# mauruszach/multimodal_diffusion

Measured on AMD Instinct MI355X. Metric: denoising steps/sec @256x256 multimodal-cond batch=32, higher is better.
Workload: dtype f32 via 3xbf16 split operands (6-term products, f32 accumulate; fp32-level error); 1 GPU; C3: 256x256 audio->video CFG denoising step (cond+null MMDiT d512 L8 H8 + noise head + DDIM), 384+37 tokens, batch 32 per GPU, DDIM 50 steps, guidance 3.5; global_batch=32, sampler_steps=50, parallelism=dp1, launch=eager, matmul=bf16x3, attn=default, cfg_halves=one stacked 2B batch, one stream

## Files before the change

include/avdiff_hip.h:

```cpp
#ifndef AVDIFF_HIP_H
#define AVDIFF_HIP_H

#include <stdint.h>

#ifdef __cplusplus
extern "C" {
#endif

#define AVD_ABI_VERSION 7

#define AVD_OK            0
#define AVD_EINVAL       -1
#define AVD_EUNSUPPORTED -2
#define AVD_ELAUNCH      -3
#define AVD_EWORKSPACE   -4

#define AVD_ACT_NONE 0
#define AVD_ACT_GELU 1
#define AVD_ACT_SILU 2
#define AVD_ACT_TANH 3
#define AVD_ACT_RELU 4
#define AVD_ACT_LEAKY_RELU 5

typedef void* avd_stream_t;

int         avd_abi_version(void);
const char* avd_last_error(void);
int         avd_device_arch(char* buf, int buflen);
int         avd_tune_set(const char* key, int64_t value);

int avd_rmsnorm_f32(const float* x, const float* scale, float* y, int64_t rows, int d, float eps,
                    avd_stream_t stream);

int avd_gemm_bias_act_f32(const float* A, int64_t lda, const float* W, const float* bias,
                          const float* residual, int64_t ldr, float* C, int64_t ldc,
                          int64_t M, int N, int K, int act, avd_stream_t stream);

int avd_gemm_rmsfold_f32(const float* A, const float* W, const float* bias, const float* residual, float* C, int64_t M,
                         int N, int K, int act, const float* ss_in, int ss_in_cols, float eps, float* ss_out,
                         avd_stream_t stream);

int avd_attn_fwd_f32(const float* qkv, float* out, int B, int N, int H, int Dh, float scale,
                     int n_query, const uint8_t* key_padding_mask, avd_stream_t stream);

int avd_layernorm_act_f32(const float* x, const float* gamma, const float* beta, float* y,
                          int64_t rows, int d, float eps, int act, avd_stream_t stream);

int avd_timestep_embedding_f32(const int64_t* t, const float* freqs, float* out, int B, int dim, float max_period,
                               avd_stream_t stream);

int avd_tube_patch_f32(const float* z, float* tok, int B, int C, int T, int H, int W, int t, int h, int w,
                       avd_stream_t stream);
int avd_tube_unpatch_f32(const float* tok, float* z, int B, int C, int T, int H, int W, int t, int h, int w,
                         avd_stream_t stream);

int avd_audio_tokens_f32(const float* z, float* tok, int B, int Ca, int F, int len, int stride,
                         avd_stream_t stream);
int avd_audio_untokens_f32(const float* tok, const float* window, float* z, int B, int Ca, int F, int len, int stride,
                           avd_stream_t stream);

int avd_ddim_step_f32(const float* x_t, const float* eps_hat, const int64_t* t_now, const int64_t* t_prev,
                      const float* alpha_bar, int T_train, float eta, const float* noise,
                      float* x_prev, int B, int64_t per_sample, avd_stream_t stream);

int avd_dpmpp_2m_step_f32(const float* x_t, const float* eps_hat, float* x0_hist, const int64_t* t_last, const int64_t* t_now,
                          const int64_t* t_prev, const float* alpha_bar, int T_train, float* x_out, int B, int64_t per_sample,
                          avd_stream_t stream);

int avd_dpmpp_2m_sde_step_f32(const float* x_t, const float* eps_hat, float* x0_hist, const int64_t* t_last, const int64_t* t_now,
                              const int64_t* t_prev, const float* alpha_bar, int T_train, float eta, const float* noise, float* x_out,
                              int B, int64_t per_sample, avd_stream_t stream);

typedef struct {
    uint64_t seed;
    int64_t sample_offset;
} avd_noise_key;
int avd_gaussian_noise_f32(const avd_noise_key* key, const int64_t* t_now, float* out, int B, int64_t per_sample,
                           avd_stream_t stream);

int avd_canvas_noise_f32(const avd_noise_key* key, const int64_t* t_now, float* out, int N, int64_t outer, int L, int hop,
                         int64_t inner, avd_stream_t stream);

// ... 277 lines not shown
```

multimodal_diffusion_amd/_lib.py:

```python
from __future__ import annotations

import ctypes as C
import os
from pathlib import Path
from typing import Optional

import torch

_HERE = Path(__file__).resolve().parent
LIB_PATH = Path(os.environ.get("AVDIFF_HIP_LIB", _HERE / "csrc" / "libavdiff_hip.so"))

ACT_NONE, ACT_GELU, ACT_SILU, ACT_TANH, ACT_RELU, ACT_LEAKY_RELU = 0, 1, 2, 3, 4, 5
EINVAL, EUNSUPPORTED, ELAUNCH, EWORKSPACE = -1, -2, -3, -4


class AvdError(RuntimeError):
    """A HIP-side failure (launch error, unsupported shape, workspace)."""


class EmbedDesc(C.Structure):
    _fields_ = [("target_kind", C.c_int), ("target_first", C.c_int), ("B", C.c_int), ("d", C.c_int),
                ("tdim", C.c_int), ("C", C.c_int), ("T", C.c_int), ("H", C.c_int), ("W", C.c_int),
                ("p0", C.c_int), ("p1", C.c_int), ("p2", C.c_int), ("Nt", C.c_int), ("Np", C.c_int),
                ("temb_freqs", C.c_void_p), ("temb_add", C.c_int)]
# ... 31 lines not shown
                ("guidance", C.c_float), ("eta", C.c_float), ("split_streams", C.c_int)]


class NoiseKey(C.Structure):
    _fields_ = [("seed", C.c_uint64), ("sample_offset", C.c_int64)]


class LatentGuide(C.Structure):
    _fields_ = [("known", C.c_void_p), ("mask", C.c_void_p), ("mask_batch_stride", C.c_int64), ("key", NoiseKey)]


class CfgControl(C.Structure):
    _fields_ = [("guidance", C.c_void_p), ("rescale", C.c_void_p), ("stats", C.c_void_p), ("stats_bytes", C.c_int64)]


class VaeDecodeDesc(C.Structure):
    _fields_ = [("B", C.c_int), ("Cv", C.c_int), ("Tp", C.c_int), ("Hp", C.c_int), ("Wp", C.c_int),
                ("T", C.c_int), ("H", C.c_int), ("W", C.c_int),
                ("base", C.c_int), ("n_blocks", C.c_int), ("out_ch", C.c_int), ("out_tanh", C.c_int),
                ("gn_eps", C.c_float),
                ("from_lat_w", C.c_void_p), ("from_lat_b", C.c_void_p),
                ("conv_w", C.POINTER(C.c_void_p)), ("conv_b", C.POINTER(C.c_void_p)),
                ("gn_w", C.POINTER(C.c_void_p)), ("gn_b", C.POINTER(C.c_void_p)),
                ("to_img_w", C.c_void_p), ("to_img_b", C.c_void_p),
                ("conv_w3", C.POINTER(C.c_void_p)), ("conv_terms", C.c_int),
                ("conv_w_scale", C.POINTER(C.c_float)), ("conv_a_scale", C.POINTER(C.c_float)),
                ("conv0_lat_w3", C.c_void_p), ("conv0_lat_btab", C.c_void_p), ("conv0_lat_w_scale", C.c_float),
                ("conv0_lat_packed", C.c_int)]


class VaeEncodeDesc(C.Structure):
    _fields_ = [("B", C.c_int), ("in_ch", C.c_int), ("T", C.c_int), ("H", C.c_int), ("W", C.c_int),
                ("t_down", C.c_int), ("s_down", C.c_int),
                ("base", C.c_int), ("n_blocks", C.c_int), ("lat_ch", C.c_int), ("gn_eps", C.c_float),
                ("conv_w", C.POINTER(C.c_void_p)), ("conv_b", C.POINTER(C.c_void_p)),
                ("gn_w", C.POINTER(C.c_void_p)), ("gn_b", C.POINTER(C.c_void_p)),
                ("to_lat_w", C.c_void_p), ("to_lat_b", C.c_void_p),
                ("conv_w3", C.POINTER(C.c_void_p)), ("conv_terms", C.c_int),
                ("conv_w_scale", C.POINTER(C.c_float)), ("conv_a_scale", C.POINTER(C.c_float)),
                ("conv0_pk_w3", C.c_void_p)]


ABI_VERSION = 7
_P, _I, _L, _F = C.c_void_p, C.c_int, C.c_int64, C.c_float

SIGNATURES = {
    "avd_abi_version": (_I, []),
    "avd_last_error": (C.c_char_p, []),
    "avd_device_arch": (_I, [C.c_char_p, _I]),
    "avd_rmsnorm_f32": (_I, [_P, _P, _P, _L, _I, _F, _P]),
    "avd_gemm_bias_act_f32": (_I, [_P, _L, _P, _P, _P, _L, _P, _L, _L, _I, _I, _I, _P]),
    "avd_gemm_rmsfold_f32": (_I, [_P, _P, _P, _P, _P, _L, _I, _I, _I, _P, _I, _F, _P, _P]),
    "avd_tune_set": (_I, [C.c_char_p, _L]),
    "avd_attn_fwd_f32": (_I, [_P, _P, _I, _I, _I, _I, _F, _I, _P, _P]),
    "avd_layernorm_act_f32": (_I, [_P, _P, _P, _P, _L, _I, _F, _I, _P]),
    "avd_timestep_embedding_f32": (_I, [_P, _P, _P, _I, _I, _F, _P]),
    "avd_tube_patch_f32": (_I, [_P, _P] + [_I] * 8 + [_P]),
    "avd_tube_unpatch_f32": (_I, [_P, _P] + [_I] * 8 + [_P]),
    "avd_audio_tokens_f32": (_I, [_P, _P] + [_I] * 5 + [_P]),
    "avd_audio_untokens_f32": (_I, [_P, _P, _P] + [_I] * 5 + [_P]),
    "avd_ddim_step_f32": (_I, [_P, _P, _P, _P, _P, _I, _F, _P, _P, _I, _L, _P]),
    "avd_cfg_unpatch_ddim_f32": (_I, [_P, _P, _P, _P, _P, _I, _F, _F, _P, _P] + [_I] * 8 + [_P]),
    "avd_cfg_untoken_ddim_audio_f32": (_I, [_P, _P, _P, _P, _P, _I, _F, _F, _P, _P] + [_I] * 5 + [_P]),
    "avd_embed_workspace_floats": (_L, [C.POINTER(EmbedDesc)]),
    "avd_embed_cfg_pair_f32": (_I, [C.POINTER(EmbedDesc), _P, _P, _P, _P, _P, _P, _P, _P]),
    "avd_core_workspace_bytes": (_L, [C.POINTER(CoreWeights), _I, _I]),
    "avd_core_forward_f32": (_I, [C.POINTER(CoreWeights), _P, _P, _I, _I, _I, _I, _P, _P, _L, _P]),
    "avd_head_workspace_bytes": (_L, [C.POINTER(HeadWeights), _L]),
    "avd_head_forward_f32": (_I, [C.POINTER(HeadWeights), _P, _L, _L, _L, _L, _P, _P, _L, _P]),
    "avd_step_workspace_bytes": (_L, [C.POINTER(StepDesc)]),
    "avd_denoise_step_f32": (_I, [C.POINTER(StepDesc), _P, _P, _P, _P, _P, _P, _P, _L, _P]),
    "avd_denoise_step_seeded_f32": (_I, [C.POINTER(StepDesc), C.POINTER(NoiseKey), _P, _P, _P, _P, _P, _P, _L, _P]),
    "avd_gaussian_noise_f32": (_I, [C.POINTER(NoiseKey), _P, _P, _I, _L, _P]),
    "avd_canvas_noise_f32": (_I, [C.POINTER(NoiseKey), _P, _P, _I, _L, _I, _I, _L, _P]),
    "avd_denoise_step_canvas_f32": (_I, [C.POINTER(StepDesc), C.POINTER(NoiseKey), _I, C.POINTER(CfgControl), C.POINTER(LatentGuide), _I,
                                         _P, _P, _P, _P, _P, _P, _L, _P]),
    "avd_sched_advance": (_I, [_P, _I, _P, _P, _P, _I, _P]),
    "avd_sched_advance_ms": (_I, [_P, _I, _P, _P, _P, _P, _I, _P]),
    "avd_dpmpp_2m_step_f32": (_I, [_P, _P, _P, _P, _P, _P, _P, _I, _P, _I, _L, _P]),
    "avd_denoise_step_dpmpp_2m_f32": (_I, [C.POINTER(StepDesc), _P, _P, _P, _P, _P, _P, _P, _P, _L, _P]),
    "avd_dpmpp_2m_sde_step_f32": (_I, [_P, _P, _P, _P, _P, _P, _P, _I, _F, _P, _P, _I, _L, _P]),
    "avd_denoise_step_dpmpp_2m_sde_f32": (_I, [C.POINTER(StepDesc), C.POINTER(NoiseKey), _I, C.POINTER(CfgControl), C.POINTER(LatentGuide),
                                               _I, _P, _P, _P, _P, _P, _P, _P, _P, _L, _P]),
    "avd_latent_guide_f32": (_I, [C.POINTER(LatentGuide), _P, _P, _I, _P, _P, _I, _L, _P]),
    "avd_latent_guide_canvas_f32": (_I, [C.POINTER(LatentGuide), _P, _P, _I, _P, _P, _I, _L, _I, _I, _L, _P]),
    "avd_denoise_step_canvas_guided_f32": (_I, [C.POINTER(StepDesc), C.POINTER(LatentGuide), _I, C.POINTER(NoiseKey), C.POINTER(CfgControl),
                                                _I, _P, _P, _P, _P, _P, _P, _P, _P, _L, _P]),
    "avd_denoise_step_guided_f32": (_I, [C.POINTER(StepDesc), C.POINTER(LatentGuide), C.POINTER(NoiseKey), _P, _P, _P, _P, _P, _P, _P,
                                         _P, _L, _P]),
    "avd_cfg_stats_bytes": (_L, [_I, _L]),
    "avd_cfg_rescale_f32": (_I, [_P, _P, _P, _P, _L, _P, _I, _L, _P]),
    "avd_denoise_step_cfg_f32": (_I, [C.POINTER(StepDesc), C.POINTER(CfgControl), C.POINTER(LatentGuide), C.POINTER(NoiseKey), _P, _P, _P,
                                      _P, _P, _P, _P, _P, _L, _P]),
    "avd_eps_unpatch_ddim_f32": (_I, [_P, _P, _P, _P, _P, _I, _F, _P, _P] + [_I] * 8 + [C.POINTER(NoiseKey), _P, _P, C.POINTER(LatentGuide), _P]),
    "avd_eps_untoken_ddim_audio_f32": (_I, [_P, _P, _P, _P, _P, _I, _F, _P, _P] + [_I] * 5 + [C.POINTER(NoiseKey), _P, _P,
                                                                                               C.POINTER(LatentGuide), _P]),
    "avd_embed_cond_f32": (_I, [C.POINTER(EmbedDesc), _P, _P, _P, _P, _P, _P, _P, _P, _P]),
    "avd_denoise_step_cond_f32": (_I, [C.POINTER(StepDesc), C.POINTER(LatentGuide), C.POINTER(NoiseKey), _P, _P, _P, _P, _P, _P, _P, _P,
                                       _P, _L, _P]),
    "avd_split3_bytes": (_L, [_L, _I]),
    "avd_split3_f32": (_I, [_P, _P, _L, _I, _P]),
    "avd_rmsnorm_split3_f32": (_I, [_P, _P, _P, _L, _I, _F, _P]),
    "avd_attn_fwd_split3_f32": (_I, [_P, _P, _I, _I, _I, _I, _F, _I, _P]),
    "avd_qkv3_bytes": (_L, [_I, _I, _I]),
    "avd_gemm_bf16x3_qkv3_f32": (_I, [_P, _P, _P, _P, _L, _I, _I, _I, _F, _I, _P]),
    "avd_attn_fwd_qkv3_f32": (_I, [_P, _P, _P, _I, _I, _I, _I, _I, _P]),
# ... 98 lines not shown
```

multimodal_diffusion_amd/csrc/attn_bf16x3.hip:

```cpp
#include "avd_common.h"

#include <stdlib.h>
#include <type_traits>

namespace avd {

constexpr int A3_DH = 64, A3_KT = 64, A3_NW = 4;
constexpr float A3_NEG = -1.0e30f;

typedef short s16x4 __attribute__((ext_vector_type(4)));
typedef unsigned int u32x2 __attribute__((ext_vector_type(2)));
typedef float f32x4t __attribute__((ext_vector_type(4)));

#define AVD_LDS_PTR(p) ((__attribute__((address_space(3))) void*)(p))
#define AVD_GLB_PTR(p) ((const __attribute__((address_space(1))) void*)(p))

template <int TERMS> struct A3Terms;
template <> struct A3Terms<6> { static constexpr int N = 6; static constexpr int PA[6] = {2, 0, 1, 1, 0, 0}; static constexpr int PB[6] = {0, 2, 1, 0, 1, 0}; };
template <> struct A3Terms<9> { static constexpr int N = 9; static constexpr int PA[9] = {2, 2, 1, 2, 0, 1, 1, 0, 0}; static constexpr int PB[9] = {2, 1, 2, 0, 2, 1, 0, 1, 0}; };
template <> struct A3Terms<1> { static constexpr int N = 1; static constexpr int PA[1] = {0}; static constexpr int PB[1] = {0}; };
template <> struct A3Terms<3> { static constexpr int N = 3; static constexpr int PA[3] = {0, 1, 0}; static constexpr int PB[3] = {1, 0, 0}; };

template <bool SPLIT_OUT, int TERMS>
__global__ __launch_bounds__(A3_NW * 64, 2) void attn_bf16x3_kernel(const unsigned char* __restrict__ img, float* __restrict__ out,
                                                                    int Bt, int N, int Npad, int H, int n_query, int nqb,
                                                                    float s_inv2, float v_inv, float o_scale, int out_tok) {
    constexpr int NW = A3_NW, ROWB = QKV3_ROWB;
    constexpr bool F16 = TERMS == 3;
    constexpr int NPL = s3_planes(TERMS);
    constexpr int PPW = 24 / NW;
    __shared__ __attribute__((aligned(16))) unsigned char Ks[A3_KT * ROWB];
    __shared__ __attribute__((aligned(16))) unsigned char Vs[A3_KT * ROWB];

    int qb, h, b;
    {
        const int nwg = gridDim.x, id = blockIdx.x, q = nwg >> 3, r = nwg & 7, x = id & 7;
        const int w = (x < r ? x * (q + 1) : r * (q + 1) + (x - r) * q) + (id >> 3);
        qb = w % nqb;
        h = (w / nqb) % H;
        b = w / (nqb * H);
    }
    const int tid = threadIdx.x, lane = tid & 63, wave = tid >> 6;
    const int l31 = lane & 31, hi = lane >> 5;
    const int64_t hstride = (int64_t)Npad * ROWB;
    const unsigned char* Qb = img + (((int64_t)0 * Bt + b) * H + h) * hstride;
    const unsigned char* Kb = img + (((int64_t)1 * Bt + b) * H + h) * hstride;
    const unsigned char* Vb = img + (((int64_t)2 * Bt + b) * H + h) * hstride;

    const int q_row = qb * (NW * 32) + wave * 32 + l31;
    bf16x8 qf[4][3];
    {
        const unsigned char* src = Qb + (int64_t)(q_row < N ? q_row : N - 1) * ROWB + hi * 16;
#pragma unroll
        for (int s = 0; s < 4; ++s)
#pragma unroll
            for (int p = 0; p < NPL; ++p) qf[s][p] = *reinterpret_cast<const bf16x8*>(src + p * 128 + s * 32);
    }

    auto dma = [&](const unsigned char* gsrc, unsigned char* ldst, int kt) {
        const int last_row = N - 1 - kt * A3_KT;
#pragma unroll
        for (int i = 0; i < PPW; ++i) {
            const int p = wave + NW * i;
            const int off = p * 1024 + lane * 16;
            int row = off / ROWB;
            const int within = off - row * ROWB;
            row = row < last_row ? row : last_row;
            __builtin_amdgcn_global_load_lds(AVD_GLB_PTR(gsrc + ((int64_t)kt * A3_KT + row) * ROWB + within), AVD_LDS_PTR(ldst + p * 1024), 16,
                                             0, 0);
        }
    };

    f32x16 o0, o1;
#pragma unroll
    for (int r = 0; r < 16; ++r) { o0[r] = 0.f; o1[r] = 0.f; }
    float m_run = A3_NEG, l_run = 0.f;

    const int nkt = (N + A3_KT - 1) / A3_KT;
    dma(Kb, Ks, 0);
    dma(Vb, Vs, 0);
    __builtin_amdgcn_s_waitcnt(0x0f70);
    __syncthreads();

    const int ksw = (l31 >> 1) & 7;
    const int k_rd = l31 * ROWB;
    const int i16 = lane & 15, cb = (lane >> 4) & 1;
    const int v_q = i16 >> 2, v_p = i16 & 3;

    const bool active = qb * (NW * 32) + wave * 32 < n_query;
    for (int kt = 0; kt < nkt; ++kt) {
        const bool more = (kt + 1) < nkt;
        if (!active) {
            __builtin_amdgcn_s_waitcnt(0x0f70);
            __syncthreads();
// ... 80 lines not shown
                const int key0 = 32 * kb + 16 * t + 4 * hi + v_q;
                const int sw = qkv3_swizzle(2, key0);
#pragma unroll
                for (int db = 0; db < 2; ++db) {
                    const int chunk = 4 * db + 2 * cb + (v_p >> 1);
                    bf16x8 vf[3];
#pragma unroll
                    for (int p = 0; p < NPL; ++p) {
                        const s16x4 lo = __builtin_amdgcn_ds_read_tr16_b64_v4i16((__attribute__((address_space(3))) s16x4*)AVD_LDS_PTR(
                            Vs + key0 * ROWB + p * 128 + ((chunk ^ sw) << 4) + 8 * (v_p & 1)));
                        const s16x4 up = __builtin_amdgcn_ds_read_tr16_b64_v4i16((__attribute__((address_space(3))) s16x4*)AVD_LDS_PTR(
                            Vs + (key0 + 8) * ROWB + p * 128 + ((chunk ^ sw) << 4) + 8 * (v_p & 1)));
                        const u32x2 a = __builtin_bit_cast(u32x2, lo), c2 = __builtin_bit_cast(u32x2, up);
                        const u32x4 w = {a[0], a[1], c2[0], c2[1]};
                        vf[p] = __builtin_bit_cast(bf16x8, w);
                    }
#pragma unroll
                    for (int tt = 0; tt < TT::N; ++tt) {
                        if (db == 0) o0 = mma16<F16>(vf[TT::PA[tt]], pf[TT::PB[tt]], o0);
                        else o1 = mma16<F16>(vf[TT::PA[tt]], pf[TT::PB[tt]], o1);
                    }
                }
            }
        __builtin_amdgcn_s_waitcnt(0x0f70);
        __syncthreads();
        if (more) dma(Vb, Vs, kt + 1);
    }
    if (!active) return;

    const float l_tot = l_run + __shfl_xor(l_run, 32, 64);
    const float inv = F16 ? v_inv / l_tot : 1.0f / l_tot;
    const int d = H * A3_DH;
    if constexpr (SPLIT_OUT) {
        float ch[8][4];
#pragma unroll
        for (int g4 = 0; g4 < 4; ++g4)
#pragma unroll
            for (int e = 0; e < 4; ++e) {
                ch[g4][e] = o0[4 * g4 + e] * inv;
                ch[4 + g4][e] = o1[4 * g4 + e] * inv;
            }
        unsigned char* o3 = reinterpret_cast<unsigned char*>(out);
#pragma unroll
        for (int c = 0; c < 8; c += 2) {
            float v[8];
#pragma unroll
            for (int e = 0; e < 4; ++e) {
                const float send = hi ? ch[c][e] : ch[c + 1][e];
                const float recv = __shfl_xor(send, 32, 64);
                v[e] = hi ? recv : ch[c][e];
                v[4 + e] = hi ? ch[c + 1][e] : recv;
            }
            if (q_row < n_query) {
                if constexpr (F16) store_split8_h2(o3, (int64_t)b * out_tok + q_row, h * A3_DH + 8 * (c + hi), d, v, o_scale);
                else store_split8(o3, (int64_t)b * out_tok + q_row, h * A3_DH + 8 * (c + hi), d, v);
            }
        }
    } else if (q_row < n_query) {
        float* dst = out + ((int64_t)b * out_tok + q_row) * d + h * A3_DH + 4 * hi;
#pragma unroll
        for (int g4 = 0; g4 < 4; ++g4) {
            f32x4 a = {o0[4 * g4] * inv, o0[4 * g4 + 1] * inv, o0[4 * g4 + 2] * inv, o0[4 * g4 + 3] * inv};
            f32x4 c = {o1[4 * g4] * inv, o1[4 * g4 + 1] * inv, o1[4 * g4 + 2] * inv, o1[4 * g4 + 3] * inv};
            *reinterpret_cast<f32x4*>(dst + 8 * g4) = a;
            *reinterpret_cast<f32x4*>(dst + 32 + 8 * g4) = c;
        }
    }
}

int g_attn_pipe = 1;

template <bool MORE_, bool KCL_, bool VCL_, bool COPY_> struct A3Flags {
    static constexpr bool MORE = MORE_, KCL = KCL_, VCL = VCL_, COPY = COPY_;
};

template <bool SPLIT_OUT, int TERMS>
__global__ __launch_bounds__(A3_NW * 64, 2) void attn_bf16x3_pipe_kernel(const unsigned char* __restrict__ img, float* __restrict__ out,
                                                                         int Bt, int N, int Npad, int H, int n_query, int nqb,
                                                                         float s_inv2, float v_inv, float o_scale, int out_tok) {
    constexpr int NW = A3_NW, ROWB = QKV3_ROWB;
    constexpr bool F16 = TERMS == 3;
    constexpr int NPL = s3_planes(TERMS);
    constexpr int PPW = 24 / NW;
    using TT = A3Terms<TERMS>;
    __shared__ __attribute__((aligned(16))) unsigned char Ks[A3_KT * ROWB];
    __shared__ __attribute__((aligned(16))) unsigned char Vs[A3_KT * ROWB];

    int qb, h, b;
    {
        const int nwg = gridDim.x, id = blockIdx.x, q = nwg >> 3, r = nwg & 7, x = id & 7;
        const int w = (x < r ? x * (q + 1) : r * (q + 1) + (x - r) * q) + (id >> 3);
        qb = w % nqb;
        h = (w / nqb) % H;
        b = w / (nqb * H);
    }
    const int tid = threadIdx.x, lane = tid & 63;
    const int wave = __builtin_amdgcn_readfirstlane(tid >> 6);
    const int l31 = lane & 31, hi = lane >> 5;
    const int64_t hstride = (int64_t)Npad * ROWB;
    const unsigned char* Qb = img + (((int64_t)0 * Bt + b) * H + h) * hstride;
    const unsigned char* Kb = img + (((int64_t)1 * Bt + b) * H + h) * hstride;
    const unsigned char* Vb = img + (((int64_t)2 * Bt + b) * H + h) * hstride;

    const int q_row = qb * (NW * 32) + wave * 32 + l31;
    bf16x8 qf[4][3];
    {
        const unsigned char* src = Qb + (int64_t)(q_row < N ? q_row : N - 1) * ROWB + hi * 16;
#pragma unroll
        for (int s = 0; s < 4; ++s)
#pragma unroll
            for (int p = 0; p < NPL; ++p) qf[s][p] = *reinterpret_cast<const bf16x8*>(src + p * 128 + s * 32);
    }
    auto dma_clamp = [&](const unsigned char* gsrc, unsigned char* ldst, int kt) {
        const int last_row = N - 1 - kt * A3_KT;
#pragma unroll
        for (int i = 0; i < PPW; ++i) {
            const int p = wave + NW * i;
            const int off = p * 1024 + lane * 16;
            int row = off / ROWB;
            const int within = off - row * ROWB;
            row = row < last_row ? row : last_row;
            __builtin_amdgcn_global_load_lds(AVD_GLB_PTR(gsrc + ((int64_t)kt * A3_KT + row) * ROWB + within), AVD_LDS_PTR(ldst + p * 1024), 16,
                                             0, 0);
        }
    };
    const unsigned lane16 = (unsigned)lane * 16u;
    auto dma_full = [&](const unsigned char* gsrc, unsigned char* ldst, int kt) {
        const unsigned char* base = gsrc + ((int64_t)kt * (A3_KT * ROWB) + wave * 1024);
#pragma unroll
        for (int i = 0; i < PPW; ++i)
            __builtin_amdgcn_global_load_lds(AVD_GLB_PTR(base + i * (NW * 1024) + lane16), AVD_LDS_PTR(ldst + (wave + NW * i) * 1024), 16, 0, 0);
    };
    auto sync = [&]() {
        __builtin_amdgcn_s_waitcnt(0x0f70);
        __syncthreads();
    };

    const int nkt = (N + A3_KT - 1) / A3_KT;
    const bool ragged = (N & (A3_KT - 1)) != 0;
    dma_clamp(Kb, Ks, 0);
    dma_clamp(Vb, Vs, 0);
    sync();

    const bool active = qb * (NW * 32) + wave * 32 < n_query;
    if (!active) {
        sync();
        if (nkt > 1) dma_clamp(Kb, Ks, 1);
        sync();
// ... 179 lines not shown
            mt = fmaxf(mt, __shfl_xor(mt, 32, 64));
            m_new = fmaxf(m_run, mt);
            if constexpr (FL::COPY) {
                c0 = n0;
                c1 = n1;
            }
            sync();
            if constexpr (FL::VCL) dma_clamp(Vb, Vs, kt + 1);
            else dma_full(Vb, Vs, kt + 1);
        }
    };
    {
        using Main = A3Flags<true, false, false, false>;
        using MainC = A3Flags<true, false, false, true>;
        using KClamp = A3Flags<true, true, false, true>;
        using VClamp = A3Flags<true, false, true, true>;
        using Last = A3Flags<false, false, false, false>;
        int kt = 0;
        for (; kt + 4 < nkt; kt += 2) {
            tile(Main{}, kt, sa0, sa1, sb0, sb1);
            tile(Main{}, kt + 1, sb0, sb1, sa0, sa1);
        }
        if (nkt - kt == 4) { tile(MainC{}, kt, sa0, sa1, sb0, sb1); ++kt; }
        if (nkt - kt == 3) { tile(KClamp{}, kt, sa0, sa1, sb0, sb1); ++kt; }
        if (nkt - kt == 2) { tile(VClamp{}, kt, sa0, sa1, sb0, sb1); ++kt; }
        tile(Last{}, kt, sa0, sa1, sb0, sb1);
    }
#undef A3_SB

    const float l_tot = l_run + __shfl_xor(l_run, 32, 64);
    const float inv = F16 ? v_inv / l_tot : 1.0f / l_tot;
    const int d = H * A3_DH;
    if constexpr (SPLIT_OUT) {
        float ch[8][4];
#pragma unroll
        for (int g4 = 0; g4 < 4; ++g4)
#pragma unroll
            for (int e = 0; e < 4; ++e) {
                ch[g4][e] = o0[4 * g4 + e] * inv;
                ch[4 + g4][e] = o1[4 * g4 + e] * inv;
            }
        unsigned char* o3 = reinterpret_cast<unsigned char*>(out);
#pragma unroll
        for (int c = 0; c < 8; c += 2) {
            float v[8];
#pragma unroll
            for (int e = 0; e < 4; ++e) {
                const float send = hi ? ch[c][e] : ch[c + 1][e];
                const float recv = __shfl_xor(send, 32, 64);
                v[e] = hi ? recv : ch[c][e];
                v[4 + e] = hi ? ch[c + 1][e] : recv;
            }
            if (q_row < n_query) {
                if constexpr (F16) store_split8_h2(o3, (int64_t)b * out_tok + q_row, h * A3_DH + 8 * (c + hi), d, v, o_scale);
                else store_split8(o3, (int64_t)b * out_tok + q_row, h * A3_DH + 8 * (c + hi), d, v);
            }
        }
    } else if (q_row < n_query) {
        float* dst = out + ((int64_t)b * out_tok + q_row) * d + h * A3_DH + 4 * hi;
#pragma unroll
        for (int g4 = 0; g4 < 4; ++g4) {
            f32x4 a = {o0[4 * g4] * inv, o0[4 * g4 + 1] * inv, o0[4 * g4 + 2] * inv, o0[4 * g4 + 3] * inv};
            f32x4 c = {o1[4 * g4] * inv, o1[4 * g4 + 1] * inv, o1[4 * g4 + 2] * inv, o1[4 * g4 + 3] * inv};
            *reinterpret_cast<f32x4*>(dst + 8 * g4) = a;
            *reinterpret_cast<f32x4*>(dst + 32 + 8 * g4) = c;
        }
    }
}

template <bool F16>
__device__ __forceinline__ f32x4t mma16s(bf16x8 a, bf16x8 b, f32x4t c) {
    if constexpr (F16) return __builtin_amdgcn_mfma_f32_16x16x32_f16(__builtin_bit_cast(f16x8, a), __builtin_bit_cast(f16x8, b), c, 0, 0, 0);
    else return __builtin_amdgcn_mfma_f32_16x16x32_bf16(a, b, c, 0, 0, 0);
}
int g_attn_m16 = 1;

struct S16 { f32x4t t[4][2]; };

template <bool SPLIT_OUT, int TERMS>
__global__ __launch_bounds__(A3_NW * 64, 2) void attn_bf16x3_p16_kernel(const unsigned char* __restrict__ img, float* __restrict__ out,
                                                                        int Bt, int N, int Npad, int H, int n_query, int nqb,
                                                                        float s_inv2, float v_inv, float o_scale, int out_tok) {
    constexpr int NW = A3_NW, ROWB = QKV3_ROWB;
    constexpr bool F16 = TERMS == 3;
    constexpr int NPL = s3_planes(TERMS);
    constexpr int PPW = 24 / NW;
    using TT = A3Terms<TERMS>;
    __shared__ __attribute__((aligned(16))) unsigned char Ks[A3_KT * ROWB];
    __shared__ __attribute__((aligned(16))) unsigned char Vs[A3_KT * ROWB];

    int qb, h, b;
    {
        const int nwg = gridDim.x, id = blockIdx.x, q = nwg >> 3, r = nwg & 7, x = id & 7;
        const int w = (x < r ? x * (q + 1) : r * (q + 1) + (x - r) * q) + (id >> 3);
        qb = w % nqb;
        h = (w / nqb) % H;
        b = w / (nqb * H);
    }
    const int tid = threadIdx.x, lane = tid & 63;
    const int wave = __builtin_amdgcn_readfirstlane(tid >> 6);
    const int l15 = lane & 15, kq = lane >> 4;
    const int64_t hstride = (int64_t)Npad * ROWB;
    const unsigned char* Qb = img + (((int64_t)0 * Bt + b) * H + h) * hstride;
    const unsigned char* Kb = img + (((int64_t)1 * Bt + b) * H + h) * hstride;
    const unsigned char* Vb = img + (((int64_t)2 * Bt + b) * H + h) * hstride;

    const int q_row0 = qb * (NW * 32) + wave * 32 + l15;
    bf16x8 qf[2][2][3];
#pragma unroll
    for (int qt = 0; qt < 2; ++qt) {
        const int qr = q_row0 + 16 * qt;
        const unsigned char* src = Qb + (int64_t)(qr < N ? qr : N - 1) * ROWB + kq * 16;
#pragma unroll
        for (int sd = 0; sd < 2; ++sd)
#pragma unroll
            for (int p = 0; p < NPL; ++p) qf[qt][sd][p] = *reinterpret_cast<const bf16x8*>(src + p * 128 + sd * 64);
    }
    auto dma_clamp = [&](const unsigned char* gsrc, unsigned char* ldst, int kt) {
        const int last_row = N - 1 - kt * A3_KT;
#pragma unroll
        for (int i = 0; i < PPW; ++i) {
            const int p = wave + NW * i;
            const int off = p * 1024 + lane * 16;
            int row = off / ROWB;
            const int within = off - row * ROWB;
            row = row < last_row ? row : last_row;
            __builtin_amdgcn_global_load_lds(AVD_GLB_PTR(gsrc + ((int64_t)kt * A3_KT + row) * ROWB + within), AVD_LDS_PTR(ldst + p * 1024), 16,
                                             0, 0);
        }
    };
    const unsigned lane16 = (unsigned)lane * 16u;
    auto dma_full = [&](const unsigned char* gsrc, unsigned char* ldst, int kt) {
        const unsigned char* base = gsrc + ((int64_t)kt * (A3_KT * ROWB) + wave * 1024);
#pragma unroll
        for (int i = 0; i < PPW; ++i)
            __builtin_amdgcn_global_load_lds(AVD_GLB_PTR(base + i * (NW * 1024) + lane16), AVD_LDS_PTR(ldst + (wave + NW * i) * 1024), 16, 0, 0);
    };
    auto sync = [&]() {
        __builtin_amdgcn_s_waitcnt(0x0f70);
        __syncthreads();
    };

    const int nkt = (N + A3_KT - 1) / A3_KT;
    const bool ragged = (N & (A3_KT - 1)) != 0;
    dma_clamp(Kb, Ks, 0);
    dma_clamp(Vb, Vs, 0);
    sync();

    const bool active = qb * (NW * 32) + wave * 32 < n_query;
    if (!active) {
        sync();
// ... 202 lines not shown
        }
        A3_SB();
        if constexpr (MORE) {
#pragma unroll
            for (int qt = 0; qt < 2; ++qt) {
                if constexpr (F16) mt[qt] *= s_inv2;
                m_new[qt] = fmaxf(m_run[qt], xmax(mt[qt]));
            }
            if constexpr (FL::COPY) c = n;
            sync();
            if constexpr (FL::VCL) dma_clamp(Vb, Vs, kt + 1);
            else dma_full(Vb, Vs, kt + 1);
        }
    };
    {
        using Main = A3Flags<true, false, false, false>;
        using MainC = A3Flags<true, false, false, true>;
        using KClamp = A3Flags<true, true, false, true>;
        using VClamp = A3Flags<true, false, true, true>;
        using Last = A3Flags<false, false, false, false>;
        int kt = 0;
        for (; kt + 4 < nkt; kt += 2) {
            tile(Main{}, kt, sa, sb);
            tile(Main{}, kt + 1, sb, sa);
        }
        if (nkt - kt == 4) { tile(MainC{}, kt, sa, sb); ++kt; }
        if (nkt - kt == 3) { tile(KClamp{}, kt, sa, sb); ++kt; }
        if (nkt - kt == 2) { tile(VClamp{}, kt, sa, sb); ++kt; }
        tile(Last{}, kt, sa, sb);
    }
#undef A3_SB

    float inv[2];
#pragma unroll
    for (int qt = 0; qt < 2; ++qt) {
        const float l_tot = xsum(l_run[qt]);
        inv[qt] = F16 ? v_inv / l_tot : 1.0f / l_tot;
    }
    const int d = H * A3_DH;
    const int q_row = q_row0 + 16 * (kq & 1);
    unsigned char* o3 = reinterpret_cast<unsigned char*>(out);
#pragma unroll
    for (int dt = 0; dt < 4; ++dt) {
        float v[8];
#pragma unroll
        for (int r = 0; r < 4; ++r) {
            const auto sw = __builtin_amdgcn_permlane16_swap(__float_as_uint(o[dt][0][r] * inv[0]), __float_as_uint(o[dt][1][r] * inv[1]), false, false);
            v[r] = __uint_as_float(sw[0]);
            v[4 + r] = __uint_as_float(sw[1]);
        }
        const int col = h * A3_DH + 16 * dt + 8 * (kq >> 1);
        if (q_row < n_query) {
            if constexpr (SPLIT_OUT) {
                if constexpr (F16) store_split8_h2(o3, (int64_t)b * out_tok + q_row, col, d, v, o_scale);
                else store_split8(o3, (int64_t)b * out_tok + q_row, col, d, v);
            } else {
                float* dst = out + ((int64_t)b * out_tok + q_row) * d + col;
                *reinterpret_cast<f32x4*>(dst) = f32x4{v[0], v[1], v[2], v[3]};
                *reinterpret_cast<f32x4*>(dst + 4) = f32x4{v[4], v[5], v[6], v[7]};
            }
        }
    }
}

int64_t qkv3_bytes(int B, int N, int H) { return (int64_t)3 * B * H * qkv3_npad(N) * QKV3_ROWB; }

template <int TERMS>
static void attn3_launch(const unsigned char* img, float* out, void* out3, int B, int N, int Npad, int H, int n_query, int nqb, hipStream_t st,
                         float img_scale, float out_scale, int out_tok) {
    const float s_inv2 = 1.0f / (img_scale * img_scale), v_inv = 1.0f / img_scale;
    if (g_attn_m16 && (TERMS == 6 || TERMS == 9 || g_attn_m16 == 2)) {
        if (out3)
            hipLaunchKernelGGL((attn_bf16x3_p16_kernel<true, TERMS>), dim3(nqb * H * B), dim3(A3_NW * 64), 0, st, img, static_cast<float*>(out3),
                               B, N, Npad, H, n_query, nqb, s_inv2, v_inv, out_scale, out_tok);
        else
            hipLaunchKernelGGL((attn_bf16x3_p16_kernel<false, TERMS>), dim3(nqb * H * B), dim3(A3_NW * 64), 0, st, img, out, B, N, Npad, H,
                               n_query, nqb, s_inv2, v_inv, out_scale, out_tok);
        return;
    }
    if (g_attn_pipe == 2 || (g_attn_pipe == 1 && (TERMS == 6 || TERMS == 9))) {
        if (out3)
            hipLaunchKernelGGL((attn_bf16x3_pipe_kernel<true, TERMS>), dim3(nqb * H * B), dim3(A3_NW * 64), 0, st, img, static_cast<float*>(out3),
                               B, N, Npad, H, n_query, nqb, s_inv2, v_inv, out_scale, out_tok);
        else
            hipLaunchKernelGGL((attn_bf16x3_pipe_kernel<false, TERMS>), dim3(nqb * H * B), dim3(A3_NW * 64), 0, st, img, out, B, N, Npad, H,
                               n_query, nqb, s_inv2, v_inv, out_scale, out_tok);
        return;
    }
    if (out3)
        hipLaunchKernelGGL((attn_bf16x3_kernel<true, TERMS>), dim3(nqb * H * B), dim3(A3_NW * 64), 0, st, img, static_cast<float*>(out3), B, N,
                           Npad, H, n_query, nqb, s_inv2, v_inv, out_scale, out_tok);
    else
        hipLaunchKernelGGL((attn_bf16x3_kernel<false, TERMS>), dim3(nqb * H * B), dim3(A3_NW * 64), 0, st, img, out, B, N, Npad, H, n_query, nqb,
                           s_inv2, v_inv, out_scale, out_tok);
}

int attn_bf16x3(const void* qkv3, float* out, void* out3, int B, int N, int H, int n_query, int terms, hipStream_t st, float img_scale,
                float out_scale, int out_tokens) {
    const int out_tok = out_tokens > 0 ? out_tokens : N;
    AVD_REQUIRE(out_tok >= n_query, AVD_EINVAL, "attn_bf16x3: out_tokens=%d < n_query=%d", out_tok, n_query);
    AVD_REQUIRE(terms == 0 || terms == 6 || terms == 9 || terms == 1 || terms == 3, AVD_EINVAL, "attn_bf16x3: terms must be 6, 9, 1 or 3, got %d", terms);
    AVD_REQUIRE(img_scale > 0.f && img_scale < __builtin_inff() && out_scale > 0.f && out_scale < __builtin_inff() &&
                    img_scale * img_scale < __builtin_inff(), AVD_EINVAL, "attn_bf16x3: image scales must be positive and finite");
    AVD_REQUIRE(qkv3 && (out || out3), AVD_EINVAL, "attn_bf16x3: null pointer");
    AVD_REQUIRE(B > 0 && N > 0 && H > 0, AVD_EINVAL, "attn_bf16x3: bad dims B=%d N=%d H=%d", B, N, H);
    AVD_REQUIRE(n_query >= 0 && n_query <= N, AVD_EINVAL, "attn_bf16x3: n_query=%d outside [0,%d]", n_query, N);
    AVD_REQUIRE(aligned16(qkv3) && aligned16(out) && aligned16(out3), AVD_EUNSUPPORTED, "attn_bf16x3: pointers must be 16-byte aligned");
    AVD_REQUIRE(!out3 || (H * A3_DH) % 16 == 0, AVD_EUNSUPPORTED, "attn_bf16x3: split3 output needs d %% 16 == 0");
    if (n_query == 0) return AVD_OK;
    const int nqb = (n_query + 32 * A3_NW - 1) / (32 * A3_NW);
    AVD_REQUIRE((int64_t)B * H * nqb < (1ll << 31), AVD_EUNSUPPORTED, "attn_bf16x3: grid too large");
    const int tag = prof_tag_id("attn_bf16x3_kernel<%d>", terms ? terms : 6);
    ProfScope prof(tag, 4.0 * (double)B * H * (double)n_query * N * A3_DH, st);
    const int Npad = qkv3_npad(N);
    const auto* img = static_cast<const unsigned char*>(qkv3);
    if (terms == 9) attn3_launch<9>(img, out, out3, B, N, Npad, H, n_query, nqb, st, 1.f, 1.f, out_tok);
    else if (terms == 1) attn3_launch<1>(img, out, out3, B, N, Npad, H, n_query, nqb, st, 1.f, 1.f, out_tok);
    else if (terms == 3) attn3_launch<3>(img, out, out3, B, N, Npad, H, n_query, nqb, st, img_scale, out_scale, out_tok);
    else attn3_launch<6>(img, out, out3, B, N, Npad, H, n_query, nqb, st, 1.f, 1.f, out_tok);
    AVD_CHECK_LAUNCH("attn_bf16x3");
    return AVD_OK;
}

}

extern "C" int64_t avd_qkv3_bytes(int B, int N, int H) {
    if (B <= 0 || N <= 0 || H <= 0) return -1;
    return avd::qkv3_bytes(B, N, H);
}
extern "C" int avd_attn_fwd_qkv_f16x2_f32(const void* qkv, float* out, void* out2, int B, int N, int H, int n_query, float qkv_scale,
                                          float out_scale, avd_stream_t stream) {
    return avd::attn_bf16x3(qkv, out, out2, B, N, H, n_query, 3, static_cast<hipStream_t>(stream), qkv_scale, out_scale);
}
extern "C" int avd_attn_fwd_qkv3_f32(const void* qkv3, float* out, void* out3, int B, int N, int H, int n_query, int terms,
                                     avd_stream_t stream) {
    return avd::attn_bf16x3(qkv3, out, out3, B, N, H, n_query, terms, static_cast<hipStream_t>(stream));
}
```

multimodal_diffusion_amd/csrc/avd_common.h:

```cpp
#pragma once
#include <hip/hip_runtime.h>
#include <stdint.h>
#include <stdio.h>
#include <stdarg.h>
#include <atomic>

#include "../../include/avdiff_hip.h"

namespace avd {

int set_error(int code, const char* fmt, ...);

#define AVD_REQUIRE(cond, code, ...)                       \
    do {                                                   \
        if (!(cond)) return avd::set_error((code), __VA_ARGS__); \
    } while (0)

#define AVD_CHECK_LAUNCH(name)                                                          \
    do {                                                                                \
        hipError_t e__ = hipGetLastError();                                             \
        if (e__ != hipSuccess)                                                          \
            return avd::set_error(AVD_ELAUNCH, "%s: %s", (name), hipGetErrorString(e__)); \
    } while (0)

struct LdsAttr {
    std::atomic<uint64_t> done{0};
    int ensure(const void* kern, int lds_bytes, const char* what);
};

static inline bool aligned16(const void* p) { return (reinterpret_cast<uintptr_t>(p) & 15u) == 0; }

typedef float f32x4 __attribute__((ext_vector_type(4)));
typedef float f32x16 __attribute__((ext_vector_type(16)));

constexpr int kWave = 64;

__device__ __forceinline__ int mfma32_row(int r, int hi) { return (r & 3) + 8 * (r >> 2) + 4 * hi; }

__device__ __forceinline__ float gelu_erf(float x) {
    const float z = x * 0.70710678118654752440f;
    const float a = fabsf(z);
    const float t = __builtin_amdgcn_rcpf(fmaf(0.3275911f, a, 1.0f));
    float p = fmaf(1.061405429f, t, -1.453152027f);
    p = fmaf(p, t, 1.421413741f);
    p = fmaf(p, t, -0.284496736f);
    p = fmaf(p, t, 0.254829592f);
    p *= t;
    const float e = __builtin_amdgcn_exp2f(-a * a * 1.4426950408889634f);
    const float er = copysignf(fmaf(-p, e, 1.0f), z);
    return 0.5f * x * (1.0f + er);
}
__device__ __forceinline__ float silu(float x) { return x / (1.0f + expf(-x)); }

template <int ACT>
__device__ __forceinline__ float apply_act(float x) {
    if constexpr (ACT == AVD_ACT_GELU) return gelu_erf(x);
    else if constexpr (ACT == AVD_ACT_SILU) return silu(x);
    else return x;
}

__device__ __forceinline__ float wave_sum(float v) {
#pragma unroll
    for (int o = 32; o > 0; o >>= 1) v += __shfl_xor(v, o, 64);
    return v;
}

struct RowMap {
    int64_t ld;
    int64_t seg;
    int64_t stride;
    __host__ __device__ __forceinline__ int64_t off(int64_t r) const {
        return seg > 0 ? (r / seg) * stride + (r % seg) * ld : r * ld;
    }
};

struct TubeGather {
    int T, H, W, t, h, w, Ht, Wt, Nt;
    int64_t per;
    __host__ __device__ __forceinline__ int64_t row_off(int64_t row) const {
        const int64_t b = row / Nt;
        const int n = (int)(row - b * Nt);
        const int nx = n % Wt, ny = (n / Wt) % Ht, nt = n / (Wt * Ht);
        return b * per + ((int64_t)(nt * t) * H + ny * h) * W + nx * w;
    }
    __host__ __device__ __forceinline__ int64_t k_off(int k) const {
        const int dx = k % w, dy = (k / w) % h, dt = (k / (w * h)) % t, c = k / (w * h * t);
        return (((int64_t)c * T + dt) * H + dy) * W + dx;
    }
};

typedef __bf16 bf16x8 __attribute__((ext_vector_type(8)));
typedef unsigned int u32x4 __attribute__((ext_vector_type(4)));

constexpr int S3_CHUNK = 128 * 96;
constexpr int S3_PLANE = 128 * 32;

typedef __bf16 bf16x2 __attribute__((ext_vector_type(2)));
typedef float f32x2 __attribute__((ext_vector_type(2)));

__device__ __forceinline__ unsigned int pk_bf16(float a, float b) {
    const f32x2 v = {a, b};
    return __builtin_bit_cast(unsigned int, __builtin_convertvector(v, bf16x2));
}
__device__ __forceinline__ float bf16_lo(unsigned int p) { return __uint_as_float(p << 16); }
__device__ __forceinline__ float bf16_hi(unsigned int p) { return __uint_as_float(p & 0xffff0000u); }

template <bool RANGE_CHECK = true>
__device__ __forceinline__ void split8(const float* v, u32x4& H, u32x4& Mi, u32x4& Lo) {
#pragma clang fp contract(off)
    bool edge = false;
    if constexpr (RANGE_CHECK) {
        float amax = fabsf(v[0]);
#pragma unroll
        for (int e = 1; e < 8; ++e) amax = fmaxf(amax, fabsf(v[e]));
        edge = __any(amax > 3.3895313892515355e38f);
    }
#pragma unroll
    for (int e = 0; e < 4; ++e) {
        const float a = v[2 * e], b = v[2 * e + 1];
        unsigned int h = pk_bf16(a, b);
        float ra = a - bf16_lo(h), rb = b - bf16_hi(h);
        if (edge) {
            if ((h & 0x7fffu) == 0x7f80u) {
                if (fabsf(a) < __builtin_inff()) { h = (h & 0xffff8000u) | 0x7f7fu; ra = a - bf16_lo(h); } else ra = 0.f;
            }
// ... 76 lines not shown
             float* C, RowMap cm, int64_t M, int N, int K, int act, hipStream_t st);
int gemm_f32_tube(const float* z, const TubeGather& tg, const float* W, const float* bias, float* C, RowMap cm, int64_t M, int N, int K,
                  hipStream_t st);

extern int g_gemm_stages;
extern int g_gemm_force_tile;
bool gemm_f32_fold_supported(int N, int K);
int gemm_f32_fold(const float* A, RowMap am, const float* W, const float* bias, const float* R, RowMap rm, float* C, RowMap cm,
                  int64_t M, int N, int K, int act, const float* ss_in, int ss_in_cols, float sqrt_d, float eps, float* ss_out,
                  hipStream_t st);
int rowss_f32(const float* x, float* ss, int64_t rows, int d, hipStream_t st);
constexpr int kGemmSplitKMax = 4;
extern int g_gemm_splitk;
int gemm_f32_splitk_slices(int64_t M, int N, int K);
int64_t gemm_f32_splitk_ws_max_floats(int64_t M, int N, int K);
int gemm_f32_splitk(const float* A, RowMap am, const float* W, const float* bias, const float* R, RowMap rm, float* C, RowMap cm, int64_t M,
                    int N, int K, int ns, float* part, float* ss_out, hipStream_t st);

int attn_f32(const float* qkv, float* out, int B, int N, int H, int Dh, float scale, int n_query, const unsigned char* key_padding_mask,
             hipStream_t st);
int rmsnorm_f32(const float* x, RowMap xm, const float* scale, float* y, RowMap ym, int64_t rows, int d, float eps,
                hipStream_t st);
int layernorm_act_f32(const float* x, const float* gamma, const float* beta, float* y, int64_t rows, int d, float eps,
                      int act, hipStream_t st);
int weight_bounds_f32(const float* x, int64_t rows, int d, float* out2, hipStream_t st);

int64_t split3_bytes(int64_t rows, int K);
int split3_f32(const float* x, int64_t ld, void* out, int64_t rows, int K, hipStream_t st, float h2_scale = 0.f);
int split3_rows_f32(const float* x, RowMap xm, void* out, int64_t rows, int K, hipStream_t st, float h2_scale = 0.f, float* ss = nullptr);
int rmsnorm_split3_f32(const float* x, const float* scale, void* out, int64_t rows, int d, float eps, hipStream_t st, float h2_scale = 0.f);
int layernorm_act_split3_f32(const float* x, const float* gamma, const float* beta, void* out, int64_t rows, int d, float eps, int act,
                             hipStream_t st, float h2_scale = 0.f);
bool gemm_bf16x3_supported(int64_t M, int N, int K);
int attn_f32_split3(const float* qkv, void* out3, int B, int N, int H, int Dh, float scale, int n_query, hipStream_t st);
extern int g_s3_stagger;
extern int g_mlp_fused;
bool mlp_bf16x3_supported(int d, int hidden, int terms);
int mlp_bf16x3(const void* X3, const void* W1n3, const float* b1, const void* W23, const float* b2, const float* ss_in, float eps,
               const float* R, float* C, void* C3, float* ss_out, int64_t M, int d, int hidden, hipStream_t st);
extern int g_attn_m16;
extern int g_attn_pipe;
extern int g_s3_m16;
extern int g_s3_w128;
extern int g_s3_rt4;
extern int g_s3_deep4;
extern int g_s3_rt;
extern int g_vae_lat;
extern int g_vae_fold;
extern int g_codec_mfma;
extern int g_cfg_rows;
extern int g_s3_sn, g_s3_super4, g_s3_super8;
extern int g_s3_tile;
extern thread_local bool t_s3_two_streams;
int gemm_bf16x3_qkv3(const void* A3, const void* W3, const float* bias, void* img, int64_t M, int tokens, int heads, int K, float qscale,
                     int terms, hipStream_t st, float ab_scale = 1.f, float c_scale = 1.f, const float* ss_in = nullptr, float eps = 0.f);
int64_t qkv3_bytes(int B, int N, int H);
int64_t attn_fp8_ws_bytes(int B, int N, int H);
int attn_fp8(const void* qkv3, void* ws, int64_t ws_bytes, float* out, void* out3, int B, int N, int H, int n_query, hipStream_t st,
             int img_terms = 6, float img_scale = 1.f, float out_scale = 1.f);
int attn_bf16x3(const void* qkv3, float* out, void* out3, int B, int N, int H, int n_query, int terms, hipStream_t st,
                float img_scale = 1.f, float out_scale = 1.f, int out_tokens = 0);
int gemm_bf16x3(const void* A3, const void* W3, const float* bias, const float* R, float* C, void* C3, int64_t M, int N, int K,
                int act, int terms, hipStream_t st, float ab_scale = 1.f, float c_scale = 1.f, const float* ss_in = nullptr, float eps = 0.f,
                float* ss_out = nullptr, const float* gamma = nullptr, int r_seg = 0, int r_stride = 0);
bool gemm_bf16x3_resmap_supported(int terms);
bool gemm_bf16x3_rownorm_supported(int N, int terms);
extern int g_s3_splitk;
int gemm_bf16x3_splitk_slices(int64_t M, int N, int K, int terms);
int64_t gemm_bf16x3_splitk_ws_floats(int64_t M, int N, int ns);
constexpr int kS3SplitKMax = 4;
int64_t gemm_bf16x3_splitk_ws_max_floats(int64_t M, int N, int K);
int gemm_bf16x3_splitk(const void* A3, const void* W3, const float* bias, const float* R, float* C, void* C3, float* ss, int64_t M, int N,
                       int K, int terms, int ns, float* part, hipStream_t st);

}
```

multimodal_diffusion_amd/csrc/composite.hip:

```cpp
#include "avd_common.h"

#include <limits.h>
#include <stdlib.h>

#include <string.h>
#include <map>
#include <mutex>
#include <string>
#include <utility>
#include <vector>

namespace avd {

static thread_local char g_err[512] = "";

int set_error(int code, const char* fmt, ...) {
    va_list ap;
    va_start(ap, fmt);
    vsnprintf(g_err, sizeof(g_err), fmt, ap);
    va_end(ap);
    return code;
}

int LdsAttr::ensure(const void* kern, int lds_bytes, const char* what) {
    int dev = 0;
    hipError_t e = hipGetDevice(&dev);
    if (e != hipSuccess) return set_error(AVD_ELAUNCH, "%s: hipGetDevice: %s", what, hipGetErrorString(e));
    const uint64_t bit = dev < 64 ? (uint64_t)1 << dev : 0;
    if (bit && (done.load(std::memory_order_acquire) & bit)) return AVD_OK;
    e = hipFuncSetAttribute(kern, hipFuncAttributeMaxDynamicSharedMemorySize, lds_bytes);
    if (e != hipSuccess) return set_error(AVD_ELAUNCH, "%s: hipFuncSetAttribute: %s", what, hipGetErrorString(e));
    done.fetch_or(bit, std::memory_order_release);
    return AVD_OK;
}

bool g_prof_on = false;
namespace {
struct ProfRec { hipEvent_t a, b; int tag; double work; };
std::vector<ProfRec> g_recs;
std::vector<hipEvent_t> g_pool;
std::vector<std::string> g_tags;
hipEvent_t take_event() {
    if (!g_pool.empty()) { hipEvent_t e = g_pool.back(); g_pool.pop_back(); return e; }
    hipEvent_t e; (void)hipEventCreate(&e); return e;
}
}
int prof_tag_id(const char* fmt, ...) {
    char buf[160];
    va_list ap;
    va_start(ap, fmt);
    vsnprintf(buf, sizeof(buf), fmt, ap);
    va_end(ap);
    for (size_t i = 0; i < g_tags.size(); ++i)
        if (g_tags[i] == buf) return (int)i;
    g_tags.emplace_back(buf);
    return (int)g_tags.size() - 1;
}
void prof_mark(int tag, double work, hipStream_t st, bool begin) {
    if (begin) {
        ProfRec r{take_event(), take_event(), tag, work};
        (void)hipEventRecord(r.a, st);
        g_recs.push_back(r);
    } else if (!g_recs.empty()) {
        (void)hipEventRecord(g_recs.back().b, st);
    }
}

int temb_f32(const int64_t* t, const float* freqs, float* out, int B, int dim, float max_period, hipStream_t st);
int tube_patch_f32(const float* z, float* tok, int B, int C, int T, int H, int W, int t, int h, int w, hipStream_t st);
int audio_tokens_f32(const float* z, float* tok, int B, int Ca, int F, int len, int stride, hipStream_t st);
int assemble_f32(float* X2, const float* temb, const float* Xp, int B, int N, int d, int tdim, int Nt, int Np,
                 int target_first, hipStream_t st);
int assemble_rows_f32(float* X2, const int64_t* t_now, const float* freqs, const float* Xp, float* ss, int B, int N, int d, int tdim,
                      int Nt, int Np, int target_first, float max_period, hipStream_t st);
int cfg_unpatch_ddim_f32(const float* eps2, const float* z, const int64_t* t_now, const int64_t* t_prev,
                         const float* abar, int T_train, float guidance, float eta, const float* noise, float* z_out,
                         int B, int C, int T, int H, int W, int t, int h, int w, hipStream_t st, const avd_noise_key* key = nullptr,
                         const int64_t* t_last = nullptr, float* x0_hist = nullptr, const avd_latent_guide* guide = nullptr,
                         const avd_cfg_control* ctl = nullptr, int canvas_hop = 0, int guide_hop = 0);
int cfg_untoken_ddim_audio_f32(const float* eps2, const float* z, const int64_t* t_now, const int64_t* t_prev,
                               const float* abar, int T_train, float guidance, float eta, const float* noise,
                               float* z_out, int B, int Ca, int F, int len, int stride, hipStream_t st,
                               const avd_noise_key* key = nullptr, const int64_t* t_last = nullptr, float* x0_hist = nullptr,
                               const avd_latent_guide* guide = nullptr, const avd_cfg_control* ctl = nullptr, int canvas_hop = 0, int guide_hop = 0);
int assemble_cond_f32(float* X1, const float* temb, const float* Xp, int B, int N, int d, int tdim, int Nt, int Np, int target_first,
                      hipStream_t st);
int assemble_rows_cond_f32(float* X1, const int64_t* t_now, const float* freqs, const float* Xp, float* ss, int B, int N, int d,
                           int tdim, int Nt, int Np, int target_first, float max_period, hipStream_t st);
int eps_unpatch_ddim_f32(const float* eps1, const float* z, const int64_t* t_now, const int64_t* t_prev, const float* abar, int T_train,
                         float eta, const float* noise, float* z_out, int B, int C, int T, int H, int W, int t, int h, int w,
                         hipStream_t st, const avd_noise_key* key, const int64_t* t_last, float* x0_hist, const avd_latent_guide* guide,
                         int canvas_hop = 0, int guide_hop = 0);
int eps_untoken_ddim_audio_f32(const float* eps1, const float* z, const int64_t* t_now, const int64_t* t_prev, const float* abar,
                               int T_train, float eta, const float* noise, float* z_out, int B, int Ca, int F, int len, int stride,
                               hipStream_t st, const avd_noise_key* key, const int64_t* t_last, float* x0_hist,
                               const avd_latent_guide* guide, int canvas_hop = 0, int guide_hop = 0);
int check_canvas_key(const avd_noise_key* key, int N, int64_t outer, int L, int hop, int64_t inner);
int check_canvas_guide(const avd_latent_guide* g, int N, int64_t outer, int L, int hop, int64_t inner, const float* out,
                       const float* x0_hist);
int check_latent_guide(const avd_latent_guide* g, int B, int64_t per, const float* out, const float* x0_hist);
int check_cfg_control(const avd_cfg_control* ctl, int B, int64_t per, const float* out, const float* x0_hist);
bool overlaps(const float* a, const float* b, int64_t n);

static inline int64_t align_up(int64_t x) { return (x + 255) & ~(int64_t)255; }

struct Carver {
    char* base;
    int64_t used, cap;
    bool ok = true;
    float* take(int64_t floats) {
        float* p = reinterpret_cast<float*>(base + used);
        used += align_up(floats * (int64_t)sizeof(float));
        if (used > cap) ok = false;
        return p;
    }
};

constexpr int64_t kSplitMinRows = 6144;
constexpr int64_t kSplitMinRowsM16 = 2048;
static int g_s3_min_rows = -1;
static int g_no_fold = 0;
static int64_t split_min_rows(int terms = 3) {
    if (g_s3_min_rows >= 0) return g_s3_min_rows;
    return (terms == 0 || terms == 6) && g_s3_m16 ? kSplitMinRowsM16 : kSplitMinRows;
}
static bool core_split_capable(const avd_core_weights* w, int64_t M) {
    if (w->norm_kind != 0) return false;
    if (!gemm_bf16x3_supported(M, 3 * w->d, w->d) || !gemm_bf16x3_supported(M, w->d, w->d) ||
        !gemm_bf16x3_supported(M, w->mlp_hidden, w->d) || !gemm_bf16x3_supported(M, w->d, w->mlp_hidden))
        return false;
    for (int l = 0; l < w->n_layers; ++l) {
        const avd_block_weights& b = w->blocks[l];
        if (!b.in_proj_weight3 || !b.out_proj_weight3 || !b.fc1_weight3 || !b.fc2_weight3) return false;
    }
    return true;
}
static thread_local int64_t t_step_rows = 0;
static bool core_use_split(const avd_core_weights* w, int64_t M) {
    const int64_t Mt = t_step_rows > M ? t_step_rows : M;
    if (Mt < split_min_rows(w->split_terms) && w->split_terms != 1 && w->attn_mode != 1) return false;
    return core_split_capable(w, M);
}

static bool core_split_fold_capable(const avd_core_weights* w) {
    if (w->norm_kind != 0 || w->split_terms == 3 || w->d % 64 != 0) return false;
    for (int l = 0; l < w->n_layers; ++l)
        if (!w->blocks[l].in_proj_weight3n || !w->blocks[l].fc1_weight3n) return false;
    return true;
}
static bool core_use_split_fold(const avd_core_weights* w) { return !g_no_fold && core_split_fold_capable(w); }

static bool core_split_rownorm_capable(const avd_core_weights* w) {
    return w->norm_kind == 0 && w->split_terms == 3 && gemm_bf16x3_rownorm_supported(w->d, 3);
}
static bool core_use_split_rownorm(const avd_core_weights* w) { return !g_no_fold && core_split_rownorm_capable(w); }

static bool core_use_fold(const avd_core_weights* w) {
    if (g_no_fold || w->norm_kind != 0) return false;
    if (!gemm_f32_fold_supported(3 * w->d, w->d) || !gemm_f32_fold_supported(w->d, w->d) ||
        !gemm_f32_fold_supported(w->mlp_hidden, w->d) || !gemm_f32_fold_supported(w->d, w->mlp_hidden))
        return false;
    for (int l = 0; l < w->n_layers; ++l)
        if (!w->blocks[l].in_proj_weight_n || !w->blocks[l].fc1_weight_n) return false;
    return true;
}

static int g_core_trim = 1;
static int64_t core_trim_floats(const avd_core_weights* w, int B, int N) { return (int64_t)B * N * w->d; }

static int64_t core_split_wide_bytes(const avd_core_weights* w, int B, int N) {
    const int64_t qkv3 = qkv3_bytes(B, N, w->n_heads), fc1 = split3_bytes((int64_t)B * N, w->mlp_hidden);
    return qkv3 > fc1 ? qkv3 : fc1;
}

static int64_t core_ws_bytes(const avd_core_weights* w, int B, int N) {
    const int64_t M = (int64_t)B * N;
    const int wide = 3 * w->d > w->mlp_hidden ? 3 * w->d : w->mlp_hidden;
    int64_t fp32_path = align_up(M * w->d * 4) + align_up(M * wide * 4) + 2 * align_up(M * (w->d / 32 + 1) * 4) +
                        align_up(gemm_f32_splitk_ws_max_floats(M, w->d, w->mlp_hidden) * 4);
    if (!core_split_capable(w, M)) return fp32_path;
    const int64_t wide_b = core_split_wide_bytes(w, B, N);
    const int64_t f8_b = w->attn_mode == 1 ? attn_fp8_ws_bytes(B, N, w->n_heads) : 0;
    const int64_t fold_b = core_split_fold_capable(w) ? align_up(split3_bytes(M, w->d)) + align_up(M * (w->d / 64) * 4)
                         : core_split_rownorm_capable(w) ? align_up(split3_bytes(M, w->d)) : 0;
    const int64_t sk_b = core_split_fold_capable(w) ? align_up(gemm_bf16x3_splitk_ws_max_floats(M, w->d, w->mlp_hidden) * 4) : 0;
    const int64_t trim_b = core_split_fold_capable(w) ? align_up(core_trim_floats(w, B, N) * 4) : 0;
    const int64_t split_path = align_up(wide_b) + align_up(split3_bytes(M, w->d)) + align_up(f8_b) + fold_b + sk_b + trim_b;
    return split_path > fp32_path ? split_path : fp32_path;
}

static int check_core(const avd_core_weights* w) {
    AVD_REQUIRE(w && w->blocks && w->final_norm_scale, AVD_EINVAL, "core: null weight table");
    AVD_REQUIRE(w->d > 0 && w->n_layers > 0 && w->n_heads > 0 && w->mlp_hidden > 0, AVD_EINVAL, "core: bad dims");
    AVD_REQUIRE(w->d % w->n_heads == 0, AVD_EINVAL, "core: d_model %d not divisible by n_heads %d", w->d, w->n_heads);
    AVD_REQUIRE(w->attn_mode == 0 || w->attn_mode == 1, AVD_EINVAL, "core: attn_mode must be 0 (follow the matmul mode) or 1 (fp8)");
    AVD_REQUIRE(w->norm_kind == 0 || w->norm_kind == 1, AVD_EINVAL, "core: norm_kind must be 0 (RMSNorm) or 1 (LayerNorm)");
    AVD_REQUIRE(w->d / w->n_heads == 64, AVD_EUNSUPPORTED, "core: head_dim %d unsupported (64 only)", w->d / w->n_heads);
    AVD_REQUIRE(w->d % 4 == 0 && w->mlp_hidden % 4 == 0, AVD_EUNSUPPORTED, "core: widths must be multiples of 4");
    AVD_REQUIRE(w->split_terms == 0 || w->split_terms == 6 || w->split_terms == 9 || w->split_terms == 1 || w->split_terms == 3, AVD_EINVAL,
                "core: split_terms must be 0/6 (default), 9 (strict), 1 (plain bf16) or 3 (f16x2), got %d", w->split_terms);
    if (w->split_terms == 3) {
        for (int l = 0; l < w->n_layers; ++l)
            for (int i = 0; i < 8; ++i) {
                const float s = w->blocks[l].f16x2_scale[i];
                AVD_REQUIRE(s > 0.f && s < __builtin_inff(), AVD_EINVAL, "core: blocks[%d].f16x2_scale[%d] must be positive and finite", l, i);
            }
    }
    return AVD_OK;
}

static int core_norm(const avd_core_weights* w, const float* x, const float* scale, const float* bias, float* y, int64_t M, hipStream_t st) {
    const RowMap rd{w->d, 0, 0};
    if (w->norm_kind == 0) return rmsnorm_f32(x, rd, scale, y, rd, M, w->d, w->norm_eps, st);
    AVD_REQUIRE(bias, AVD_EINVAL, "core: norm_kind 1 (LayerNorm) needs the bias vectors");
    return layernorm_act_f32(x, scale, bias, y, M, w->d, w->norm_eps, AVD_ACT_NONE, st);
}

static int core_forward(const avd_core_weights* w, const float* x, float* y, int B, int N, int out_row0,
                        int n_out_rows, const unsigned char* kpm, void* ws, int64_t ws_bytes, hipStream_t st,
                        const float* ss_first = nullptr) {
    if (int rc = check_core(w)) return rc;
    AVD_REQUIRE(x && y && B > 0 && N > 0, AVD_EINVAL, "core: bad input");
    AVD_REQUIRE(out_row0 >= 0 && n_out_rows > 0 && out_row0 + n_out_rows <= N, AVD_EINVAL, "core: bad output row window");
    const int64_t M = (int64_t)B * N;
    AVD_REQUIRE(ws && ws_bytes >= core_ws_bytes(w, B, N), AVD_EWORKSPACE, "core: workspace %lld < %lld bytes",
                (long long)ws_bytes, (long long)core_ws_bytes(w, B, N));
    const int d = w->d, hid = w->mlp_hidden, H = w->n_heads;
    Carver cv{static_cast<char*>(ws), 0, ws_bytes};
    float* hbuf = cv.take(M * d);
    float* wide = cv.take(M * (3 * d > hid ? 3 * d : hid));
    const RowMap rd{d, 0, 0}, r3{3 * d, 0, 0}, rh{hid, 0, 0};
    const float scale = 1.0f / sqrtf((float)(d / H));
    const float* cur = x;
    AVD_REQUIRE(!(w->attn_mode == 1 && (kpm || w->norm_kind != 0)), AVD_EUNSUPPORTED,
                "core: attn_mode 1 (fp8 attention) cannot be combined with a key_padding_mask or norm_kind 1 (LayerNorm)");
    AVD_REQUIRE(!(w->attn_mode == 1 && !core_use_split(w, M)), AVD_EUNSUPPORTED,
                "core: attn_mode 1 (fp8 attention) reads the q|k|v image of the split-operand projections, which these weights / shapes "
                "do not take (every block needs its *_weight3 images; 3 d, d and mlp_hidden must be multiples of 256, d of 16)");
    if (!kpm && core_use_split(w, M)) {
        const int terms = w->split_terms;
        Carver cs{static_cast<char*>(ws), 0, ws_bytes};
        const int64_t wide_b = core_split_wide_bytes(w, B, N);
        float* qkv = cs.take((wide_b + 3) / 4);
        void* wide3 = qkv;
        void* hs = cs.take((split3_bytes(M, d) + 3) / 4);
        const int64_t f8_b = w->attn_mode == 1 ? attn_fp8_ws_bytes(B, N, H) : 0;
        float* f8w = cs.take((f8_b + 3) / 4);
        if (core_use_split_fold(w)) {
            void* hx = cs.take((split3_bytes(M, d) + 3) / 4);
            float* ss = cs.take(M * (d / 64));
            const int ns = gemm_bf16x3_splitk_slices(M, d, hid, terms);
            float* part = ns ? cs.take(gemm_bf16x3_splitk_ws_floats(M, d, ns)) : nullptr;
            const bool trim = g_core_trim && out_row0 == 0 && n_out_rows < N && w->attn_mode == 0 && gemm_bf16x3_resmap_supported(terms);
            float* yc = cs.take(core_trim_floats(w, B, N));
            const bool fused = g_mlp_fused && !ns && mlp_bf16x3_supported(d, hid, terms) && gemm_bf16x3_resmap_supported(terms);
            AVD_REQUIRE(cs.ok, AVD_EWORKSPACE, "core: workspace carve %lld > %lld bytes", (long long)cs.used, (long long)cs.cap);
            if (int rc = split3_rows_f32(cur, rd, hx, M, d, st, 0.f, ss)) return rc;
            for (int l = 0; l < w->n_layers; ++l) {
                const avd_block_weights& b = w->blocks[l];
                const bool last = l == w->n_layers - 1;
                const int nq = (last && out_row0 == 0) ? n_out_rows : N;
                if (last && trim) {
                    const int64_t Mc = (int64_t)B * nq;
                    if (int rc = gemm_bf16x3_qkv3(hx, b.in_proj_weight3n, b.in_proj_bias, qkv, M, N, H, d, scale * 1.4426950408889634f, terms, st,
                                                  1.f, 1.f, ss, w->norm_eps)) return rc;
                    if (int rc = attn_bf16x3(qkv, nullptr, hs, B, N, H, nq, terms, st, 1.f, 1.f, nq)) return rc;
                    if (int rc = gemm_bf16x3(hs, b.out_proj_weight3, b.out_proj_bias, cur, yc, hx, Mc, d, d, AVD_ACT_NONE, terms, st, 1.f, 1.f,
                                             nullptr, 0.f, ss, nullptr, nq, N)) return rc;
                    if (fused) {
                        if (int rc = mlp_bf16x3(hx, b.fc1_weight3n, b.fc1_bias, b.fc2_weight3, b.fc2_bias, ss, w->norm_eps, yc, yc, nullptr, nullptr, Mc,
                                                d, hid, st)) return rc;
                    } else {
                        if (int rc = gemm_bf16x3(hx, b.fc1_weight3n, b.fc1_bias, nullptr, nullptr, wide3, Mc, hid, d, AVD_ACT_GELU, terms, st, 1.f, 1.f,
                                                 ss, w->norm_eps)) return rc;
                        if (ns) {
                            if (int rc = gemm_bf16x3_splitk(wide3, b.fc2_weight3, b.fc2_bias, yc, yc, nullptr, nullptr, Mc, d, hid, terms, ns, part,
                                                            st)) return rc;
                        } else {
                            if (int rc = gemm_bf16x3(wide3, b.fc2_weight3, b.fc2_bias, yc, yc, nullptr, Mc, d, hid, AVD_ACT_NONE, terms, st)) return rc;
                        }
                    }
                    return rmsnorm_f32(yc, rd, w->final_norm_scale, y, RowMap{d, nq, (int64_t)N * d}, Mc, d, w->norm_eps, st);
                }
                if (int rc = gemm_bf16x3_qkv3(hx, b.in_proj_weight3n, b.in_proj_bias, qkv, M, N, H, d, scale * 1.4426950408889634f, terms, st,
                                              1.f, 1.f, ss, w->norm_eps)) return rc;
                if (w->attn_mode == 1) {
                    if (int rc = attn_fp8(qkv, f8w, f8_b, nullptr, hs, B, N, H, nq, st, terms, 1.f, 1.f)) return rc;
                } else {
                    if (int rc = attn_bf16x3(qkv, nullptr, hs, B, N, H, nq, terms, st, 1.f, 1.f)) return rc;
                }
                if (int rc = gemm_bf16x3(hs, b.out_proj_weight3, b.out_proj_bias, cur, y, hx, M, d, d, AVD_ACT_NONE, terms, st, 1.f, 1.f, nullptr,
                                         0.f, ss)) return rc;
                cur = y;
                if (fused) {
                    if (int rc = mlp_bf16x3(hx, b.fc1_weight3n, b.fc1_bias, b.fc2_weight3, b.fc2_bias, ss, w->norm_eps, y, y, last ? nullptr : hx,
                                            last ? nullptr : ss, M, d, hid, st)) return rc;
                    continue;
                }
                if (int rc = gemm_bf16x3(hx, b.fc1_weight3n, b.fc1_bias, nullptr, nullptr, wide3, M, hid, d, AVD_ACT_GELU, terms, st, 1.f, 1.f, ss,
                                         w->norm_eps)) return rc;
                if (ns) {
                    if (int rc = gemm_bf16x3_splitk(wide3, b.fc2_weight3, b.fc2_bias, y, y, last ? nullptr : hx, last ? nullptr : ss, M, d, hid,
                                                    terms, ns, part, st)) return rc;
                } else if (last) {
                    if (int rc = gemm_bf16x3(wide3, b.fc2_weight3, b.fc2_bias, y, y, nullptr, M, d, hid, AVD_ACT_NONE, terms, st)) return rc;
                } else {
                    if (int rc = gemm_bf16x3(wide3, b.fc2_weight3, b.fc2_bias, y, y, hx, M, d, hid, AVD_ACT_NONE, terms, st, 1.f, 1.f, nullptr, 0.f,
                                             ss)) return rc;
                }
            }
            return rmsnorm_f32(y, rd, w->final_norm_scale, y, rd, M, d, w->norm_eps, st);
        }
        const bool rown = core_use_split_rownorm(w);
        void* hn = rown ? cs.take((split3_bytes(M, d) + 3) / 4) : hs;
        AVD_REQUIRE(cs.ok, AVD_EWORKSPACE, "core: workspace carve %lld > %lld bytes", (long long)cs.used, (long long)cs.cap);
        for (int l = 0; l < w->n_layers; ++l) {
            const avd_block_weights& b = w->blocks[l];
            const bool last = l == w->n_layers - 1;
            const int nq = (last && out_row0 == 0) ? n_out_rows : N;
            const bool h2 = terms == 3;
            const float* fs = b.f16x2_scale;
            const float s_n1 = h2 ? fs[4] : 0.f, s_qkv = h2 ? fs[5] : 1.f, s_n2 = h2 ? fs[6] : 0.f, s_fc1 = h2 ? fs[7] : 1.f;
            const float w_in = h2 ? fs[0] : 1.f, w_out = h2 ? fs[1] : 1.f, w_fc1 = h2 ? fs[2] : 1.f, w_fc2 = h2 ? fs[3] : 1.f;
            if (!rown || l == 0)
                if (int rc = rmsnorm_split3_f32(cur, b.norm1_scale, hn, M, d, w->norm_eps, st, s_n1)) return rc;
            if (int rc = gemm_bf16x3_qkv3(hn, b.in_proj_weight3, b.in_proj_bias, qkv, M, N, H, d, scale * 1.4426950408889634f, terms, st,
                                          h2 ? s_n1 * w_in : 1.f, s_qkv)) return rc;
            if (w->attn_mode == 1) {
                if (int rc = attn_fp8(qkv, f8w, f8_b, nullptr, hs, B, N, H, nq, st, terms, s_qkv, s_qkv)) return rc;
            } else {
                if (int rc = attn_bf16x3(qkv, nullptr, hs, B, N, H, nq, terms, st, s_qkv, s_qkv)) return rc;
            }
            if (rown) {
                if (int rc = gemm_bf16x3(hs, b.out_proj_weight3, b.out_proj_bias, cur, y, hn, M, d, d, AVD_ACT_NONE, terms, st, s_qkv * w_out, s_n2,
                                         nullptr, w->norm_eps, nullptr, b.norm2_scale)) return rc;
                cur = y;
            } else {
                if (int rc = gemm_bf16x3(hs, b.out_proj_weight3, b.out_proj_bias, cur, y, nullptr, M, d, d, AVD_ACT_NONE, terms, st,
                                         h2 ? s_qkv * w_out : 1.f, 1.f)) return rc;
                cur = y;
                if (int rc = rmsnorm_split3_f32(y, b.norm2_scale, hn, M, d, w->norm_eps, st, s_n2)) return rc;
            }
            if (int rc = gemm_bf16x3(hn, b.fc1_weight3, b.fc1_bias, nullptr, nullptr, wide3, M, hid, d, AVD_ACT_GELU, terms, st,
                                     h2 ? s_n2 * w_fc1 : 1.f, s_fc1)) return rc;
            if (rown && !last) {
                const avd_block_weights& nb = w->blocks[l + 1];
                if (int rc = gemm_bf16x3(wide3, b.fc2_weight3, b.fc2_bias, y, y, hn, M, d, hid, AVD_ACT_NONE, terms, st, s_fc1 * w_fc2,
                                         nb.f16x2_scale[4], nullptr, w->norm_eps, nullptr, nb.norm1_scale)) return rc;
            } else {
                if (int rc = gemm_bf16x3(wide3, b.fc2_weight3, b.fc2_bias, y, y, nullptr, M, d, hid, AVD_ACT_NONE, terms, st,
                                         h2 ? s_fc1 * w_fc2 : 1.f, 1.f)) return rc;
            }
        }
        return rmsnorm_f32(y, rd, w->final_norm_scale, y, rd, M, d, w->norm_eps, st);
    }
    if (core_use_fold(w)) {
        float* ssA = cv.take(M * (d / 32 + 1));
        float* ssB = cv.take(M * (d / 32 + 1));
        const int nsf = gemm_f32_splitk_slices(M, d, hid);
        float* partf = nsf ? cv.take((int64_t)nsf * M * d) : nullptr;
        AVD_REQUIRE(cv.ok, AVD_EWORKSPACE, "core: workspace carve %lld > %lld bytes", (long long)cv.used, (long long)cv.cap);
        const float sqrt_d = (float)sqrt((double)d);
        const float* ssA_in = ss_first;
        if (!ssA_in) {
            if (int rc = rowss_f32(cur, ssA, M, d, st)) return rc;
            ssA_in = ssA;
        }
        int colsA = 1;
        for (int l = 0; l < w->n_layers; ++l) {
            const avd_block_weights& b = w->blocks[l];
            const bool last = l == w->n_layers - 1;
            const int nq = (last && out_row0 == 0) ? n_out_rows : N;
            if (int rc = gemm_f32_fold(cur, rd, b.in_proj_weight_n, b.in_proj_bias, nullptr, rd, wide, r3, M, 3 * d, d, AVD_ACT_NONE,
                                       l == 0 ? ssA_in : ssA, colsA, sqrt_d, w->norm_eps, nullptr, st)) return rc;
            if (int rc = attn_f32(wide, hbuf, B, N, H, d / H, scale, nq, kpm, st)) return rc;
            if (int rc = gemm_f32_fold(hbuf, rd, b.out_proj_weight, b.out_proj_bias, cur, rd, y, rd, M, d, d, AVD_ACT_NONE, nullptr, 0,
                                       1.f, 0.f, ssB, st)) return rc;
            cur = y;
            if (int rc = gemm_f32_fold(y, rd, b.fc1_weight_n, b.fc1_bias, nullptr, rd, wide, rh, M, hid, d, AVD_ACT_GELU, ssB, d / 32,
// ... 74 lines not shown
        if (int rc = split3_rows_f32(h, hm, imgA, rows, w->d_in, st, asc(0))) return rc;
        if (int rc = gemm_bf16x3(imgA, w->input_proj_weight3, w->input_proj_bias, nullptr, nullptr, imgB, rows, w->hidden, w->d_in, AVD_ACT_NONE,
                                 terms, st, h2 ? asc(0) * wsc(0) : 1.f, h2 ? asc(1) : 1.f)) return rc;
        void* cur = imgB;
        void* nxt = imgA;
        for (int j = 0; j < n; ++j) {
            if (int rc = gemm_bf16x3(cur, w->shared_lin_weight3[j], w->shared_lin_bias[j], nullptr, t2, nullptr, rows, w->hidden, w->hidden,
                                     AVD_ACT_NONE, terms, st, h2 ? asc(1 + j) * wsc(1 + j) : 1.f, 1.f)) return rc;
            if (int rc = layernorm_act_split3_f32(t2, w->shared_ln_weight[j], w->shared_ln_bias[j], nxt, rows, w->hidden, w->ln_eps, w->act, st,
                                                  asc(2 + j))) return rc;
            void* t = cur; cur = nxt; nxt = t;
        }
        return gemm_bf16x3(cur, w->out_proj_weight3, w->out_proj_bias, nullptr, out, nullptr, rows, w->d_out, w->hidden, AVD_ACT_NONE, terms, st,
                           h2 ? asc(1 + n) * wsc(1 + n) : 1.f, 1.f);
    }
    float* t1 = cv.take(rows * w->hidden);
    float* t2 = cv.take(rows * w->hidden);
    if (int rc = gemm_f32(h, hm, w->input_proj_weight, w->input_proj_bias, nullptr, rh, t1, rh, rows, w->hidden, w->d_in, AVD_ACT_NONE, st)) return rc;
    for (int j = 0; j < w->n_shared; ++j) {
        if (int rc = gemm_f32(t1, rh, w->shared_lin_weight[j], w->shared_lin_bias[j], nullptr, rh, t2, rh, rows, w->hidden, w->hidden, AVD_ACT_NONE, st)) return rc;
        if (int rc = layernorm_act_f32(t2, w->shared_ln_weight[j], w->shared_ln_bias[j], t1, rows, w->hidden, w->ln_eps, w->act, st)) return rc;
    }
    return gemm_f32(t1, rh, w->out_proj_weight, w->out_proj_bias, nullptr, ro, out, ro, rows, w->d_out, w->hidden, AVD_ACT_NONE, st);
}

static int check_embed(const avd_embed_desc* e) {
    AVD_REQUIRE(e, AVD_EINVAL, "embed: null descriptor");
    AVD_REQUIRE(e->B > 0 && e->d > 0 && e->tdim >= 0, AVD_EINVAL, "embed: bad widths");
    AVD_REQUIRE(e->temb_add ? e->tdim == e->d : e->tdim < e->d, AVD_EINVAL,
                "embed: timestep width %d does not fit token width %d in %s mode", e->tdim, e->d, e->temb_add ? "add" : "concat");
    AVD_REQUIRE(e->d % 4 == 0 && e->tdim % 4 == 0, AVD_EUNSUPPORTED, "embed: d and tdim must be multiples of 4");
    AVD_REQUIRE(e->Nt > 0 && e->Np >= 0, AVD_EINVAL, "embed: bad token counts");
    if (e->target_kind == 0) {
        AVD_REQUIRE(e->p0 > 0 && e->p1 > 0 && e->p2 > 0 && e->T % e->p0 == 0 && e->H % e->p1 == 0 && e->W % e->p2 == 0,
                    AVD_EINVAL, "tube sizes must divide latent dims");
        AVD_REQUIRE(e->Nt == (e->T / e->p0) * (e->H / e->p1) * (e->W / e->p2), AVD_EINVAL, "embed: token count mismatch");
    } else if (e->target_kind == 1) {
        AVD_REQUIRE(e->p0 > 0 && e->p1 > 0 && e->T >= e->p0, AVD_EINVAL, "embed: bad audio chunking");
        AVD_REQUIRE(e->Nt == (e->T - e->p0) / e->p1 + 1, AVD_EINVAL, "embed: token count mismatch");
    } else {
        return set_error(AVD_EINVAL, "embed: unknown target_kind %d", e->target_kind);
    }
    return AVD_OK;
}
static int embed_tok_dim(const avd_embed_desc* e) {
    return e->target_kind == 0 ? e->C * e->p0 * e->p1 * e->p2 : e->C * e->p0;
}
static int64_t embed_ws_floats(const avd_embed_desc* e) {
    return align_up((int64_t)e->B * e->Nt * embed_tok_dim(e) * 4) / 4 + align_up((int64_t)e->B * (e->tdim > 0 ? e->tdim : 1) * 4) / 4;
}

static int embed_cfg_pair(const avd_embed_desc* e, const float* z, const float* Wt, const float* bt,
                          const int64_t* t_now, const float* Xp, float* tok_ws, float* X2, hipStream_t st, float* ss_out = nullptr,
                          bool cond_only = false) {
    if (int rc = check_embed(e)) return rc;
    AVD_REQUIRE(z && Wt && t_now && tok_ws && X2 && (e->Np == 0 || Xp), AVD_EINVAL, "embed: null pointer");
    const int B = e->B, d = e->d, N = e->Nt + e->Np, D = embed_tok_dim(e);
    float* tok = tok_ws;
    float* temb = tok_ws + align_up((int64_t)B * e->Nt * D * 4) / 4;
    const bool fuse_patch = e->target_kind == 0 && !e->temb_add && e->p2 % 4 == 0 && e->W % 4 == 0 && D % 4 == 0 && aligned16(z);
    if (e->target_kind == 0) {
        if (!fuse_patch)
            if (int rc = tube_patch_f32(z, tok, B, e->C, e->T, e->H, e->W, e->p0, e->p1, e->p2, st)) return rc;
    } else {
        if (int rc = audio_tokens_f32(z, tok, B, e->C, e->T, e->p0, e->p1, st)) return rc;
    }
    if (e->tdim > 0 && e->temb_add)
        if (int rc = temb_f32(t_now, e->temb_freqs, temb, B, e->tdim, 10000.f, st)) return rc;
    float* c0 = X2 + (e->target_first ? 0 : (int64_t)e->Np * d);
    const RowMap cm{d, e->Nt, (int64_t)N * d};
    if (e->temb_add) {
        const RowMap rm{0, e->Nt, (int64_t)e->tdim};
        if (int rc = gemm_f32(tok, RowMap{D, 0, 0}, Wt, bt, temb, rm, c0, cm, (int64_t)B * e->Nt, d, D, AVD_ACT_NONE, st)) return rc;
        if (cond_only) return assemble_cond_f32(X2, temb, Xp, B, N, d, 0, e->Nt, e->Np, e->target_first, st);
        return assemble_f32(X2, temb, Xp, B, N, d, 0, e->Nt, e->Np, e->target_first, st);
    }
    if (fuse_patch) {
        const TubeGather tg{e->T, e->H, e->W, e->p0, e->p1, e->p2, e->H / e->p1, e->W / e->p2, e->Nt, (int64_t)e->C * e->T * e->H * e->W};
        if (int rc = gemm_f32_tube(z, tg, Wt, bt, c0, cm, (int64_t)B * e->Nt, d - e->tdim, D, st)) return rc;
    } else {
        if (int rc = gemm_f32(tok, RowMap{D, 0, 0}, Wt, bt, nullptr, cm, c0, cm, (int64_t)B * e->Nt, d - e->tdim, D, AVD_ACT_NONE, st)) return rc;
    }
    if (cond_only)
        return assemble_rows_cond_f32(X2, t_now, e->temb_freqs, Xp, ss_out, B, N, d, e->tdim, e->Nt, e->Np, e->target_first, 10000.f, st);
    return assemble_rows_f32(X2, t_now, e->temb_freqs, Xp, ss_out, B, N, d, e->tdim, e->Nt, e->Np, e->target_first, 10000.f, st);
}

#define AVD_HIP(call)                                                                        \
    do {                                                                                     \
        hipError_t e__ = (call);                                                             \
        if (e__ != hipSuccess) return set_error(AVD_ELAUNCH, "%s: %s", #call, hipGetErrorString(e__)); \
    } while (0)

struct AuxState { hipStream_t aux = nullptr; hipEvent_t fork = nullptr, join = nullptr; };
static std::mutex g_aux_mu;
static std::map<std::pair<int, hipStream_t>, AuxState> g_aux_map;
static int ensure_aux(hipStream_t st, AuxState& out) {
    int dev = 0;
    AVD_HIP(hipGetDevice(&dev));
    std::lock_guard<std::mutex> lk(g_aux_mu);
    AuxState& a = g_aux_map[{dev, st}];
    if (!a.aux) {
        AVD_HIP(hipStreamCreateWithFlags(&a.aux, hipStreamNonBlocking));
        AVD_HIP(hipEventCreateWithFlags(&a.fork, hipEventDisableTiming));
        AVD_HIP(hipEventCreateWithFlags(&a.join, hipEventDisableTiming));
    }
    out = a;
    return AVD_OK;
}

struct StepPlan {
    int64_t x2, tok, core, head, eps, ss, total;
    int N, D;
    int64_t rows;
};
static int plan_step(const avd_step_desc* s, StepPlan& p) {
    AVD_REQUIRE(s && s->core && s->head, AVD_EINVAL, "step: null descriptor");
    if (int rc = check_embed(&s->embed)) return rc;
    if (int rc = check_core(s->core)) return rc;
    const avd_embed_desc& e = s->embed;
    AVD_REQUIRE(e.d == s->core->d && s->head->d_in == e.d, AVD_EINVAL, "step: width mismatch between embed/core/head");
    p.N = e.Nt + e.Np;
    p.D = embed_tok_dim(&e);
    AVD_REQUIRE(s->head->d_out == p.D, AVD_EINVAL, "step: head d_out %d != token dim %d", s->head->d_out, p.D);
    p.rows = (int64_t)2 * e.B * e.Nt;
    p.x2 = align_up((int64_t)2 * e.B * p.N * e.d * 4);
    p.tok = align_up(embed_ws_floats(&e) * 4);
    const int64_t halves = 2 * core_ws_bytes(s->core, e.B, p.N), whole = core_ws_bytes(s->core, 2 * e.B, p.N);
    p.core = halves > whole ? halves : whole;
    const int64_t head_halves = 2 * head_ws_bytes(s->head, p.rows / 2), head_whole = head_ws_bytes(s->head, p.rows);
    p.head = head_halves > head_whole ? head_halves : head_whole;
    p.eps = align_up(p.rows * p.D * 4);
    p.ss = align_up((int64_t)2 * e.B * p.N * 4);
    p.total = p.x2 + p.tok + p.core + p.head + p.ss + p.eps;
    return AVD_OK;
}

struct StepWs {
// ... 26 lines not shown

extern "C" int avd_abi_version(void) { return AVD_ABI_VERSION; }
extern "C" const char* avd_last_error(void) { return g_err; }

constexpr int kNoExcept = INT_MIN;
struct TuneKey { const char* key; const char* env; int* var; int lo, hi; bool boolean; int except = kNoExcept; };
static const TuneKey kTuneKeys[] = {
    {"s3_tile", "AVD_S3_TILE", &g_s3_tile, INT_MIN, INT_MAX, false},
    {"s3_m16", "AVD_S3_M16", &g_s3_m16, INT_MIN, INT_MAX, false},
    {"s3_rt", "AVD_S3_RT", &g_s3_rt, INT_MIN, INT_MAX, false},
    {"s3_rt4", "AVD_S3_RT4", &g_s3_rt4, 0, 8, false, 1},
    {"s3_deep4", "AVD_S3_DEEP4", &g_s3_deep4, INT_MIN, INT_MAX, true},
    {"s3_w128", "AVD_S3_W128", &g_s3_w128, INT_MIN, INT_MAX, false},
    {"s3_splitk", "AVD_S3_SPLITK", &g_s3_splitk, 0, kS3SplitKMax, false},
    {"s3_stagger", "AVD_S3_STAGGER", &g_s3_stagger, INT_MIN, INT_MAX, false},
    {"cfg_rows", "AVD_CFG_ROWS", &g_cfg_rows, INT_MIN, INT_MAX, true},
    {"vae_lat", "AVD_VAE_LAT", &g_vae_lat, INT_MIN, INT_MAX, true},
    {"vae_fold", "AVD_VAE_FOLD", &g_vae_fold, INT_MIN, INT_MAX, true},
    {"codec_mfma", "AVD_CODEC_MFMA", &g_codec_mfma, INT_MIN, INT_MAX, true},
    {"s3_sn", "AVD_S3_SN", &g_s3_sn, INT_MIN, INT_MAX, false},
    {"s3_super4", "AVD_S3_SUPER4", &g_s3_super4, INT_MIN, INT_MAX, false},
    {"s3_super8", "AVD_S3_SUPER8", &g_s3_super8, INT_MIN, INT_MAX, false},
    {"attn_pipe", "AVD_ATTN_PIPE", &g_attn_pipe, INT_MIN, INT_MAX, false},
    {"attn_m16", "AVD_ATTN_M16", &g_attn_m16, INT_MIN, INT_MAX, false},
    {"core_trim", "AVD_CORE_TRIM", &g_core_trim, INT_MIN, INT_MAX, true},
    {"mlp_fused", "AVD_MLP_FUSED", &g_mlp_fused, INT_MIN, INT_MAX, false},
    {"gemm_tile", "AVD_GEMM_TILE", &g_gemm_force_tile, INT_MIN, INT_MAX, false},
    {"gemm_stages", "AVD_GEMM_STAGES", &g_gemm_stages, INT_MIN, INT_MAX, false},
    {"gemm_splitk", "AVD_GEMM_SPLITK", &g_gemm_splitk, 0, kGemmSplitKMax, false},
    {"s3_min_rows", "AVD_S3_MIN_ROWS", &g_s3_min_rows, INT_MIN, INT_MAX, false},
    {"no_fold", "AVD_NO_FOLD", &g_no_fold, INT_MIN, INT_MAX, true},
};
static void tune_store(const TuneKey& t, int64_t value) { *t.var = t.boolean ? value != 0 : (int)value; }
[[maybe_unused]] static const bool g_tune_env_applied = [] {
    for (const TuneKey& t : kTuneKeys)
        if (const char* e = getenv(t.env)) {
            const long long v = atoll(e);
            tune_store(t, v < t.lo ? t.lo : v > t.hi ? t.hi : v);
        }
    return true;
}();

extern "C" int avd_tune_set(const char* key, int64_t value) {
    AVD_REQUIRE(key, AVD_EINVAL, "tune_set: null key");
    for (const TuneKey& t : kTuneKeys) {
        if (strcmp(key, t.key)) continue;
        AVD_REQUIRE(value >= t.lo && value <= t.hi && value != t.except, AVD_EINVAL, "tune_set: %s does not take %lld", key, (long long)value);
        tune_store(t, value);
        return AVD_OK;
    }
    return set_error(AVD_EINVAL, "tune_set: unknown key '%s'", key);
}

extern "C" int avd_device_arch(char* buf, int buflen) {
    AVD_REQUIRE(buf && buflen > 0, AVD_EINVAL, "device_arch: bad buffer");
    hipDeviceProp_t prop;
    int dev = 0;
    hipError_t e = hipGetDevice(&dev);
    if (e != hipSuccess) return set_error(AVD_ELAUNCH, "hipGetDevice: %s", hipGetErrorString(e));
    e = hipGetDeviceProperties(&prop, dev);
    if (e != hipSuccess) return set_error(AVD_ELAUNCH, "hipGetDeviceProperties: %s", hipGetErrorString(e));
    strncpy(buf, prop.gcnArchName, buflen - 1);
    buf[buflen - 1] = 0;
    return AVD_OK;
}

extern "C" int64_t avd_core_workspace_bytes(const avd_core_weights* w, int B, int N) {
    if (!w || B <= 0 || N <= 0) return -1;
    return core_ws_bytes(w, B, N);
}
extern "C" int avd_core_forward_f32(const avd_core_weights* w, const float* x, float* y, int B, int N, int out_row0,
                                    int n_out_rows, const uint8_t* key_padding_mask, void* workspace, int64_t workspace_bytes,
                                    avd_stream_t stream) {
    return core_forward(w, x, y, B, N, out_row0, n_out_rows, key_padding_mask, workspace, workspace_bytes,
                        static_cast<hipStream_t>(stream));
}

extern "C" int64_t avd_head_workspace_bytes(const avd_head_weights* w, int64_t rows) {
    if (!w || rows < 0) return -1;
    return head_ws_bytes(w, rows);
}
extern "C" int avd_head_forward_f32(const avd_head_weights* w, const float* h, int64_t ldh, int64_t seg_rows,
                                    int64_t seg_stride, int64_t rows, float* out, void* workspace,
                                    int64_t workspace_bytes, avd_stream_t stream) {
    return head_forward(w, h, RowMap{ldh, seg_rows, seg_stride}, rows, out, workspace, workspace_bytes,
                        static_cast<hipStream_t>(stream));
}

extern "C" int64_t avd_embed_workspace_floats(const avd_embed_desc* e) {
    if (check_embed(e)) return -1;
    return embed_ws_floats(e);
}
extern "C" int avd_embed_cfg_pair_f32(const avd_embed_desc* desc, const float* z_target, const float* Wt,
                                      const float* bt, const int64_t* t_now, const float* Xp, float* tok_ws, float* X2,
                                      avd_stream_t stream) {
    return embed_cfg_pair(desc, z_target, Wt, bt, t_now, Xp, tok_ws, X2, static_cast<hipStream_t>(stream));
}

extern "C" int avd_embed_cond_f32(const avd_embed_desc* desc, const float* z_target, const float* Wt, const float* bt,
                                  const int64_t* t_now, const float* Xp, float* tok_ws, float* X1, float* ss, avd_stream_t stream) {
    return embed_cfg_pair(desc, z_target, Wt, bt, t_now, Xp, tok_ws, X1, static_cast<hipStream_t>(stream), ss, true);
}

extern "C" int64_t avd_step_workspace_bytes(const avd_step_desc* s) {
    StepPlan p;
    if (plan_step(s, p)) return -1;
    return p.total;
}

static int denoise_step(const avd_step_desc* s, const avd_noise_key* key, const float* z, const float* Xp, const int64_t* t_now,
                        const int64_t* t_prev, const float* noise, float* z_out, void* workspace, int64_t workspace_bytes,
                        avd_stream_t stream, const int64_t* t_last = nullptr, float* x0_hist = nullptr,
                        const avd_latent_guide* guide = nullptr, const avd_cfg_control* ctl = nullptr, int canvas_hop = 0,
                        int guide_hop = 0) {
    StepWs ws;
    if (int rc = open_step(s, z, z_out, t_now, t_prev, workspace, workspace_bytes, ws)) return rc;
    auto& [p, X2, tok, core_ws, head_ws, ssx, eps2] = ws;
    hipStream_t st = static_cast<hipStream_t>(stream);
    const avd_embed_desc& e = s->embed;
    const bool have_ss = !e.temb_add;

    if (int rc = embed_cfg_pair(&e, z, s->adapt_w, s->adapt_b, t_now, Xp, tok, X2, st, ssx)) return rc;
    const int row0 = e.target_first ? 0 : e.Np;
    const RowMap hm{e.d, e.Nt, (int64_t)p.N * e.d};
    if (!s->split_streams) {
        if (int rc = core_forward(s->core, X2, X2, 2 * e.B, p.N, row0, e.Nt, nullptr, core_ws, p.core, st, have_ss ? ssx : nullptr)) return rc;
        if (int rc = head_forward(s->head, X2 + (int64_t)row0 * e.d, hm, p.rows, eps2, head_ws, p.head, st)) return rc;
    } else {
        AuxState ax;
        if (int rc = ensure_aux(st, ax)) return rc;
        hipStream_t g_aux = ax.aux;
        hipEvent_t g_fork = ax.fork, g_join = ax.join;
        const int64_t half_rows = (int64_t)e.B * p.N * e.d;
        const int64_t hc = p.core / 2, hh = p.head / 2;
        AVD_HIP(hipEventRecord(g_fork, st));
        AVD_HIP(hipStreamWaitEvent(g_aux, g_fork, 0));
        struct TwoStreams {
            TwoStreams(int64_t rows, int64_t head_rows) { t_s3_two_streams = true; t_step_rows = rows; t_step_head_rows = head_rows; }
            ~TwoStreams() { t_s3_two_streams = false; t_step_rows = 0; t_step_head_rows = 0; }
        } two_streams_scope((int64_t)2 * e.B * p.N, p.rows);
        for (int half = 0; half < 2; ++half) {
            hipStream_t hs = half ? g_aux : st;
            float* xh = X2 + half * half_rows;
            if (int rc = core_forward(s->core, xh, xh, e.B, p.N, row0, e.Nt, nullptr, static_cast<char*>(core_ws) + half * hc, hc, hs,
                                      have_ss ? ssx + (int64_t)half * e.B * p.N : nullptr)) return rc;
            if (int rc = head_forward(s->head, xh + (int64_t)row0 * e.d, hm, p.rows / 2, eps2 + half * (p.rows / 2) * p.D,
                                      static_cast<char*>(head_ws) + half * hh, hh, hs)) return rc;
        }
        AVD_HIP(hipEventRecord(g_join, g_aux));
        AVD_HIP(hipStreamWaitEvent(st, g_join, 0));
    }
    if (e.target_kind == 0)
        return cfg_unpatch_ddim_f32(eps2, z, t_now, t_prev, s->alpha_bar, s->T_train, s->guidance, s->eta, noise, z_out,
                                    e.B, e.C, e.T, e.H, e.W, e.p0, e.p1, e.p2, st, key, t_last, x0_hist, guide, ctl, canvas_hop,
                                    guide_hop);
    return cfg_untoken_ddim_audio_f32(eps2, z, t_now, t_prev, s->alpha_bar, s->T_train, s->guidance, s->eta, noise, z_out,
                                      e.B, e.C, e.T, e.p0, e.p1, st, key, t_last, x0_hist, guide, ctl, canvas_hop, guide_hop);
}

static int denoise_step_cond(const avd_step_desc* s, const avd_noise_key* key, const float* z, const float* Xp, const int64_t* t_now,
                             const int64_t* t_prev, const float* noise, float* z_out, void* workspace, int64_t workspace_bytes,
                             avd_stream_t stream, const int64_t* t_last, float* x0_hist, const avd_latent_guide* guide,
                             int canvas_hop = 0, int guide_hop = 0) {
    StepWs ws;
    if (int rc = open_step(s, z, z_out, t_now, t_prev, workspace, workspace_bytes, ws)) return rc;
    auto& [p, X1, tok, core_ws, head_ws, ssx, eps1] = ws;
    hipStream_t st = static_cast<hipStream_t>(stream);
    const avd_embed_desc& e = s->embed;
    const bool have_ss = !e.temb_add;

    if (int rc = embed_cfg_pair(&e, z, s->adapt_w, s->adapt_b, t_now, Xp, tok, X1, st, ssx, true)) return rc;
    const int row0 = e.target_first ? 0 : e.Np;
    const RowMap hm{e.d, e.Nt, (int64_t)p.N * e.d};
    if (int rc = core_forward(s->core, X1, X1, e.B, p.N, row0, e.Nt, nullptr, core_ws, p.core / 2, st, have_ss ? ssx : nullptr)) return rc;
    if (int rc = head_forward(s->head, X1 + (int64_t)row0 * e.d, hm, p.rows / 2, eps1, head_ws, p.head / 2, st)) return rc;
    if (e.target_kind == 0)
        return eps_unpatch_ddim_f32(eps1, z, t_now, t_prev, s->alpha_bar, s->T_train, s->eta, noise, z_out, e.B, e.C, e.T, e.H, e.W, e.p0,
                                    e.p1, e.p2, st, key, t_last, x0_hist, guide, canvas_hop, guide_hop);
// ... 171 lines not shown
```

multimodal_diffusion_amd/csrc/gemm_bf16x3.hip:

```cpp
#include "avd_common.h"
#include "s3_common.h"

#include <stdlib.h>
#include <optional>
#include <type_traits>

namespace avd {


template <bool F16>
__global__ __launch_bounds__(256) void split3_kernel(const float* __restrict__ x, RowMap xm, unsigned char* __restrict__ out,
                                                     int64_t rows, int64_t rows_pad, int K, float s, float* __restrict__ ss) {
    const int64_t i = (int64_t)blockIdx.x * 256 + threadIdx.x;
    const int per_row = K >> 3;
    if (i >= rows_pad * per_row) return;
    const int64_t r = i / per_row;
    const int k = (int)(i % per_row) * 8;
    float v[8] = {0.f, 0.f, 0.f, 0.f, 0.f, 0.f, 0.f, 0.f};
    if (r < rows) {
        const float* xr = x + xm.off(r) + k;
        *reinterpret_cast<f32x4*>(v) = *reinterpret_cast<const f32x4*>(xr);
        *reinterpret_cast<f32x4*>(v + 4) = *reinterpret_cast<const f32x4*>(xr + 4);
    }
    if constexpr (F16) store_split8_h2(out, r, k, K, v, s);
// ... 134 lines not shown
                    if constexpr (F16) store_split8_h2(g.C3, m, n, g.N, v, g.c_scale);
                    else store_split8(g.C3, m, n, g.N, v);
                }
            }
        } else {
            const int cr = lane >> 4, cc = (lane & 15) * 4;
            const int n = nbase + cc;
            f32x4 bv = {0.f, 0.f, 0.f, 0.f};
            if (g.bias) bv = *reinterpret_cast<const f32x4*>(g.bias + n);
            float* cptr = g.C + (m0 + cr) * g.N + n;
            const float* rptr = EPI == S3_EPI_RES ? g.R + (m0 + cr) * g.N + n : nullptr;
#pragma unroll
            for (int c0 = 0; c0 < 16; c0 += 8) {
                f32x4 rv[8];
                if constexpr (EPI == S3_EPI_RES) {
#pragma unroll
                    for (int u = 0; u < 8; ++u)
                        rv[u] = m0 + cr + (c0 + u) * 4 < g.M ? *reinterpret_cast<const f32x4*>(rptr + (int64_t)(c0 + u) * 4 * g.N)
                                                            : f32x4{0.f, 0.f, 0.f, 0.f};
                }
#pragma unroll
                for (int u = 0; u < 8; ++u) {
                    const int it = c0 + u;
                    f32x4 v = *reinterpret_cast<const f32x4*>(slab + (cr + it * 4) * CLD + cc);
                    if constexpr (F16) v *= g.ab_inv;
                    v += bv;
                    if constexpr (EPI == S3_EPI_RES) v += rv[u];
                    if (m0 + cr + it * 4 < g.M) *reinterpret_cast<f32x4*>(cptr + (int64_t)it * 4 * g.N) = v;
                }
            }
        }
    }
}

template <int EPI, bool F16>
__device__ __forceinline__ void s3_epilogue_img_t(const S3Args& g, f32x16 (&acc)[4][2], int64_t mwave0, int nbase, int lane, bool big) {
    const int l31 = lane & 31, hi = lane >> 5;
    float bv[2][2][8];
#pragma unroll
    for (int j = 0; j < 2; ++j)
#pragma unroll
        for (int cg = 0; cg < 2; ++cg) {
            const float* bp = g.bias + nbase + 32 * j + 8 * (2 * cg + hi);
            *reinterpret_cast<f32x4*>(bv[j][cg]) = *reinterpret_cast<const f32x4*>(bp);
            *reinterpret_cast<f32x4*>(bv[j][cg] + 4) = *reinterpret_cast<const f32x4*>(bp + 4);
        }
    [[maybe_unused]] float mul = 1.0f;
    [[maybe_unused]] float ssq[4] = {0.f, 0.f, 0.f, 0.f};
    [[maybe_unused]] int64_t qbase = 0;
    if constexpr (EPI == S3_EPI_QKV3) {
        const int dmodel = g.heads * 64;
        const int part = nbase / dmodel, head = (nbase % dmodel) >> 6;
        mul = part == 0 ? g.qscale : 1.0f;
        qbase = (((int64_t)part * (g.M / g.tokN)) * g.heads + head) * (int64_t)g.tokNpad * QKV3_ROWB;
    }
#pragma unroll
    for (int i = 0; i < 4; ++i) {
        const int64_t m = mwave0 + 32 * i + l31;
        float rinv = 1.0f;
        if (EPI != S3_EPI_RES_IMG && g.ss_in != nullptr && m < g.M) {
            const int nc = g.K >> 6;
            const float* sp = g.ss_in + m * nc;
            float ssum = 0.f;
            if (nc == 8) {
                const f32x4 p0 = *reinterpret_cast<const f32x4*>(sp), p1 = *reinterpret_cast<const f32x4*>(sp + 4);
                const f32x4 t = p0 + p1;
                ssum = (t[0] + t[1]) + (t[2] + t[3]);
            } else {
                for (int c = 0; c < nc; ++c) ssum += sp[c];
            }
            rinv = 1.0f / (sqrtf(ssum) / g.ss_sqrt_d + g.ss_eps);
        }
        [[maybe_unused]] unsigned char* qrow = nullptr;
        [[maybe_unused]] int qsw = 0;
        if constexpr (EPI == S3_EPI_QKV3) {
            const unsigned b = (unsigned)m / (unsigned)g.tokN, tok = (unsigned)m - b * (unsigned)g.tokN;
            const int dmodel = g.heads * 64;
            qrow = g.C3 + qbase + ((int64_t)b * g.heads * g.tokNpad + tok) * QKV3_ROWB;
            qsw = qkv3_swizzle(nbase / dmodel, (int)tok);
        }
#pragma unroll
        for (int j = 0; j < 2; ++j)
#pragma unroll
            for (int cg = 0; cg < 2; ++cg) {
                float v[8];
#pragma unroll
                for (int e = 0; e < 4; ++e) {
                    const auto sw = __builtin_amdgcn_permlane32_swap(__float_as_uint(acc[i][j][8 * cg + e]), __float_as_uint(acc[i][j][8 * cg + 4 + e]),
                                                                     false, false);
                    v[e] = __uint_as_float(sw[0]);
                    v[4 + e] = __uint_as_float(sw[1]);
                }
                if constexpr (EPI == S3_EPI_QKV3) {
#pragma unroll
                    for (int e = 0; e < 8; ++e) v[e] = fmaf(F16 ? v[e] * g.ab_inv : v[e], rinv, bv[j][cg][e]) * mul;
                    if (S3_ROW_OK(m)) {
                        const int c = 4 * j + 2 * cg + hi;
                        unsigned char* dst = qrow + ((c ^ qsw) << 4);
                        if constexpr (F16) {
                            u32x4 Hh, Lo;
                            split8_h2(v, g.c_scale, Hh, Lo);
                            *reinterpret_cast<u32x4*>(dst) = Hh;
                            *reinterpret_cast<u32x4*>(dst + 128) = Lo;
                        } else {
                            u32x4 Hh, Mi, Lo;
                            if (big) split8<true>(v, Hh, Mi, Lo);
                            else split8<false>(v, Hh, Mi, Lo);
                            *reinterpret_cast<u32x4*>(dst) = Hh;
                            *reinterpret_cast<u32x4*>(dst + 128) = Mi;
                            *reinterpret_cast<u32x4*>(dst + 256) = Lo;
                        }
                    }
                } else if constexpr (EPI == S3_EPI_RES_IMG) {
                    const int n = nbase + 32 * j + 8 * (2 * cg + hi);
                    if (m < g.M) {
                        const float* rp = g.R + m * g.N + n;
                        const f32x4 r0 = *reinterpret_cast<const f32x4*>(rp), r1 = *reinterpret_cast<const f32x4*>(rp + 4);
#pragma unroll
                        for (int e = 0; e < 8; ++e) v[e] = ((F16 ? v[e] * g.ab_inv : v[e]) + bv[j][cg][e]) + (e < 4 ? r0[e] : r1[e - 4]);
                        float* cp = g.C + m * g.N + n;
                        *reinterpret_cast<f32x4*>(cp) = f32x4{v[0], v[1], v[2], v[3]};
                        *reinterpret_cast<f32x4*>(cp + 4) = f32x4{v[4], v[5], v[6], v[7]};
                        ssq[i] += ((v[0] * v[0] + v[1] * v[1]) + (v[2] * v[2] + v[3] * v[3])) + ((v[4] * v[4] + v[5] * v[5]) + (v[6] * v[6] + v[7] * v[7]));
                        if constexpr (F16) store_split8_h2(g.C3, m, n, g.N, v, g.c_scale);
                        else if (big) store_split8<true>(g.C3, m, n, g.N, v);
                        else store_split8<false>(g.C3, m, n, g.N, v);
                    }
                } else {
                    const int n = nbase + 32 * j + 8 * (2 * cg + hi);
// ... 1039 lines not shown
int g_s3_rt = 0;
template <int EPI, int WAVES, int RT = 8, int NSTK = 0>
static int launch_s3w16(const S3Args& g, hipStream_t st) {
    using Cf = S3Cfg<6, WAVES>;
    constexpr S3Geom ge{WAVES == 8 || RT < 8 ? 32 * RT : Cf::BM, Cf::BN, NSTK ? NSTK * Cf::STAGE : Cf::LDS, WAVES * 64, WAVES == 4, 48};
    static LdsAttr attr;
    static const int tag = prof_tag_id("gemm_bf16x3_m16_kernel<%d, %d, %d, %d>", EPI, WAVES, RT, NSTK);
    return s3_launch(gemm_bf16x3_m16_kernel<EPI, WAVES, RT, NSTK>, attr, ge, tag, "gemm_bf16x3 (16x16x32)", g, st);
}

int g_s3_w128 = 1;
template <int EPI, int RT>
static int launch_s3w128(const S3Args& g, hipStream_t st) {
    constexpr S3Geom ge{32 * RT, 256, 3 * 6 * 256 * 32, 256, false, -1};
    static LdsAttr attr;
    static const int tag = prof_tag_id("gemm_bf16x3_w128_kernel<%d, %d>", EPI, RT);
    return s3_launch(gemm_bf16x3_w128_kernel<EPI, RT>, attr, ge, tag, "gemm_bf16x3 (128x128 wave tile)", g, st);
}

int g_s3_rt4 = 0;
static int s3_rt4_for(int64_t M, int N, int rt_min) {
    if (g_s3_rt4 >= 2 && g_s3_rt4 <= 8) return g_s3_rt4 > rt_min ? g_s3_rt4 : rt_min;
    const int64_t cu = s3_cu_or_256(), nbn = N / 128;
    int best = 8;
    int64_t cost8 = 0, cbest = 0;
    for (int rt = 8; rt >= rt_min; --rt) {
        const int64_t blocks = (M + 32 * rt - 1) / (32 * rt) * nbn, cost = (blocks + cu - 1) / cu * (rt + 3);
        if (rt == 8) cost8 = cbest = cost;
        else if (cost < cbest) { cbest = cost; best = rt; }
    }
    return cbest * 100 <= cost8 * 94 ? best : 8;
}
static int s3_rt8_for(int64_t M, int N) {
    const int64_t cu = s3_cu_or_256(), nbn = N / 256;
    const int64_t g8 = ((M + 255) / 256 * nbn + cu - 1) / cu * 8, g7 = ((M + 223) / 224 * nbn + cu - 1) / cu * 7;
    const int64_t g6 = ((M + 191) / 192 * nbn + cu - 1) / cu * 6;
    if (g_s3_w128 && (g_s3_rt == 6 || (g_s3_rt == 0 && g6 < g7 && g6 < g8))) return 6;
    return g_s3_rt == 7 || (g_s3_rt != 8 && g7 < g8) ? 7 : 8;
}
int g_s3_deep4 = 1;
static bool s3_deep4_for(int64_t M, int N, int rt) {
    return g_s3_deep4 != 0 && (M + 32 * rt - 1) / (32 * rt) * (N / 128) <= s3_cu_or_256();
}

template <int LO, int HI, class F>
static std::optional<int> s3_with_rt(int rt, bool hi_is_default, F&& f) {
    if (rt == LO || (LO == HI && hi_is_default)) return f(std::integral_constant<int, LO>{});
    if constexpr (LO < HI) return s3_with_rt<LO + 1, HI>(rt, hi_is_default, f);
    else return std::nullopt;
}

template <int EPI, int TERMS>
static int launch_s3t(const S3Args& a, hipStream_t st) {
    if constexpr (TERMS == 6 && EPI != S3_EPI_RES_NORM) {
        if (g_s3_m16) {
            if (s3_tile_for(EPI, a.M, a.N)) {
                if constexpr (EPI == S3_EPI_BIAS || EPI == S3_EPI_SPLIT || EPI == S3_EPI_RES_IMG) {
                    constexpr int E2 = EPI == S3_EPI_BIAS ? (int)S3_EPI_BIAS_REG : (int)EPI;
                    const int rt = s3_rt4_for(a.M, a.N, 2);
                    if ((EPI == S3_EPI_RES_IMG || (a.bias && a.N % 128 == 0)) && s3_deep4_for(a.M, a.N, rt))
                        return *s3_with_rt<2, 8>(rt, true, [&](auto r) { return launch_s3w16<E2, 4, r(), 4>(a, st); });
                    if constexpr (EPI == S3_EPI_RES_IMG) {
                        if (const auto rc = s3_with_rt<2, 4>(rt, false, [&](auto r) { return launch_s3w16<EPI, 4, r()>(a, st); })) return *rc;
                    }
                }
                if constexpr (EPI == S3_EPI_GELU_SPLIT || EPI == S3_EPI_QKV3 || EPI == S3_EPI_RES_IMG) {
                    const int rt = s3_rt4_for(a.M, a.N, 5);
                    if (const auto rc = s3_with_rt<5, 7>(rt, false, [&](auto r) { return launch_s3w16<EPI, 4, r()>(a, st); })) return *rc;
                }
                return launch_s3w16<EPI, 4>(a, st);
            }
            constexpr bool RI = EPI == S3_EPI_RES_IMG;
            const int rt = RI ? s3_rt8_for(a.M, a.N) : 8;
            if constexpr (RI || EPI == S3_EPI_GELU_SPLIT || EPI == S3_EPI_SPLIT || EPI == S3_EPI_QKV3) {
                if (g_s3_w128) return *s3_with_rt<RI ? 6 : 7, 8>(rt, true, [&](auto r) { return launch_s3w128<EPI, r()>(a, st); });
            }
            if constexpr (RI) {
                if (rt == 7) return launch_s3w16<EPI, 8, 7>(a, st);
            }
            return launch_s3w16<EPI, 8>(a, st);
        }
    }
    if constexpr (EPI == S3_EPI_RES_NORM) {
        if constexpr (TERMS == 3) return launch_s3w<EPI, 3, 8>(a, st);
        else AVD_REQUIRE(false, AVD_EUNSUPPORTED, "gemm_bf16x3: the residual + RMSNorm epilogue exists for f16x2 images only");
    } else {
        return s3_tile_for(EPI, a.M, a.N) ? launch_s3w<EPI, TERMS, 4>(a, st) : launch_s3w<EPI, TERMS, 8>(a, st);
    }
}

template <int EPI>
static int launch_s3(const S3Args& a, hipStream_t st) {
    switch (a.terms) {
        case 0: case 6: return launch_s3t<EPI, 6>(a, st);
        case 9: return launch_s3t<EPI, 9>(a, st);
        case 1: return launch_s3t<EPI, 1>(a, st);
        case 3: return launch_s3t<EPI, 3>(a, st);
        default: return set_error(AVD_EINVAL, "gemm_bf16x3: terms must be 6 (default), 9 (strict), 1 (plain bf16) or 3 (f16x2), got %d", a.terms);
    }
}

bool gemm_bf16x3_resmap_supported(int terms) { return (terms == 0 || terms == 6) && g_s3_m16 != 0; }

static S3Args s3_args(const void* A3, const void* W3, int64_t M, int N, int K, int terms) {
    S3Args a{};
    a.A = static_cast<const unsigned char*>(A3);
    a.W = static_cast<const unsigned char*>(W3);
    a.M = M, a.N = N, a.K = K, a.terms = terms;
    a.ab_inv = a.c_scale = a.ss_sqrt_d = 1.0f;
    return a;
}

int gemm_bf16x3(const void* A3, const void* W3, const float* bias, const float* R, float* C, void* C3, int64_t M, int N, int K,
                int act, int terms, hipStream_t st, float ab_scale, float c_scale, const float* ss_in, float eps, float* ss_out,
                const float* gamma, int r_seg, int r_stride) {
    AVD_REQUIRE(r_seg == 0 || (r_seg > 0 && r_stride >= r_seg && ss_out && gemm_bf16x3_resmap_supported(terms) && M < (1ll << 31)), AVD_EUNSUPPORTED,
                "gemm_bf16x3: a residual row map needs the fp32 + image residual epilogue of the six-term 16x16x32 kernels");
    AVD_REQUIRE(A3 && W3 && (C || C3), AVD_EINVAL, "gemm_bf16x3: null pointer");
    AVD_REQUIRE(!gamma || (gemm_bf16x3_rownorm_supported(N, terms) && C && C3 && R && bias && !ss_in && !ss_out && act == AVD_ACT_NONE && aligned16(gamma)),
                AVD_EUNSUPPORTED, "gemm_bf16x3: the residual + RMSNorm epilogue needs N == 512, f16x2 images, fp32 and image outputs, bias and residual");
    AVD_REQUIRE(!ss_in || (C3 && !C && K % 64 == 0), AVD_EUNSUPPORTED, "gemm_bf16x3: a folded norm needs an image output and K %% 64 == 0");
    AVD_REQUIRE(!ss_out || (C && C3 && R && bias && N % 64 == 0 && act == AVD_ACT_NONE && terms != 3), AVD_EUNSUPPORTED,
                "gemm_bf16x3: sums of squares are written by the fp32 + image residual epilogue only (bf16 planes)");
    AVD_REQUIRE(scale_ok(ab_scale) && scale_ok(c_scale), AVD_EINVAL, "gemm_bf16x3: image scales must be positive and finite");
    AVD_REQUIRE(gemm_bf16x3_supported(M, N, K), AVD_EUNSUPPORTED, "gemm_bf16x3: need N %% 256 == 0 and K %% 16 == 0 (M=%lld N=%d K=%d)",
                (long long)M, N, K);
    AVD_REQUIRE(aligned16(A3) && aligned16(W3) && aligned16(C) && aligned16(C3) && aligned16(bias) && aligned16(R), AVD_EUNSUPPORTED,
                "gemm_bf16x3: pointers must be 16-byte aligned");
    S3Args a = s3_args(A3, W3, M, N, K, terms);
    a.bias = bias, a.R = R, a.C = C, a.C3 = static_cast<unsigned char*>(C3);
    a.ab_inv = 1.0f / ab_scale, a.c_scale = c_scale;
    a.ss_in = ss_in, a.ss_out = ss_out, a.ss_sqrt_d = (float)sqrt((double)K), a.ss_eps = eps;
    a.gamma = gamma, a.r_seg = r_seg, a.r_stride = r_stride;
    if (gamma) {
        a.ss_sqrt_d = (float)sqrt((double)N);
        return launch_s3<S3_EPI_RES_NORM>(a, st);
    }
    if (C && C3) {
        AVD_REQUIRE(ss_out, AVD_EUNSUPPORTED, "gemm_bf16x3: fp32 and image output together imply the residual + sums-of-squares epilogue");
        return launch_s3<S3_EPI_RES_IMG>(a, st);
    }
    if (C3) {
        AVD_REQUIRE((act == AVD_ACT_GELU || act == AVD_ACT_NONE) && !R && bias, AVD_EUNSUPPORTED,
                    "gemm_bf16x3: image output implies bias, act NONE or GELU, no residual");
        return act == AVD_ACT_GELU ? launch_s3<S3_EPI_GELU_SPLIT>(a, st) : launch_s3<S3_EPI_SPLIT>(a, st);
    }
    AVD_REQUIRE(act == AVD_ACT_NONE, AVD_EUNSUPPORTED, "gemm_bf16x3: fp32 output supports act NONE only");
    if (R) {
        if ((terms == 0 || terms == 6) && g_s3_m16 && bias) return launch_s3<S3_EPI_RES_IMG>(a, st);
        return launch_s3<S3_EPI_RES>(a, st);
    }
    return launch_s3<S3_EPI_BIAS>(a, st);
}

template <bool IMG>
__global__ __launch_bounds__(256) void splitk_reduce_kernel(const float* __restrict__ part, int ns, const float* __restrict__ bias,
                                                            const float* R, float* C, unsigned char* __restrict__ C3,
                                                            float* __restrict__ ss, int64_t M, int N) {
    const int64_t i = (int64_t)blockIdx.x * 256 + threadIdx.x;
    const int per_row = N >> 3;
    const int64_t m = i / per_row;
    const int n = (int)(i % per_row) * 8;
    float v[8] = {0.f, 0.f, 0.f, 0.f, 0.f, 0.f, 0.f, 0.f};
    if (m < M) {
        const int64_t o = m * N + n;
        *reinterpret_cast<f32x4*>(v) = *reinterpret_cast<const f32x4*>(part + o);
        *reinterpret_cast<f32x4*>(v + 4) = *reinterpret_cast<const f32x4*>(part + o + 4);
        for (int z = 1; z < ns; ++z) {
            const float* pz = part + (int64_t)z * M * N + o;
            const f32x4 a = *reinterpret_cast<const f32x4*>(pz), b = *reinterpret_cast<const f32x4*>(pz + 4);
#pragma unroll
            for (int e = 0; e < 4; ++e) { v[e] += a[e]; v[4 + e] += b[e]; }
        }
        const f32x4 b0 = *reinterpret_cast<const f32x4*>(bias + n), b1 = *reinterpret_cast<const f32x4*>(bias + n + 4);
        const f32x4 r0 = *reinterpret_cast<const f32x4*>(R + o), r1 = *reinterpret_cast<const f32x4*>(R + o + 4);
#pragma unroll
        for (int e = 0; e < 4; ++e) { v[e] = (v[e] + b0[e]) + r0[e]; v[4 + e] = (v[4 + e] + b1[e]) + r1[e]; }
        *reinterpret_cast<f32x4*>(C + o) = f32x4{v[0], v[1], v[2], v[3]};
        *reinterpret_cast<f32x4*>(C + o + 4) = f32x4{v[4], v[5], v[6], v[7]};
        if constexpr (IMG) store_split8<true>(C3, m, n, N, v);
    }
    if constexpr (IMG) {
        float q = ((v[0] * v[0] + v[1] * v[1]) + (v[2] * v[2] + v[3] * v[3])) + ((v[4] * v[4] + v[5] * v[5]) + (v[6] * v[6] + v[7] * v[7]));
        q += __shfl_xor(q, 1, 64);
        q += __shfl_xor(q, 2, 64);
        q += __shfl_xor(q, 4, 64);
        if ((threadIdx.x & 7) == 0 && m < M) ss[m * (N >> 6) + (n >> 6)] = q;
    }
}

int g_s3_splitk = 4;
static bool splitk_shape_ok(int64_t M, int N, int K) {
    if (N % 128 || K % 32 || K / 2 < 512) return false;
    return (M + 255) / 256 * (N / 128) * 2 <= (int64_t)s3_cu_count();
}
int gemm_bf16x3_splitk_slices(int64_t M, int N, int K, int terms) {
    if (g_s3_splitk < 2 || terms == 3 || ((terms == 0 || terms == 6) && g_s3_m16) || !splitk_shape_ok(M, N, K)) return 0;
    const int64_t cu = s3_cu_count(), blocks = (M + 255) / 256 * (N / 128);
    int ns = 1;
    while (ns * 2 <= g_s3_splitk && blocks * ns * 2 <= cu && K % (32 * ns) == 0 && K / (ns * 2) >= 512) ns *= 2;
    return ns >= 2 ? ns : 0;
}
int64_t gemm_bf16x3_splitk_ws_floats(int64_t M, int N, int ns) { return (int64_t)ns * M * N; }
int64_t gemm_bf16x3_splitk_ws_max_floats(int64_t M, int N, int K) {
    return splitk_shape_ok(M, N, K) ? gemm_bf16x3_splitk_ws_floats(M, N, kS3SplitKMax) : 0;
}

int gemm_bf16x3_splitk(const void* A3, const void* W3, const float* bias, const float* R, float* C, void* C3, float* ss, int64_t M, int N,
                       int K, int terms, int ns, float* part, hipStream_t st) {
    AVD_REQUIRE(A3 && W3 && bias && R && C && part && ns >= 2, AVD_EINVAL, "gemm_bf16x3_splitk: null pointer");
    AVD_REQUIRE((C3 != nullptr) == (ss != nullptr), AVD_EINVAL, "gemm_bf16x3_splitk: the image and the sums of squares come together");
    AVD_REQUIRE(K % (16 * ns) == 0 && N % 128 == 0 && N % 64 == 0 && gemm_bf16x3_supported(M, N, K / ns), AVD_EUNSUPPORTED,
                "gemm_bf16x3_splitk: shape (M=%lld N=%d K=%d slices=%d)", (long long)M, N, K, ns);
    AVD_REQUIRE(aligned16(A3) && aligned16(W3) && aligned16(C) && aligned16(C3) && aligned16(bias) && aligned16(R) && aligned16(part),
                AVD_EUNSUPPORTED, "gemm_bf16x3_splitk: pointers must be 16-byte aligned");
    S3Args a = s3_args(A3, W3, M, N, K / ns, terms);
    a.C = part;
    int rc;
    switch (terms) {
        case 1: rc = launch_s3w<S3_EPI_BIAS, 1, 4>(a, st, ns); break;
        case 9: rc = launch_s3w<S3_EPI_BIAS, 9, 4>(a, st, ns); break;
        case 0: case 6: rc = launch_s3w<S3_EPI_BIAS, 6, 4>(a, st, ns); break;
        default: AVD_REQUIRE(false, AVD_EUNSUPPORTED, "gemm_bf16x3_splitk: bf16-plane modes only (terms %d)", terms);
    }
    if (rc) return rc;
    const int64_t threads = M * (N >> 3);
    static const int tag = prof_tag_id("splitk_reduce_kernel");
    ProfScope prof(tag, (double)M * N * 4.0 * (ns + 2) + (C3 ? (double)M * N * 6.0 : 0.0), st);
    with_bool(C3 != nullptr, [&](auto img) {
        hipLaunchKernelGGL(splitk_reduce_kernel<img()>, dim3((unsigned)((threads + 255) / 256)), dim3(256), 0, st, part, ns, bias, R, C,
                           static_cast<unsigned char*>(C3), ss, M, N);
    });
    AVD_CHECK_LAUNCH("splitk_reduce");
    return AVD_OK;
}

int gemm_bf16x3_qkv3(const void* A3, const void* W3, const float* bias, void* img, int64_t M, int tokens, int heads, int K, float qscale,
                     int terms, hipStream_t st, float ab_scale, float c_scale, const float* ss_in, float eps) {
    AVD_REQUIRE(!ss_in || K % 64 == 0, AVD_EUNSUPPORTED, "gemm_bf16x3_qkv3: a folded norm needs K %% 64 == 0");
    AVD_REQUIRE(A3 && W3 && bias && img, AVD_EINVAL, "gemm_bf16x3_qkv3: null pointer");
    AVD_REQUIRE(scale_ok(ab_scale) && scale_ok(c_scale), AVD_EINVAL, "gemm_bf16x3_qkv3: image scales must be positive and finite");
    const int N = 3 * heads * 64;
    AVD_REQUIRE(tokens > 0 && heads > 0 && M > 0 && M % tokens == 0, AVD_EINVAL, "gemm_bf16x3_qkv3: rows %lld not a multiple of tokens %d",
                (long long)M, tokens);
    AVD_REQUIRE(M < (1ll << 31) - 256, AVD_EUNSUPPORTED, "gemm_bf16x3_qkv3: more than 2^31 rows");
    AVD_REQUIRE(gemm_bf16x3_supported(M, N, K), AVD_EUNSUPPORTED, "gemm_bf16x3_qkv3: need 3*heads*64 %% 256 == 0 and K %% 16 == 0");
    AVD_REQUIRE(aligned16(A3) && aligned16(W3) && aligned16(bias) && aligned16(img), AVD_EUNSUPPORTED, "gemm_bf16x3_qkv3: alignment");
    S3Args a = s3_args(A3, W3, M, N, K, terms);
    a.bias = bias, a.C3 = static_cast<unsigned char*>(img);
    a.tokN = tokens, a.tokNpad = qkv3_npad(tokens), a.heads = heads, a.qscale = qscale;
    a.ab_inv = 1.0f / ab_scale, a.c_scale = c_scale;
    a.ss_in = ss_in, a.ss_sqrt_d = (float)sqrt((double)K), a.ss_eps = eps;
    return launch_s3<S3_EPI_QKV3>(a, st);
}

}

using namespace avd;

extern "C" int64_t avd_split3_bytes(int64_t rows, int K) {
    if (rows <= 0 || K <= 0 || K % 16) return -1;
    return split3_bytes(rows, K);
}
extern "C" int avd_split3_f32(const float* x, void* out, int64_t rows, int K, avd_stream_t stream) {
    return split3_f32(x, K, out, rows, K, static_cast<hipStream_t>(stream));
}
extern "C" int avd_rmsnorm_split3_f32(const float* x, const float* scale, void* out, int64_t rows, int d, float eps,
                                      avd_stream_t stream) {
    return rmsnorm_split3_f32(x, scale, out, rows, d, eps, static_cast<hipStream_t>(stream));
}
extern "C" int avd_gemm_bf16x3_f32(const void* A3, const void* W3, const float* bias, const float* residual, float* C, void* C3,
                                   int64_t M, int N, int K, int act, int terms, avd_stream_t stream) {
    return gemm_bf16x3(A3, W3, bias, residual, C, C3, M, N, K, act, terms, static_cast<hipStream_t>(stream));
}
extern "C" int avd_gemm_bf16x3_qkv3_f32(const void* A3, const void* W3, const float* bias, void* qkv3, int64_t M, int tokens, int heads,
                                        int K, float qscale, int terms, avd_stream_t stream) {
    return gemm_bf16x3_qkv3(A3, W3, bias, qkv3, M, tokens, heads, K, qscale, terms, static_cast<hipStream_t>(stream));
}

extern "C" int avd_split_f16x2_f32(const float* x, void* out, int64_t rows, int K, float scale, avd_stream_t stream) {
    AVD_REQUIRE(scale > 0.f, AVD_EINVAL, "avd_split_f16x2_f32: scale must be positive");
    return split3_f32(x, K, out, rows, K, static_cast<hipStream_t>(stream), scale);
}
extern "C" int avd_rmsnorm_split_f16x2_f32(const float* x, const float* gamma, void* out, int64_t rows, int d, float eps, float scale,
                                           avd_stream_t stream) {
    AVD_REQUIRE(scale > 0.f, AVD_EINVAL, "avd_rmsnorm_split_f16x2_f32: scale must be positive");
    return rmsnorm_split3_f32(x, gamma, out, rows, d, eps, static_cast<hipStream_t>(stream), scale);
}
extern "C" int avd_gemm_f16x2_f32(const void* A2, const void* W2, const float* bias, const float* residual, float* C, void* C2, int64_t M,
                                  int N, int K, int act, float ab_scale, float c_scale, avd_stream_t stream) {
    return gemm_bf16x3(A2, W2, bias, residual, C, C2, M, N, K, act, 3, static_cast<hipStream_t>(stream), ab_scale, c_scale);
}
extern "C" int avd_gemm_f16x2_qkv_f32(const void* A2, const void* W2, const float* bias, void* qkv, int64_t M, int tokens, int heads, int K,
                                      float qscale, float ab_scale, float qkv_scale, avd_stream_t stream) {
    return gemm_bf16x3_qkv3(A2, W2, bias, qkv, M, tokens, heads, K, qscale, 3, static_cast<hipStream_t>(stream), ab_scale, qkv_scale);
}
```

multimodal_diffusion_amd/csrc/s3_common.h:

```cpp
#pragma once
#include "avd_common.h"

namespace avd {

#define AVD_LDS_PTR(p) ((__attribute__((address_space(3))) void*)(p))
#define AVD_GLB_PTR(p) ((const __attribute__((address_space(1))) void*)(p))

enum { S3_EPI_BIAS = 0, S3_EPI_RES = 2, S3_EPI_GELU_SPLIT = 3, S3_EPI_QKV3 = 4, S3_EPI_SPLIT = 5, S3_EPI_RES_IMG = 6, S3_EPI_RES_NORM = 7,
       S3_EPI_BIAS_REG = 8 };

struct S3Args {
    const unsigned char* A;
    const unsigned char* W;
    const float* bias;
    const float* R;
    float* C;
    unsigned char* C3;
    int64_t M;
    int N, K, nbn, sm, sn;
    int tokN, tokNpad, heads;
    float qscale;
    int stagger;
    int first_gen;
    int terms;
    float ab_inv, c_scale;
    const float* ss_in;
    float* ss_out;
    float ss_sqrt_d, ss_eps;
    const float* gamma;
    int r_seg, r_stride;
#ifdef AVD_S3_STAMPS
    unsigned long long* dbg;
#endif
};

#ifdef AVD_S3_STAMPS
#define S3_T() __builtin_amdgcn_s_memtime()
#define S3_RT() __builtin_amdgcn_s_memrealtime()
#define S3_DBG(i, v) do { if (threadIdx.x == 0) g.dbg[(size_t)blockIdx.x * 16 + (i)] = (v); } while (0)
#else
#define S3_T() 0ull
#define S3_RT() 0ull
#define S3_DBG(i, v) do { } while (0)
#endif

__device__ __forceinline__ void s3_block_of(const S3Args& g, int nbm, int& bm, int& bn) {
    const int b = blockIdx.x, nwg = gridDim.x, q = nwg >> 3, r = nwg & 7, x = b & 7;
    const int wg = (x < r ? x * (q + 1) : r * (q + 1) + (x - r) * q) + (b >> 3);
    const int per_row = g.sm * g.nbn;
    const int srow = wg / per_row, rem = wg - srow * per_row;
    const int left = nbm - srow * g.sm, h = left < g.sm ? left : g.sm;
    const int per_st = h * g.sn;
    const int sc = rem / per_st, rem2 = rem - sc * per_st;
    bm = srow * g.sm + rem2 / g.sn;
    bn = sc * g.sn + rem2 % g.sn;
}

template <int N> __device__ __forceinline__ void wait_vm() {
    static_assert(N >= 0 && N < 64, "vmcnt range");
    __builtin_amdgcn_s_waitcnt(0x0f70 | (N & 15) | ((N >> 4) << 14));
}

#ifdef AVD_LAB_NOSTORE
#define S3_ROW_OK(m) ((m) < g.M && __float_as_uint(v[0]) == 0x7fc12345u)
#else
#define S3_ROW_OK(m) ((m) < g.M)
#endif

typedef float f32x4t __attribute__((ext_vector_type(4)));

__device__ __forceinline__ f32x4t mma16x16(bf16x8 a, bf16x8 b, f32x4t c) { return __builtin_amdgcn_mfma_f32_16x16x32_bf16(a, b, c, 0, 0, 0); }

template <int EPI, int RT = 8>
__device__ __forceinline__ void s3_epilogue_img16(const S3Args& g, f32x4t (&acc)[8][4], int64_t mwave0, int nbase, int lane) {
    const int l15 = lane & 15, kq = lane >> 4;
    bool big = EPI == S3_EPI_RES_IMG;
    if constexpr (EPI != S3_EPI_RES_IMG && EPI != S3_EPI_BIAS_REG) {
        float amax = 0.f;
#pragma unroll
        for (int i = 0; i < 8; ++i) {
            float a = 0.f;
#pragma unroll
            for (int j = 0; j < 4; ++j)
#pragma unroll
                for (int r = 0; r < 4; ++r) a = fmaxf(a, fabsf(acc[i][j][r]));
            if (mwave0 + 16 * i + l15 < g.M) amax = fmaxf(amax, a);
        }
        float bmax = 0.f;
#pragma unroll
        for (int e = 0; e < 64; e += 4) {
            const f32x4 b4 = *reinterpret_cast<const f32x4*>(g.bias + nbase + e);
            bmax = fmaxf(fmaxf(bmax, fmaxf(fabsf(b4[0]), fabsf(b4[1]))), fmaxf(fabsf(b4[2]), fabsf(b4[3])));
        }
        big = __any(!(amax < 1.2676506e30f) || !(bmax < 1.2676506e30f) || !(fabsf(g.qscale) < 1.0e6f));
    }
    float bv[4][8];
#pragma unroll
    for (int j = 0; j < 4; ++j) {
        const float* bp = g.bias + nbase + 16 * j + 8 * (kq >> 1);
        *reinterpret_cast<f32x4*>(bv[j]) = *reinterpret_cast<const f32x4*>(bp);
        *reinterpret_cast<f32x4*>(bv[j] + 4) = *reinterpret_cast<const f32x4*>(bp + 4);
    }
    [[maybe_unused]] float mul = 1.0f;
    [[maybe_unused]] int64_t qbase = 0;
    if constexpr (EPI == S3_EPI_QKV3) {
        const int dmodel = g.heads * 64;
        const int part = nbase / dmodel, head = (nbase % dmodel) >> 6;
        mul = part == 0 ? g.qscale : 1.0f;
        qbase = (((int64_t)part * (g.M / g.tokN)) * g.heads + head) * (int64_t)g.tokNpad * QKV3_ROWB;
    }
#pragma unroll
    for (int ip = 0; ip < 4; ++ip) {
        const int tile = 2 * ip + (kq & 1);
        const int64_t m = (RT == 8 || tile < RT) ? mwave0 + 16 * tile + l15 : g.M;
        float rinv = 1.0f;
        if (EPI != S3_EPI_RES_IMG && EPI != S3_EPI_BIAS_REG && g.ss_in != nullptr && m < g.M) {
            const int nc = g.K >> 6;
            const float* sp = g.ss_in + m * nc;
            float ssum = 0.f;
            if (nc == 8) {
                const f32x4 p0 = *reinterpret_cast<const f32x4*>(sp), p1 = *reinterpret_cast<const f32x4*>(sp + 4);
                const f32x4 t = p0 + p1;
                ssum = (t[0] + t[1]) + (t[2] + t[3]);
            } else {
                for (int c = 0; c < nc; ++c) ssum += sp[c];
            }
            rinv = 1.0f / (sqrtf(ssum) / g.ss_sqrt_d + g.ss_eps);
        }
        [[maybe_unused]] unsigned char* qrow = nullptr;
        [[maybe_unused]] int qsw = 0;
        if constexpr (EPI == S3_EPI_QKV3) {
            const unsigned b = (unsigned)m / (unsigned)g.tokN, tok = (unsigned)m - b * (unsigned)g.tokN;
            qrow = g.C3 + qbase + ((int64_t)b * g.heads * g.tokNpad + tok) * QKV3_ROWB;
            qsw = qkv3_swizzle(nbase / (g.heads * 64), (int)tok);
        }
        [[maybe_unused]] float ssq = 0.f;
        [[maybe_unused]] int64_t rrow = m;
        if constexpr (EPI == S3_EPI_RES_IMG) {
            if (g.r_seg > 0 && m < g.M) {
                const unsigned sgi = (unsigned)m / (unsigned)g.r_seg;
                rrow = (int64_t)sgi * g.r_stride + ((unsigned)m - sgi * (unsigned)g.r_seg);
            }
        }
#pragma unroll
        for (int j = 0; j < 4; ++j) {
            float v[8];
#pragma unroll
            for (int r = 0; r < 4; ++r) {
                const auto sw = __builtin_amdgcn_permlane16_swap(__float_as_uint(acc[2 * ip][j][r]), __float_as_uint(acc[2 * ip + 1][j][r]), false, false);
                v[r] = __uint_as_float(sw[0]);
                v[4 + r] = __uint_as_float(sw[1]);
            }
            const int n = nbase + 16 * j + 8 * (kq >> 1);
            if constexpr (EPI == S3_EPI_QKV3) {
#pragma unroll
                for (int e = 0; e < 8; ++e) v[e] = fmaf(v[e], rinv, bv[j][e]) * mul;
                if (S3_ROW_OK(m)) {
                    const int c = 2 * j + (kq >> 1);
                    unsigned char* dst = qrow + ((c ^ qsw) << 4);
                    u32x4 Hh, Mi, Lo;
                    if (big) split8<true>(v, Hh, Mi, Lo);
                    else split8<false>(v, Hh, Mi, Lo);
                    *reinterpret_cast<u32x4*>(dst) = Hh;
                    *reinterpret_cast<u32x4*>(dst + 128) = Mi;
                    *reinterpret_cast<u32x4*>(dst + 256) = Lo;
                }
            } else if constexpr (EPI == S3_EPI_BIAS_REG) {
                if (S3_ROW_OK(m)) {
#pragma unroll
                    for (int e = 0; e < 8; ++e) v[e] += bv[j][e];
                    float* cp = g.C + m * g.N + n;
                    *reinterpret_cast<f32x4*>(cp) = f32x4{v[0], v[1], v[2], v[3]};
                    *reinterpret_cast<f32x4*>(cp + 4) = f32x4{v[4], v[5], v[6], v[7]};
                }
            } else if constexpr (EPI == S3_EPI_RES_IMG) {
                if (S3_ROW_OK(m)) {
                    const float* rp = g.R + rrow * g.N + n;
                    const f32x4 r0 = *reinterpret_cast<const f32x4*>(rp), r1 = *reinterpret_cast<const f32x4*>(rp + 4);
#pragma unroll
                    for (int e = 0; e < 8; ++e) v[e] = (v[e] + bv[j][e]) + (e < 4 ? r0[e] : r1[e - 4]);
                    float* cp = g.C + m * g.N + n;
                    *reinterpret_cast<f32x4*>(cp) = f32x4{v[0], v[1], v[2], v[3]};
                    *reinterpret_cast<f32x4*>(cp + 4) = f32x4{v[4], v[5], v[6], v[7]};
                    ssq += ((v[0] * v[0] + v[1] * v[1]) + (v[2] * v[2] + v[3] * v[3])) + ((v[4] * v[4] + v[5] * v[5]) + (v[6] * v[6] + v[7] * v[7]));
                    if (g.C3) store_split8<true>(g.C3, m, n, g.N, v);
                }
            } else {
#pragma unroll
                for (int e = 0; e < 8; ++e) {
                    const float t = fmaf(v[e], rinv, bv[j][e]);
                    v[e] = EPI == S3_EPI_GELU_SPLIT ? gelu_erf(t) : t;
                }
                if (S3_ROW_OK(m)) {
                    if (big) store_split8<true>(g.C3, m, n, g.N, v);
// ... 13 lines not shown
```

multimodal_diffusion_amd/csrc/tokens.hip:

```cpp
#include "avd_common.h"

#include <stdlib.h>
#include <type_traits>

namespace avd {

__global__ void temb_kernel(const int64_t* __restrict__ t, const float* __restrict__ freqs, float* __restrict__ out,
                            int B, int dim, float neg_log_mp) {
    const int half = dim >> 1;
    const int i = blockIdx.x * blockDim.x + threadIdx.x;
    if (i >= B * dim) return;
    const int b = i / dim, c = i % dim;
    float v = 0.f;
    if (c < 2 * half) {
        const int k = c < half ? c : c - half;
        const float f = freqs ? freqs[k] : expf(neg_log_mp * (float)k / (float)half);
        const float a = (float)t[b] * f;
        v = c < half ? cosf(a) : sinf(a);
    }
    out[i] = v;
}

int temb_f32(const int64_t* t, const float* freqs, float* out, int B, int dim, float max_period, hipStream_t st) {
    AVD_REQUIRE(t && out, AVD_EINVAL, "timestep_embedding: null pointer");
// ... 1292 lines not shown
    UpdateKeys k;
    const CanvasDims cv{Ca, F, canvas_hop, 1};
    const CanvasDims gcv{Ca, F, guide_hop, 1};
    if (int rc = check_fused_update("eps_untoken_ddim_audio", a, (int64_t)Ca * F, key, t_last, x0_hist, guide, nullptr, k,
                                    canvas_hop ? &cv : nullptr, guide_hop ? &gcv : nullptr)) return rc;
    const AudioGeom ag{Ca, F, len, stride, audio_na(F, len, stride)};
    with_update_pack(k, true, [&](auto... p) { launch_untoken(a, ag, st, p...); });
    AVD_CHECK_LAUNCH("eps_untoken_ddim_audio");
    return AVD_OK;
}

__global__ __launch_bounds__(256) void assemble_kernel(float* __restrict__ X2, const float* __restrict__ temb,
                                                       const float* __restrict__ Xp, int B, int N, int d, int tdim,
                                                       int Nt, int Np, int target_first, int64_t total4) {
    const int64_t i = (int64_t)blockIdx.x * 256 + threadIdx.x;
    if (i >= total4) return;
    const int d4 = d >> 2;
    const int col = (int)(i % d4) * 4;
    const int64_t row = i / d4;
    const int n = (int)(row % N);
    const int bb = (int)(row / N);
    const int half = bb >= B, b = half ? bb - B : bb;
    const int t0 = target_first ? 0 : Np;
    const bool is_t = n >= t0 && n < t0 + Nt;
    f32x4 v;
    if (is_t) {
        if (col >= d - tdim) {
            v = *reinterpret_cast<const f32x4*>(temb + (int64_t)b * tdim + (col - (d - tdim)));
        } else {
            if (!half) return;
            v = *reinterpret_cast<const f32x4*>(X2 + ((int64_t)b * N + n) * d + col);
        }
    } else {
        const int np = target_first ? n - Nt : n;
        v = half ? f32x4{0.f, 0.f, 0.f, 0.f} : *reinterpret_cast<const f32x4*>(Xp + ((int64_t)b * Np + np) * d + col);
    }
    *reinterpret_cast<f32x4*>(X2 + row * d + col) = v;
}

int assemble_f32(float* X2, const float* temb, const float* Xp, int B, int N, int d, int tdim, int Nt, int Np,
                 int target_first, hipStream_t st) {
    const int64_t total4 = (int64_t)2 * B * N * (d >> 2);
    static const int tag = prof_tag_id("assemble_kernel");
    ProfScope prof(tag, 4.0 * (2.0 * B * N * d + (double)B * Nt * (d - tdim) + (double)B * Np * d), st);
    hipLaunchKernelGGL(assemble_kernel, dim3((unsigned)((total4 + 255) / 256)), dim3(256), 0, st, X2, temb, Xp, B, N, d,
                       tdim, Nt, Np, target_first, total4);
    AVD_CHECK_LAUNCH("assemble");
    return AVD_OK;
}

__global__ __launch_bounds__(256) void assemble_rows_kernel(float* __restrict__ X2, const int64_t* __restrict__ t_now,
                                                            const float* __restrict__ freqs, const float* __restrict__ Xp,
                                                            float* __restrict__ ss, int B, int N, int d, int tdim, int Nt, int Np,
                                                            int target_first, float neg_log_mp) {
    const int lane = threadIdx.x & 63;
    const int64_t row = (int64_t)blockIdx.x * 4 + (threadIdx.x >> 6);
    if (row >= (int64_t)2 * B * N) return;
    const int n = (int)(row % N);
    const int bb = (int)(row / N);
    const int half = bb >= B, b = half ? bb - B : bb;
    const int t0 = target_first ? 0 : Np;
    const bool is_t = n >= t0 && n < t0 + Nt;
    const int da = d - tdim, th = tdim >> 1;
    const float tf = is_t ? (float)t_now[b] : 0.f;
    float acc = 0.f;
    for (int col = lane * 4; col < d; col += 256) {
        f32x4 v;
        bool store = true;
        if (is_t) {
            if (col >= da) {
#pragma unroll
                for (int e = 0; e < 4; ++e) {
                    const int c = col - da + e;
                    float x = 0.f;
                    if (c < 2 * th) {
                        const int k = c < th ? c : c - th;
                        const float f = freqs ? freqs[k] : expf(neg_log_mp * (float)k / (float)th);
                        const float a = tf * f;
                        x = c < th ? cosf(a) : sinf(a);
                    }
                    v[e] = x;
                }
            } else {
                v = *reinterpret_cast<const f32x4*>(X2 + ((int64_t)b * N + n) * d + col);
                store = half != 0;
            }
        } else {
            const int np = target_first ? n - Nt : n;
            v = half ? f32x4{0.f, 0.f, 0.f, 0.f} : *reinterpret_cast<const f32x4*>(Xp + ((int64_t)b * Np + np) * d + col);
        }
        if (store) *reinterpret_cast<f32x4*>(X2 + row * d + col) = v;
        acc += v[0] * v[0] + v[1] * v[1] + v[2] * v[2] + v[3] * v[3];
    }
    acc = wave_sum(acc);
    if (ss && lane == 0) ss[row] = acc;
}

int assemble_rows_f32(float* X2, const int64_t* t_now, const float* freqs, const float* Xp, float* ss, int B, int N, int d, int tdim,
                      int Nt, int Np, int target_first, float max_period, hipStream_t st) {
    const int64_t rows = (int64_t)2 * B * N;
    static const int tag = prof_tag_id("assemble_rows_kernel");
    ProfScope prof(tag, 4.0 * (2.0 * B * N * d + (double)B * Nt * (d - tdim) + (double)B * Np * d), st);
    hipLaunchKernelGGL(assemble_rows_kernel, dim3((unsigned)((rows + 3) / 4)), dim3(256), 0, st, X2, t_now, freqs, Xp, ss, B, N, d, tdim,
                       Nt, Np, target_first, -(float)log((double)max_period));
    AVD_CHECK_LAUNCH("assemble_rows");
    return AVD_OK;
}

__global__ __launch_bounds__(256) void assemble_cond_kernel(float* __restrict__ X1, const float* __restrict__ temb,
                                                            const float* __restrict__ Xp, int B, int N, int d, int tdim, int Nt,
                                                            int Np, int target_first, int64_t total4) {
    const int64_t i = (int64_t)blockIdx.x * 256 + threadIdx.x;
    if (i >= total4) return;
    const int d4 = d >> 2;
    const int col = (int)(i % d4) * 4;
    const int64_t row = i / d4;
    const int n = (int)(row % N);
    const int b = (int)(row / N);
    const int t0 = target_first ? 0 : Np;
    const bool is_t = n >= t0 && n < t0 + Nt;
    f32x4 v;
    if (is_t) {
        if (col < d - tdim) return;
        v = *reinterpret_cast<const f32x4*>(temb + (int64_t)b * tdim + (col - (d - tdim)));
    } else {
        const int np = target_first ? n - Nt : n;
        v = *reinterpret_cast<const f32x4*>(Xp + ((int64_t)b * Np + np) * d + col);
    }
    *reinterpret_cast<f32x4*>(X1 + row * d + col) = v;
}

int assemble_cond_f32(float* X1, const float* temb, const float* Xp, int B, int N, int d, int tdim, int Nt, int Np, int target_first,
                      hipStream_t st) {
    const int64_t total4 = (int64_t)B * N * (d >> 2);
    static const int tag = prof_tag_id("assemble_cond_kernel");
    ProfScope prof(tag, 4.0 * 2.0 * ((double)B * Nt * tdim + (double)B * Np * d), st);
    hipLaunchKernelGGL(assemble_cond_kernel, dim3((unsigned)((total4 + 255) / 256)), dim3(256), 0, st, X1, temb, Xp, B, N, d, tdim, Nt, Np,
                       target_first, total4);
    AVD_CHECK_LAUNCH("assemble_cond");
    return AVD_OK;
}

__global__ __launch_bounds__(256) void assemble_rows_cond_kernel(float* __restrict__ X1, const int64_t* __restrict__ t_now,
                                                                 const float* __restrict__ freqs, const float* __restrict__ Xp,
                                                                 float* __restrict__ ss, int B, int N, int d, int tdim, int Nt, int Np,
                                                                 int target_first, float neg_log_mp) {
    const int lane = threadIdx.x & 63;
    const int64_t row = (int64_t)blockIdx.x * 4 + (threadIdx.x >> 6);
    if (row >= (int64_t)B * N) return;
    const int n = (int)(row % N);
    const int b = (int)(row / N);
    const int t0 = target_first ? 0 : Np;
    const bool is_t = n >= t0 && n < t0 + Nt;
    const int da = d - tdim, th = tdim >> 1;
    const float tf = is_t ? (float)t_now[b] : 0.f;
    float acc = 0.f;
    for (int col = lane * 4; col < d; col += 256) {
        f32x4 v;
// ... 191 lines not shown
```

Before: 114.8 steps/s.

## Deduplicate identical null-prompt rows in the CFG unconditional half

In the null half of the stacked CFG batch, every prompt token is zero, so all of those rows stay identical through each per-token layer. The change keeps only the target rows plus one prompt row per null sample, using a two-segment row map (RowSegs) threaded through assemble, the QKV GEMM epilogue, residual mapping and the attention output stores. A new replicate kernel copies that single prompt row's K/V into the remaining key slots so the attention softmax still sees every key. This trims GEMM and attention query work on the null half, at the cost of an extra small kernel and more complex row indexing in several kernels.

```diff
diff --git a/include/avdiff_hip.h b/include/avdiff_hip.h
--- a/include/avdiff_hip.h
+++ b/include/avdiff_hip.h
@@ -28,6 +28,7 @@
 const char* avd_last_error(void);
 int         avd_device_arch(char* buf, int buflen);
 int         avd_tune_set(const char* key, int64_t value);
+int         avd_cfg_dedup_set(int on);
 
 int avd_rmsnorm_f32(const float* x, const float* scale, float* y, int64_t rows, int d, float eps,
                     avd_stream_t stream);
diff --git a/multimodal_diffusion_amd/_lib.py b/multimodal_diffusion_amd/_lib.py
--- a/multimodal_diffusion_amd/_lib.py
+++ b/multimodal_diffusion_amd/_lib.py
@@ -107,6 +107,7 @@
     "avd_gemm_bias_act_f32": (_I, [_P, _L, _P, _P, _P, _L, _P, _L, _L, _I, _I, _I, _P]),
     "avd_gemm_rmsfold_f32": (_I, [_P, _P, _P, _P, _P, _L, _I, _I, _I, _P, _I, _F, _P, _P]),
     "avd_tune_set": (_I, [C.c_char_p, _L]),
+    "avd_cfg_dedup_set": (_I, [_I]),
     "avd_attn_fwd_f32": (_I, [_P, _P, _I, _I, _I, _I, _F, _I, _P, _P]),
     "avd_layernorm_act_f32": (_I, [_P, _P, _P, _P, _L, _I, _F, _I, _P]),
     "avd_timestep_embedding_f32": (_I, [_P, _P, _P, _I, _I, _F, _P]),
diff --git a/multimodal_diffusion_amd/csrc/attn_bf16x3.hip b/multimodal_diffusion_amd/csrc/attn_bf16x3.hip
--- a/multimodal_diffusion_amd/csrc/attn_bf16x3.hip
+++ b/multimodal_diffusion_amd/csrc/attn_bf16x3.hip
@@ -23,8 +23,8 @@
 
 template <bool SPLIT_OUT, int TERMS>
 __global__ __launch_bounds__(A3_NW * 64, 2) void attn_bf16x3_kernel(const unsigned char* __restrict__ img, float* __restrict__ out,
-                                                                    int Bt, int N, int Npad, int H, int n_query, int nqb,
-                                                                    float s_inv2, float v_inv, float o_scale, int out_tok) {
+                                                                    int Bt, int N, int Npad, int H, int n_query_max, int nqb,
+                                                                    float s_inv2, float v_inv, float o_scale, RowSegs oseg) {
     constexpr int NW = A3_NW, ROWB = QKV3_ROWB;
     constexpr bool F16 = TERMS == 3;
     constexpr int NPL = s3_planes(TERMS);
@@ -40,6 +40,8 @@
         h = (w / nqb) % H;
         b = w / (nqb * H);
     }
+    const int seg_tok = oseg.tok[b < oseg.samples[0] ? 0 : 1], n_query = n_query_max < seg_tok ? n_query_max : seg_tok;
+    if (qb * (A3_NW * 32) >= n_query) return;
     const int tid = threadIdx.x, lane = tid & 63, wave = tid >> 6;
     const int l31 = lane & 31, hi = lane >> 5;
     const int64_t hstride = (int64_t)Npad * ROWB;
@@ -226,12 +228,12 @@
                 v[4 + e] = hi ? ch[c + 1][e] : recv;
             }
             if (q_row < n_query) {
-                if constexpr (F16) store_split8_h2(o3, (int64_t)b * out_tok + q_row, h * A3_DH + 8 * (c + hi), d, v, o_scale);
-                else store_split8(o3, (int64_t)b * out_tok + q_row, h * A3_DH + 8 * (c + hi), d, v);
+                if constexpr (F16) store_split8_h2(o3, oseg.row(b, q_row), h * A3_DH + 8 * (c + hi), d, v, o_scale);
+                else store_split8(o3, oseg.row(b, q_row), h * A3_DH + 8 * (c + hi), d, v);
             }
         }
     } else if (q_row < n_query) {
-        float* dst = out + ((int64_t)b * out_tok + q_row) * d + h * A3_DH + 4 * hi;
+        float* dst = out + (oseg.row(b, q_row)) * d + h * A3_DH + 4 * hi;
 #pragma unroll
         for (int g4 = 0; g4 < 4; ++g4) {
             f32x4 a = {o0[4 * g4] * inv, o0[4 * g4 + 1] * inv, o0[4 * g4 + 2] * inv, o0[4 * g4 + 3] * inv};
@@ -250,8 +252,8 @@
 
 template <bool SPLIT_OUT, int TERMS>
 __global__ __launch_bounds__(A3_NW * 64, 2) void attn_bf16x3_pipe_kernel(const unsigned char* __restrict__ img, float* __restrict__ out,
-                                                                         int Bt, int N, int Npad, int H, int n_query, int nqb,
-                                                                         float s_inv2, float v_inv, float o_scale, int out_tok) {
+                                                                         int Bt, int N, int Npad, int H, int n_query_max, int nqb,
+                                                                         float s_inv2, float v_inv, float o_scale, RowSegs oseg) {
     constexpr int NW = A3_NW, ROWB = QKV3_ROWB;
     constexpr bool F16 = TERMS == 3;
     constexpr int NPL = s3_planes(TERMS);
@@ -268,6 +270,8 @@
         h = (w / nqb) % H;
         b = w / (nqb * H);
     }
+    const int seg_tok = oseg.tok[b < oseg.samples[0] ? 0 : 1], n_query = n_query_max < seg_tok ? n_query_max : seg_tok;
+    if (qb * (A3_NW * 32) >= n_query) return;
     const int tid = threadIdx.x, lane = tid & 63;
     const int wave = __builtin_amdgcn_readfirstlane(tid >> 6);
     const int l31 = lane & 31, hi = lane >> 5;
@@ -553,12 +557,12 @@
                 v[4 + e] = hi ? ch[c + 1][e] : recv;
             }
             if (q_row < n_query) {
-                if constexpr (F16) store_split8_h2(o3, (int64_t)b * out_tok + q_row, h * A3_DH + 8 * (c + hi), d, v, o_scale);
-                else store_split8(o3, (int64_t)b * out_tok + q_row, h * A3_DH + 8 * (c + hi), d, v);
+                if constexpr (F16) store_split8_h2(o3, oseg.row(b, q_row), h * A3_DH + 8 * (c + hi), d, v, o_scale);
+                else store_split8(o3, oseg.row(b, q_row), h * A3_DH + 8 * (c + hi), d, v);
             }
         }
     } else if (q_row < n_query) {
-        float* dst = out + ((int64_t)b * out_tok + q_row) * d + h * A3_DH + 4 * hi;
+        float* dst = out + (oseg.row(b, q_row)) * d + h * A3_DH + 4 * hi;
 #pragma unroll
         for (int g4 = 0; g4 < 4; ++g4) {
             f32x4 a = {o0[4 * g4] * inv, o0[4 * g4 + 1] * inv, o0[4 * g4 + 2] * inv, o0[4 * g4 + 3] * inv};
@@ -580,8 +584,8 @@
 
 template <bool SPLIT_OUT, int TERMS>
 __global__ __launch_bounds__(A3_NW * 64, 2) void attn_bf16x3_p16_kernel(const unsigned char* __restrict__ img, float* __restrict__ out,
-                                                                        int Bt, int N, int Npad, int H, int n_query, int nqb,
-                                                                        float s_inv2, float v_inv, float o_scale, int out_tok) {
+                                                                        int Bt, int N, int Npad, int H, int n_query_max, int nqb,
+                                                                        float s_inv2, float v_inv, float o_scale, RowSegs oseg) {
     constexpr int NW = A3_NW, ROWB = QKV3_ROWB;
     constexpr bool F16 = TERMS == 3;
     constexpr int NPL = s3_planes(TERMS);
@@ -598,6 +602,8 @@
         h = (w / nqb) % H;
         b = w / (nqb * H);
     }
+    const int seg_tok = oseg.tok[b < oseg.samples[0] ? 0 : 1], n_query = n_query_max < seg_tok ? n_query_max : seg_tok;
+    if (qb * (A3_NW * 32) >= n_query) return;
     const int tid = threadIdx.x, lane = tid & 63;
     const int wave = __builtin_amdgcn_readfirstlane(tid >> 6);
     const int l15 = lane & 15, kq = lane >> 4;
@@ -906,10 +912,10 @@
         const int col = h * A3_DH + 16 * dt + 8 * (kq >> 1);
         if (q_row < n_query) {
             if constexpr (SPLIT_OUT) {
-                if constexpr (F16) store_split8_h2(o3, (int64_t)b * out_tok + q_row, col, d, v, o_scale);
-                else store_split8(o3, (int64_t)b * out_tok + q_row, col, d, v);
+                if constexpr (F16) store_split8_h2(o3, oseg.row(b, q_row), col, d, v, o_scale);
+                else store_split8(o3, oseg.row(b, q_row), col, d, v);
             } else {
-                float* dst = out + ((int64_t)b * out_tok + q_row) * d + col;
+                float* dst = out + (oseg.row(b, q_row)) * d + col;
                 *reinterpret_cast<f32x4*>(dst) = f32x4{v[0], v[1], v[2], v[3]};
                 *reinterpret_cast<f32x4*>(dst + 4) = f32x4{v[4], v[5], v[6], v[7]};
             }
@@ -921,38 +927,42 @@
 
 template <int TERMS>
 static void attn3_launch(const unsigned char* img, float* out, void* out3, int B, int N, int Npad, int H, int n_query, int nqb, hipStream_t st,
-                         float img_scale, float out_scale, int out_tok) {
+                         float img_scale, float out_scale, const RowSegs& oseg) {
     const float s_inv2 = 1.0f / (img_scale * img_scale), v_inv = 1.0f / img_scale;
     if (g_attn_m16 && (TERMS == 6 || TERMS == 9 || g_attn_m16 == 2)) {
         if (out3)
             hipLaunchKernelGGL((attn_bf16x3_p16_kernel<true, TERMS>), dim3(nqb * H * B), dim3(A3_NW * 64), 0, st, img, static_cast<float*>(out3),
-                               B, N, Npad, H, n_query, nqb, s_inv2, v_inv, out_scale, out_tok);
+                               B, N, Npad, H, n_query, nqb, s_inv2, v_inv, out_scale, oseg);
         else
             hipLaunchKernelGGL((attn_bf16x3_p16_kernel<false, TERMS>), dim3(nqb * H * B), dim3(A3_NW * 64), 0, st, img, out, B, N, Npad, H,
-                               n_query, nqb, s_inv2, v_inv, out_scale, out_tok);
+                               n_query, nqb, s_inv2, v_inv, out_scale, oseg);
         return;
     }
     if (g_attn_pipe == 2 || (g_attn_pipe == 1 && (TERMS == 6 || TERMS == 9))) {
         if (out3)
             hipLaunchKernelGGL((attn_bf16x3_pipe_kernel<true, TERMS>), dim3(nqb * H * B), dim3(A3_NW * 64), 0, st, img, static_cast<float*>(out3),
-                               B, N, Npad, H, n_query, nqb, s_inv2, v_inv, out_scale, out_tok);
+                               B, N, Npad, H, n_query, nqb, s_inv2, v_inv, out_scale, oseg);
         else
             hipLaunchKernelGGL((attn_bf16x3_pipe_kernel<false, TERMS>), dim3(nqb * H * B), dim3(A3_NW * 64), 0, st, img, out, B, N, Npad, H,
-                               n_query, nqb, s_inv2, v_inv, out_scale, out_tok);
+                               n_query, nqb, s_inv2, v_inv, out_scale, oseg);
         return;
     }
     if (out3)
         hipLaunchKernelGGL((attn_bf16x3_kernel<true, TERMS>), dim3(nqb * H * B), dim3(A3_NW * 64), 0, st, img, static_cast<float*>(out3), B, N,
-                           Npad, H, n_query, nqb, s_inv2, v_inv, out_scale, out_tok);
+                           Npad, H, n_query, nqb, s_inv2, v_inv, out_scale, oseg);
     else
         hipLaunchKernelGGL((attn_bf16x3_kernel<false, TERMS>), dim3(nqb * H * B), dim3(A3_NW * 64), 0, st, img, out, B, N, Npad, H, n_query, nqb,
-                           s_inv2, v_inv, out_scale, out_tok);
+                           s_inv2, v_inv, out_scale, oseg);
 }
 
 int attn_bf16x3(const void* qkv3, float* out, void* out3, int B, int N, int H, int n_query, int terms, hipStream_t st, float img_scale,
-                float out_scale, int out_tokens) {
+                float out_scale, int out_tokens, const RowSegs* out_rows) {
     const int out_tok = out_tokens > 0 ? out_tokens : N;
     AVD_REQUIRE(out_tok >= n_query, AVD_EINVAL, "attn_bf16x3: out_tokens=%d < n_query=%d", out_tok, n_query);
+    AVD_REQUIRE(!out_rows || (out_rows->n_samples() == B && out_rows->samples[0] > 0 && out_rows->tok[0] > 0 && out_rows->tok[1] > 0 &&
+                              out_rows->m0 == (int64_t)out_rows->samples[0] * out_rows->tok[0]), AVD_EINVAL,
+                "attn_bf16x3: the output row layout does not hold the batch's %d samples", B);
+    const RowSegs oseg = out_rows ? *out_rows : RowSegs::uniform(B, out_tok);
     AVD_REQUIRE(terms == 0 || terms == 6 || terms == 9 || terms == 1 || terms == 3, AVD_EINVAL, "attn_bf16x3: terms must be 6, 9, 1 or 3, got %d", terms);
     AVD_REQUIRE(img_scale > 0.f && img_scale < __builtin_inff() && out_scale > 0.f && out_scale < __builtin_inff() &&
                     img_scale * img_scale < __builtin_inff(), AVD_EINVAL, "attn_bf16x3: image scales must be positive and finite");
@@ -968,10 +978,10 @@
     ProfScope prof(tag, 4.0 * (double)B * H * (double)n_query * N * A3_DH, st);
     const int Npad = qkv3_npad(N);
     const auto* img = static_cast<const unsigned char*>(qkv3);
-    if (terms == 9) attn3_launch<9>(img, out, out3, B, N, Npad, H, n_query, nqb, st, 1.f, 1.f, out_tok);
-    else if (terms == 1) attn3_launch<1>(img, out, out3, B, N, Npad, H, n_query, nqb, st, 1.f, 1.f, out_tok);
-    else if (terms == 3) attn3_launch<3>(img, out, out3, B, N, Npad, H, n_query, nqb, st, img_scale, out_scale, out_tok);
-    else attn3_launch<6>(img, out, out3, B, N, Npad, H, n_query, nqb, st, 1.f, 1.f, out_tok);
+    if (terms == 9) attn3_launch<9>(img, out, out3, B, N, Npad, H, n_query, nqb, st, 1.f, 1.f, oseg);
+    else if (terms == 1) attn3_launch<1>(img, out, out3, B, N, Npad, H, n_query, nqb, st, 1.f, 1.f, oseg);
+    else if (terms == 3) attn3_launch<3>(img, out, out3, B, N, Npad, H, n_query, nqb, st, img_scale, out_scale, oseg);
+    else attn3_launch<6>(img, out, out3, B, N, Npad, H, n_query, nqb, st, 1.f, 1.f, oseg);
     AVD_CHECK_LAUNCH("attn_bf16x3");
     return AVD_OK;
 }
diff --git a/multimodal_diffusion_amd/csrc/avd_common.h b/multimodal_diffusion_amd/csrc/avd_common.h
--- a/multimodal_diffusion_amd/csrc/avd_common.h
+++ b/multimodal_diffusion_amd/csrc/avd_common.h
@@ -71,6 +71,24 @@
     int64_t stride;
     __host__ __device__ __forceinline__ int64_t off(int64_t r) const {
         return seg > 0 ? (r / seg) * stride + (r % seg) * ld : r * ld;
+    }
+};
+
+struct RowSegs {
+    int64_t m0;
+    int tok[2], samples[2];
+    static RowSegs uniform(int samples, int tok) { return RowSegs{(int64_t)samples * tok, {tok, tok}, {samples, 0}}; }
+    __host__ __device__ __forceinline__ int64_t rows() const { return m0 + (int64_t)samples[1] * tok[1]; }
+    __host__ __device__ __forceinline__ int n_samples() const { return samples[0] + samples[1]; }
+    __host__ __device__ __forceinline__ void locate(int64_t m, int& sample, int& token) const {
+        const bool s1 = m >= m0;
+        const unsigned r = (unsigned)(s1 ? m - m0 : m), t = (unsigned)(s1 ? tok[1] : tok[0]);
+        const unsigned b = r / t;
+        sample = (int)b + (s1 ? samples[0] : 0);
+        token = (int)(r - b * t);
+    }
+    __host__ __device__ __forceinline__ int64_t row(int sample, int token) const {
+        return sample < samples[0] ? (int64_t)sample * tok[0] + token : m0 + (int64_t)(sample - samples[0]) * tok[1] + token;
     }
 };
 
@@ -253,17 +271,18 @@
 extern int g_s3_sn, g_s3_super4, g_s3_super8;
 extern int g_s3_tile;
 extern thread_local bool t_s3_two_streams;
-int gemm_bf16x3_qkv3(const void* A3, const void* W3, const float* bias, void* img, int64_t M, int tokens, int heads, int K, float qscale,
-                     int terms, hipStream_t st, float ab_scale = 1.f, float c_scale = 1.f, const float* ss_in = nullptr, float eps = 0.f);
+int gemm_bf16x3_qkv3(const void* A3, const void* W3, const float* bias, void* img, const RowSegs& seg, int heads, int K, float qscale,
+                     int terms, hipStream_t st, float ab_scale = 1.f, float c_scale = 1.f, const float* ss_in = nullptr, float eps = 0.f,
+                     int64_t plan_rows = 0);
 int64_t qkv3_bytes(int B, int N, int H);
 int64_t attn_fp8_ws_bytes(int B, int N, int H);
 int attn_fp8(const void* qkv3, void* ws, int64_t ws_bytes, float* out, void* out3, int B, int N, int H, int n_query, hipStream_t st,
              int img_terms = 6, float img_scale = 1.f, float out_scale = 1.f);
 int attn_bf16x3(const void* qkv3, float* out, void* out3, int B, int N, int H, int n_query, int terms, hipStream_t st,
-                float img_scale = 1.f, float out_scale = 1.f, int out_tokens = 0);
+                float img_scale = 1.f, float out_scale = 1.f, int out_tokens = 0, const RowSegs* out_rows = nullptr);
 int gemm_bf16x3(const void* A3, const void* W3, const float* bias, const float* R, float* C, void* C3, int64_t M, int N, int K,
                 int act, int terms, hipStream_t st, float ab_scale = 1.f, float c_scale = 1.f, const float* ss_in = nullptr, float eps = 0.f,
-                float* ss_out = nullptr, const float* gamma = nullptr, int r_seg = 0, int r_stride = 0);
+                float* ss_out = nullptr, const float* gamma = nullptr, int r_seg = 0, const RowSegs* r_map = nullptr, int64_t plan_rows = 0);
 bool gemm_bf16x3_resmap_supported(int terms);
 bool gemm_bf16x3_rownorm_supported(int N, int terms);
 extern int g_s3_splitk;
diff --git a/multimodal_diffusion_amd/csrc/composite.hip b/multimodal_diffusion_amd/csrc/composite.hip
--- a/multimodal_diffusion_amd/csrc/composite.hip
+++ b/multimodal_diffusion_amd/csrc/composite.hip
@@ -72,7 +72,8 @@
 int assemble_f32(float* X2, const float* temb, const float* Xp, int B, int N, int d, int tdim, int Nt, int Np,
                  int target_first, hipStream_t st);
 int assemble_rows_f32(float* X2, const int64_t* t_now, const float* freqs, const float* Xp, float* ss, int B, int N, int d, int tdim,
-                      int Nt, int Np, int target_first, float max_period, hipStream_t st);
+                      int Nt, int Np, int target_first, float max_period, hipStream_t st, const RowSegs* short_null = nullptr);
+int qkv3_replicate(void* img, int img_samples, int H, int n_keys, int first_sample, int n_samples, int src, hipStream_t st);
 int cfg_unpatch_ddim_f32(const float* eps2, const float* z, const int64_t* t_now, const int64_t* t_prev,
                          const float* abar, int T_train, float guidance, float eta, const float* noise, float* z_out,
                          int B, int C, int T, int H, int W, int t, int h, int w, hipStream_t st, const avd_noise_key* key = nullptr,
@@ -168,6 +169,12 @@
 static int g_core_trim = 1;
 static int64_t core_trim_floats(const avd_core_weights* w, int B, int N) { return (int64_t)B * N * w->d; }
 
+static int g_cfg_dedup = 1;
+[[maybe_unused]] static const bool g_cfg_dedup_env_applied = [] {
+    if (const char* e = getenv("AVD_CFG_DEDUP")) g_cfg_dedup = atoll(e) != 0;
+    return true;
+}();
+
 static int64_t core_split_wide_bytes(const avd_core_weights* w, int B, int N) {
     const int64_t qkv3 = qkv3_bytes(B, N, w->n_heads), fc1 = split3_bytes((int64_t)B * N, w->mlp_hidden);
     return qkv3 > fc1 ? qkv3 : fc1;
@@ -216,9 +223,15 @@
     return layernorm_act_f32(x, scale, bias, y, M, w->d, w->norm_eps, AVD_ACT_NONE, st);
 }
 
+static bool core_dedup_ok(const avd_core_weights* w, int B2, int N, int n_out) {
+    const int terms = w->split_terms;
+    return B2 % 2 == 0 && n_out > 0 && n_out + 2 <= N && w->attn_mode == 0 && (terms == 0 || terms == 6 || terms == 9) && g_core_trim &&
+           !g_mlp_fused && gemm_bf16x3_resmap_supported(terms) && core_use_split(w, (int64_t)B2 * N) && core_use_split_fold(w);
+}
+
 static int core_forward(const avd_core_weights* w, const float* x, float* y, int B, int N, int out_row0,
                         int n_out_rows, const unsigned char* kpm, void* ws, int64_t ws_bytes, hipStream_t st,
-                        const float* ss_first = nullptr) {
+                        const float* ss_first = nullptr, const RowSegs* segs = nullptr) {
     if (int rc = check_core(w)) return rc;
     AVD_REQUIRE(x && y && B > 0 && N > 0, AVD_EINVAL, "core: bad input");
     AVD_REQUIRE(out_row0 >= 0 && n_out_rows > 0 && out_row0 + n_out_rows <= N, AVD_EINVAL, "core: bad output row window");
@@ -234,6 +247,10 @@
     const float* cur = x;
     AVD_REQUIRE(!(w->attn_mode == 1 && (kpm || w->norm_kind != 0)), AVD_EUNSUPPORTED,
                 "core: attn_mode 1 (fp8 attention) cannot be combined with a key_padding_mask or norm_kind 1 (LayerNorm)");
+    const int null_from = segs ? segs->samples[0] : 0;
+    AVD_REQUIRE(!segs || (null_from > 0 && segs->n_samples() == B && segs->tok[0] == N && segs->tok[1] == n_out_rows + 1 &&
+                          segs->m0 == (int64_t)null_from * N && out_row0 == 0 && !kpm && core_dedup_ok(w, B, N, n_out_rows)), AVD_EUNSUPPORTED,
+                "core: the two-segment row layout needs the folded six-term split path with the trimmed last block");
     AVD_REQUIRE(!(w->attn_mode == 1 && !core_use_split(w, M)), AVD_EUNSUPPORTED,
                 "core: attn_mode 1 (fp8 attention) reads the q|k|v image of the split-operand projections, which these weights / shapes "
                 "do not take (every block needs its *_weight3 images; 3 d, d and mlp_hidden must be multiples of 256, d of 16)");
@@ -255,18 +272,25 @@
             float* yc = cs.take(core_trim_floats(w, B, N));
             const bool fused = g_mlp_fused && !ns && mlp_bf16x3_supported(d, hid, terms) && gemm_bf16x3_resmap_supported(terms);
             AVD_REQUIRE(cs.ok, AVD_EWORKSPACE, "core: workspace carve %lld > %lld bytes", (long long)cs.used, (long long)cs.cap);
-            if (int rc = split3_rows_f32(cur, rd, hx, M, d, st, 0.f, ss)) return rc;
+            const RowSegs seg = segs ? *segs : RowSegs::uniform(B, N);
+            const int64_t Mr = seg.rows();
+            const float qscale = scale * 1.4426950408889634f;
+            auto in_proj = [&](const avd_block_weights& b) {
+                if (int rc = gemm_bf16x3_qkv3(hx, b.in_proj_weight3n, b.in_proj_bias, qkv, seg, H, d, qscale, terms, st, 1.f, 1.f, ss, w->norm_eps, M))
+                    return rc;
+                return null_from ? qkv3_replicate(qkv, B, H, N, null_from, B - null_from, n_out_rows, st) : (int)AVD_OK;
+            };
+            if (int rc = split3_rows_f32(cur, rd, hx, Mr, d, st, 0.f, ss)) return rc;
             for (int l = 0; l < w->n_layers; ++l) {
                 const avd_block_weights& b = w->blocks[l];
                 const bool last = l == w->n_layers - 1;
                 const int nq = (last && out_row0 == 0) ? n_out_rows : N;
                 if (last && trim) {
                     const int64_t Mc = (int64_t)B * nq;
-                    if (int rc = gemm_bf16x3_qkv3(hx, b.in_proj_weight3n, b.in_proj_bias, qkv, M, N, H, d, scale * 1.4426950408889634f, terms, st,
-                                                  1.f, 1.f, ss, w->norm_eps)) return rc;
+                    if (int rc = in_proj(b)) return rc;
                     if (int rc = attn_bf16x3(qkv, nullptr, hs, B, N, H, nq, terms, st, 1.f, 1.f, nq)) return rc;
                     if (int rc = gemm_bf16x3(hs, b.out_proj_weight3, b.out_proj_bias, cur, yc, hx, Mc, d, d, AVD_ACT_NONE, terms, st, 1.f, 1.f,
-                                             nullptr, 0.f, ss, nullptr, nq, N)) return rc;
+                                             nullptr, 0.f, ss, nullptr, nq, &seg)) return rc;
                     if (fused) {
                         if (int rc = mlp_bf16x3(hx, b.fc1_weight3n, b.fc1_bias, b.fc2_weight3, b.fc2_bias, ss, w->norm_eps, yc, yc, nullptr, nullptr, Mc,
                                                 d, hid, st)) return rc;
@@ -280,36 +304,37 @@
                             if (int rc = gemm_bf16x3(wide3, b.fc2_weight3, b.fc2_bias, yc, yc, nullptr, Mc, d, hid, AVD_ACT_NONE, terms, st)) return rc;
                         }
                     }
-                    return rmsnorm_f32(yc, rd, w->final_norm_scale, y, RowMap{d, nq, (int64_t)N * d}, Mc, d, w->norm_eps, st);
+                    return rmsnorm_f32(yc, rd, w->final_norm_scale, y, null_from ? rd : RowMap{d, nq, (int64_t)N * d}, Mc, d, w->norm_eps, st);
                 }
-                if (int rc = gemm_bf16x3_qkv3(hx, b.in_proj_weight3n, b.in_proj_bias, qkv, M, N, H, d, scale * 1.4426950408889634f, terms, st,
-                                              1.f, 1.f, ss, w->norm_eps)) return rc;
+                if (int rc = in_proj(b)) return rc;
                 if (w->attn_mode == 1) {
                     if (int rc = attn_fp8(qkv, f8w, f8_b, nullptr, hs, B, N, H, nq, st, terms, 1.f, 1.f)) return rc;
+                } else if (null_from) {
+                    if (int rc = attn_bf16x3(qkv, nullptr, hs, B, N, H, N, terms, st, 1.f, 1.f, 0, &seg)) return rc;
                 } else {
                     if (int rc = attn_bf16x3(qkv, nullptr, hs, B, N, H, nq, terms, st, 1.f, 1.f)) return rc;
                 }
-                if (int rc = gemm_bf16x3(hs, b.out_proj_weight3, b.out_proj_bias, cur, y, hx, M, d, d, AVD_ACT_NONE, terms, st, 1.f, 1.f, nullptr,
-                                         0.f, ss)) return rc;
+                if (int rc = gemm_bf16x3(hs, b.out_proj_weight3, b.out_proj_bias, cur, y, hx, Mr, d, d, AVD_ACT_NONE, terms, st, 1.f, 1.f, nullptr,
+                                         0.f, ss, nullptr, 0, nullptr, M)) return rc;
                 cur = y;
                 if (fused) {
                     if (int rc = mlp_bf16x3(hx, b.fc1_weight3n, b.fc1_bias, b.fc2_weight3, b.fc2_bias, ss, w->norm_eps, y, y, last ? nullptr : hx,
-                                            last ? nullptr : ss, M, d, hid, st)) return rc;
+                                            last ? nullptr : ss, Mr, d, hid, st)) return rc;
                     continue;
                 }
-                if (int rc = gemm_bf16x3(hx, b.fc1_weight3n, b.fc1_bias, nullptr, nullptr, wide3, M, hid, d, AVD_ACT_GELU, terms, st, 1.f, 1.f, ss,
-                                         w->norm_eps)) return rc;
+                if (int rc = gemm_bf16x3(hx, b.fc1_weight3n, b.fc1_bias, nullptr, nullptr, wide3, Mr, hid, d, AVD_ACT_GELU, terms, st, 1.f, 1.f, ss,
+                                         w->norm_eps, nullptr, nullptr, 0, nullptr, M)) return rc;
                 if (ns) {
-                    if (int rc = gemm_bf16x3_splitk(wide3, b.fc2_weight3, b.fc2_bias, y, y, last ? nullptr : hx, last ? nullptr : ss, M, d, hid,
+                    if (int rc = gemm_bf16x3_splitk(wide3, b.fc2_weight3, b.fc2_bias, y, y, last ? nullptr : hx, last ? nullptr : ss, Mr, d, hid,
                                                     terms, ns, part, st)) return rc;
                 } else if (last) {
-                    if (int rc = gemm_bf16x3(wide3, b.fc2_weight3, b.fc2_bias, y, y, nullptr, M, d, hid, AVD_ACT_NONE, terms, st)) return rc;
+                    if (int rc = gemm_bf16x3(wide3, b.fc2_weight3, b.fc2_bias, y, y, nullptr, Mr, d, hid, AVD_ACT_NONE, terms, st)) return rc;
                 } else {
-                    if (int rc = gemm_bf16x3(wide3, b.fc2_weight3, b.fc2_bias, y, y, hx, M, d, hid, AVD_ACT_NONE, terms, st, 1.f, 1.f, nullptr, 0.f,
-                                             ss)) return rc;
+                    if (int rc = gemm_bf16x3(wide3, b.fc2_weight3, b.fc2_bias, y, y, hx, Mr, d, hid, AVD_ACT_NONE, terms, st, 1.f, 1.f, nullptr, 0.f,
+                                             ss, nullptr, 0, nullptr, M)) return rc;
                 }
             }
-            return rmsnorm_f32(y, rd, w->final_norm_scale, y, rd, M, d, w->norm_eps, st);
+            return rmsnorm_f32(y, rd, w->final_norm_scale, y, rd, Mr, d, w->norm_eps, st);
         }
         const bool rown = core_use_split_rownorm(w);
         void* hn = rown ? cs.take((split3_bytes(M, d) + 3) / 4) : hs;
@@ -324,7 +349,7 @@
             const float w_in = h2 ? fs[0] : 1.f, w_out = h2 ? fs[1] : 1.f, w_fc1 = h2 ? fs[2] : 1.f, w_fc2 = h2 ? fs[3] : 1.f;
             if (!rown || l == 0)
                 if (int rc = rmsnorm_split3_f32(cur, b.norm1_scale, hn, M, d, w->norm_eps, st, s_n1)) return rc;
-            if (int rc = gemm_bf16x3_qkv3(hn, b.in_proj_weight3, b.in_proj_bias, qkv, M, N, H, d, scale * 1.4426950408889634f, terms, st,
+            if (int rc = gemm_bf16x3_qkv3(hn, b.in_proj_weight3, b.in_proj_bias, qkv, RowSegs::uniform(B, N), H, d, scale * 1.4426950408889634f, terms, st,
                                           h2 ? s_n1 * w_in : 1.f, s_qkv)) return rc;
             if (w->attn_mode == 1) {
                 if (int rc = attn_fp8(qkv, f8w, f8_b, nullptr, hs, B, N, H, nq, st, terms, s_qkv, s_qkv)) return rc;
@@ -505,9 +530,11 @@
 
 static int embed_cfg_pair(const avd_embed_desc* e, const float* z, const float* Wt, const float* bt,
                           const int64_t* t_now, const float* Xp, float* tok_ws, float* X2, hipStream_t st, float* ss_out = nullptr,
-                          bool cond_only = false) {
+                          bool cond_only = false, const RowSegs* short_null = nullptr) {
     if (int rc = check_embed(e)) return rc;
     AVD_REQUIRE(z && Wt && t_now && tok_ws && X2 && (e->Np == 0 || Xp), AVD_EINVAL, "embed: null pointer");
+    AVD_REQUIRE(!short_null || (!cond_only && !e->temb_add && e->target_first && e->Np >= 1), AVD_EINVAL,
+                "embed: the short null half is the concat-mode CFG pair with the target rows first");
     const int B = e->B, d = e->d, N = e->Nt + e->Np, D = embed_tok_dim(e);
     float* tok = tok_ws;
     float* temb = tok_ws + align_up((int64_t)B * e->Nt * D * 4) / 4;
@@ -536,7 +563,8 @@
     }
     if (cond_only)
         return assemble_rows_cond_f32(X2, t_now, e->temb_freqs, Xp, ss_out, B, N, d, e->tdim, e->Nt, e->Np, e->target_first, 10000.f, st);
-    return assemble_rows_f32(X2, t_now, e->temb_freqs, Xp, ss_out, B, N, d, e->tdim, e->Nt, e->Np, e->target_first, 10000.f, st);
+    return assemble_rows_f32(X2, t_now, e->temb_freqs, Xp, ss_out, B, N, d, e->tdim, e->Nt, e->Np, e->target_first, 10000.f, st,
+                             short_null);
 }
 
 #define AVD_HIP(call)                                                                        \
@@ -669,6 +697,12 @@
     return set_error(AVD_EINVAL, "tune_set: unknown key '%s'", key);
 }
 
+extern "C" int avd_cfg_dedup_set(int on) {
+    const int prev = g_cfg_dedup;
+    g_cfg_dedup = on != 0;
+    return prev;
+}
+
 extern "C" int avd_device_arch(char* buf, int buflen) {
     AVD_REQUIRE(buf && buflen > 0, AVD_EINVAL, "device_arch: bad buffer");
     hipDeviceProp_t prop;
@@ -737,10 +771,15 @@
     const avd_embed_desc& e = s->embed;
     const bool have_ss = !e.temb_add;
 
-    if (int rc = embed_cfg_pair(&e, z, s->adapt_w, s->adapt_b, t_now, Xp, tok, X2, st, ssx)) return rc;
+    const bool dedup = g_cfg_dedup && !s->split_streams && !e.temb_add && e.target_first && e.Np >= 2 && core_dedup_ok(s->core, 2 * e.B, p.N, e.Nt);
+    const RowSegs seg{(int64_t)e.B * p.N, {p.N, e.Nt + 1}, {e.B, e.B}};
+    if (int rc = embed_cfg_pair(&e, z, s->adapt_w, s->adapt_b, t_now, Xp, tok, X2, st, ssx, false, dedup ? &seg : nullptr)) return rc;
     const int row0 = e.target_first ? 0 : e.Np;
     const RowMap hm{e.d, e.Nt, (int64_t)p.N * e.d};
-    if (!s->split_streams) {
+    if (dedup) {
+        if (int rc = core_forward(s->core, X2, X2, 2 * e.B, p.N, 0, e.Nt, nullptr, core_ws, p.core, st, nullptr, &seg)) return rc;
+        if (int rc = head_forward(s->head, X2, RowMap{e.d, 0, 0}, p.rows, eps2, head_ws, p.head, st)) return rc;
+    } else if (!s->split_streams) {
         if (int rc = core_forward(s->core, X2, X2, 2 * e.B, p.N, row0, e.Nt, nullptr, core_ws, p.core, st, have_ss ? ssx : nullptr)) return rc;
         if (int rc = head_forward(s->head, X2 + (int64_t)row0 * e.d, hm, p.rows, eps2, head_ws, p.head, st)) return rc;
     } else {
diff --git a/multimodal_diffusion_amd/csrc/gemm_bf16x3.hip b/multimodal_diffusion_amd/csrc/gemm_bf16x3.hip
--- a/multimodal_diffusion_amd/csrc/gemm_bf16x3.hip
+++ b/multimodal_diffusion_amd/csrc/gemm_bf16x3.hip
@@ -210,7 +210,7 @@
         const int dmodel = g.heads * 64;
         const int part = nbase / dmodel, head = (nbase % dmodel) >> 6;
         mul = part == 0 ? g.qscale : 1.0f;
-        qbase = (((int64_t)part * (g.M / g.tokN)) * g.heads + head) * (int64_t)g.tokNpad * QKV3_ROWB;
+        qbase = (((int64_t)part * g.seg.n_samples()) * g.heads + head) * (int64_t)g.tokNpad * QKV3_ROWB;
     }
 #pragma unroll
     for (int i = 0; i < 4; ++i) {
@@ -232,7 +232,8 @@
         [[maybe_unused]] unsigned char* qrow = nullptr;
         [[maybe_unused]] int qsw = 0;
         if constexpr (EPI == S3_EPI_QKV3) {
-            const unsigned b = (unsigned)m / (unsigned)g.tokN, tok = (unsigned)m - b * (unsigned)g.tokN;
+            int b, tok;
+            g.seg.locate(m, b, tok);
             const int dmodel = g.heads * 64;
             qrow = g.C3 + qbase + ((int64_t)b * g.heads * g.tokNpad + tok) * QKV3_ROWB;
             qsw = qkv3_swizzle(nbase / dmodel, (int)tok);
@@ -1378,26 +1379,27 @@
 
 template <int EPI, int TERMS>
 static int launch_s3t(const S3Args& a, hipStream_t st) {
+    const int64_t Mp = a.M_plan > a.M ? a.M_plan : a.M;
     if constexpr (TERMS == 6 && EPI != S3_EPI_RES_NORM) {
         if (g_s3_m16) {
-            if (s3_tile_for(EPI, a.M, a.N)) {
+            if (s3_tile_for(EPI, Mp, a.N)) {
                 if constexpr (EPI == S3_EPI_BIAS || EPI == S3_EPI_SPLIT || EPI == S3_EPI_RES_IMG) {
                     constexpr int E2 = EPI == S3_EPI_BIAS ? (int)S3_EPI_BIAS_REG : (int)EPI;
-                    const int rt = s3_rt4_for(a.M, a.N, 2);
-                    if ((EPI == S3_EPI_RES_IMG || (a.bias && a.N % 128 == 0)) && s3_deep4_for(a.M, a.N, rt))
+                    const int rt = s3_rt4_for(Mp, a.N, 2);
+                    if ((EPI == S3_EPI_RES_IMG || (a.bias && a.N % 128 == 0)) && s3_deep4_for(Mp, a.N, rt))
                         return *s3_with_rt<2, 8>(rt, true, [&](auto r) { return launch_s3w16<E2, 4, r(), 4>(a, st); });
                     if constexpr (EPI == S3_EPI_RES_IMG) {
                         if (const auto rc = s3_with_rt<2, 4>(rt, false, [&](auto r) { return launch_s3w16<EPI, 4, r()>(a, st); })) return *rc;
                     }
                 }
                 if constexpr (EPI == S3_EPI_GELU_SPLIT || EPI == S3_EPI_QKV3 || EPI == S3_EPI_RES_IMG) {
-                    const int rt = s3_rt4_for(a.M, a.N, 5);
+                    const int rt = s3_rt4_for(Mp, a.N, 5);
                     if (const auto rc = s3_with_rt<5, 7>(rt, false, [&](auto r) { return launch_s3w16<EPI, 4, r()>(a, st); })) return *rc;
                 }
                 return launch_s3w16<EPI, 4>(a, st);
             }
             constexpr bool RI = EPI == S3_EPI_RES_IMG;
-            const int rt = RI ? s3_rt8_for(a.M, a.N) : 8;
+            const int rt = RI ? s3_rt8_for(Mp, a.N) : 8;
             if constexpr (RI || EPI == S3_EPI_GELU_SPLIT || EPI == S3_EPI_SPLIT || EPI == S3_EPI_QKV3) {
                 if (g_s3_w128) return *s3_with_rt<RI ? 6 : 7, 8>(rt, true, [&](auto r) { return launch_s3w128<EPI, r()>(a, st); });
             }
@@ -1411,7 +1413,7 @@
         if constexpr (TERMS == 3) return launch_s3w<EPI, 3, 8>(a, st);
         else AVD_REQUIRE(false, AVD_EUNSUPPORTED, "gemm_bf16x3: the residual + RMSNorm epilogue exists for f16x2 images only");
     } else {
-        return s3_tile_for(EPI, a.M, a.N) ? launch_s3w<EPI, TERMS, 4>(a, st) : launch_s3w<EPI, TERMS, 8>(a, st);
+        return s3_tile_for(EPI, Mp, a.N) ? launch_s3w<EPI, TERMS, 4>(a, st) : launch_s3w<EPI, TERMS, 8>(a, st);
     }
 }
 
@@ -1439,8 +1441,9 @@
 
 int gemm_bf16x3(const void* A3, const void* W3, const float* bias, const float* R, float* C, void* C3, int64_t M, int N, int K,
                 int act, int terms, hipStream_t st, float ab_scale, float c_scale, const float* ss_in, float eps, float* ss_out,
-                const float* gamma, int r_seg, int r_stride) {
-    AVD_REQUIRE(r_seg == 0 || (r_seg > 0 && r_stride >= r_seg && ss_out && gemm_bf16x3_resmap_supported(terms) && M < (1ll << 31)), AVD_EUNSUPPORTED,
+                const float* gamma, int r_seg, const RowSegs* r_map, int64_t plan_rows) {
+    AVD_REQUIRE(r_seg == 0 || (r_seg > 0 && r_map && r_map->tok[0] >= r_seg && r_map->tok[1] >= r_seg && M == (int64_t)r_map->n_samples() * r_seg &&
+                               ss_out && gemm_bf16x3_resmap_supported(terms) && r_map->rows() < (1ll << 31)), AVD_EUNSUPPORTED,
                 "gemm_bf16x3: a residual row map needs the fp32 + image residual epilogue of the six-term 16x16x32 kernels");
     AVD_REQUIRE(A3 && W3 && (C || C3), AVD_EINVAL, "gemm_bf16x3: null pointer");
     AVD_REQUIRE(!gamma || (gemm_bf16x3_rownorm_supported(N, terms) && C && C3 && R && bias && !ss_in && !ss_out && act == AVD_ACT_NONE && aligned16(gamma)),
@@ -1457,7 +1460,8 @@
     a.bias = bias, a.R = R, a.C = C, a.C3 = static_cast<unsigned char*>(C3);
     a.ab_inv = 1.0f / ab_scale, a.c_scale = c_scale;
     a.ss_in = ss_in, a.ss_out = ss_out, a.ss_sqrt_d = (float)sqrt((double)K), a.ss_eps = eps;
-    a.gamma = gamma, a.r_seg = r_seg, a.r_stride = r_stride;
+    a.gamma = gamma, a.r_seg = r_seg, a.M_plan = plan_rows;
+    if (r_seg) a.seg = *r_map;
     if (gamma) {
         a.ss_sqrt_d = (float)sqrt((double)N);
         return launch_s3<S3_EPI_RES_NORM>(a, st);
@@ -1561,20 +1565,23 @@
     return AVD_OK;
 }
 
-int gemm_bf16x3_qkv3(const void* A3, const void* W3, const float* bias, void* img, int64_t M, int tokens, int heads, int K, float qscale,
-                     int terms, hipStream_t st, float ab_scale, float c_scale, const float* ss_in, float eps) {
+int gemm_bf16x3_qkv3(const void* A3, const void* W3, const float* bias, void* img, const RowSegs& seg, int heads, int K, float qscale,
+                     int terms, hipStream_t st, float ab_scale, float c_scale, const float* ss_in, float eps, int64_t plan_rows) {
+    const int64_t M = seg.rows();
+    const int tokens = seg.tok[0] > seg.tok[1] ? seg.tok[0] : seg.tok[1];
     AVD_REQUIRE(!ss_in || K % 64 == 0, AVD_EUNSUPPORTED, "gemm_bf16x3_qkv3: a folded norm needs K %% 64 == 0");
     AVD_REQUIRE(A3 && W3 && bias && img, AVD_EINVAL, "gemm_bf16x3_qkv3: null pointer");
     AVD_REQUIRE(scale_ok(ab_scale) && scale_ok(c_scale), AVD_EINVAL, "gemm_bf16x3_qkv3: image scales must be positive and finite");
     const int N = 3 * heads * 64;
-    AVD_REQUIRE(tokens > 0 && heads > 0 && M > 0 && M % tokens == 0, AVD_EINVAL, "gemm_bf16x3_qkv3: rows %lld not a multiple of tokens %d",
-                (long long)M, tokens);
+    AVD_REQUIRE(seg.tok[0] > 0 && seg.tok[1] > 0 && seg.samples[0] > 0 && seg.samples[1] >= 0 && heads > 0 &&
+                    seg.m0 == (int64_t)seg.samples[0] * seg.tok[0], AVD_EINVAL, "gemm_bf16x3_qkv3: bad row layout (%d x %d + %d x %d rows)",
+                seg.samples[0], seg.tok[0], seg.samples[1], seg.tok[1]);
     AVD_REQUIRE(M < (1ll << 31) - 256, AVD_EUNSUPPORTED, "gemm_bf16x3_qkv3: more than 2^31 rows");
     AVD_REQUIRE(gemm_bf16x3_supported(M, N, K), AVD_EUNSUPPORTED, "gemm_bf16x3_qkv3: need 3*heads*64 %% 256 == 0 and K %% 16 == 0");
     AVD_REQUIRE(aligned16(A3) && aligned16(W3) && aligned16(bias) && aligned16(img), AVD_EUNSUPPORTED, "gemm_bf16x3_qkv3: alignment");
     S3Args a = s3_args(A3, W3, M, N, K, terms);
     a.bias = bias, a.C3 = static_cast<unsigned char*>(img);
-    a.tokN = tokens, a.tokNpad = qkv3_npad(tokens), a.heads = heads, a.qscale = qscale;
+    a.seg = seg, a.tokNpad = qkv3_npad(tokens), a.heads = heads, a.qscale = qscale, a.M_plan = plan_rows;
     a.ab_inv = 1.0f / ab_scale, a.c_scale = c_scale;
     a.ss_in = ss_in, a.ss_sqrt_d = (float)sqrt((double)K), a.ss_eps = eps;
     return launch_s3<S3_EPI_QKV3>(a, st);
@@ -1601,7 +1608,10 @@
 }
 extern "C" int avd_gemm_bf16x3_qkv3_f32(const void* A3, const void* W3, const float* bias, void* qkv3, int64_t M, int tokens, int heads,
                                         int K, float qscale, int terms, avd_stream_t stream) {
-    return gemm_bf16x3_qkv3(A3, W3, bias, qkv3, M, tokens, heads, K, qscale, terms, static_cast<hipStream_t>(stream));
+    AVD_REQUIRE(tokens > 0 && M > 0 && M % tokens == 0 && M < (1ll << 31), AVD_EINVAL, "gemm_bf16x3_qkv3: rows %lld not a multiple of tokens %d",
+                (long long)M, tokens);
+    return gemm_bf16x3_qkv3(A3, W3, bias, qkv3, RowSegs::uniform((int)(M / tokens), tokens), heads, K, qscale, terms,
+                            static_cast<hipStream_t>(stream));
 }
 
 extern "C" int avd_split_f16x2_f32(const float* x, void* out, int64_t rows, int K, float scale, avd_stream_t stream) {
@@ -1619,5 +1629,8 @@
 }
 extern "C" int avd_gemm_f16x2_qkv_f32(const void* A2, const void* W2, const float* bias, void* qkv, int64_t M, int tokens, int heads, int K,
                                       float qscale, float ab_scale, float qkv_scale, avd_stream_t stream) {
-    return gemm_bf16x3_qkv3(A2, W2, bias, qkv, M, tokens, heads, K, qscale, 3, static_cast<hipStream_t>(stream), ab_scale, qkv_scale);
-}
+    AVD_REQUIRE(tokens > 0 && M > 0 && M % tokens == 0 && M < (1ll << 31), AVD_EINVAL, "gemm_f16x2_qkv: rows %lld not a multiple of tokens %d",
+                (long long)M, tokens);
+    return gemm_bf16x3_qkv3(A2, W2, bias, qkv, RowSegs::uniform((int)(M / tokens), tokens), heads, K, qscale, 3,
+                            static_cast<hipStream_t>(stream), ab_scale, qkv_scale);
+}
diff --git a/multimodal_diffusion_amd/csrc/s3_common.h b/multimodal_diffusion_amd/csrc/s3_common.h
--- a/multimodal_diffusion_amd/csrc/s3_common.h
+++ b/multimodal_diffusion_amd/csrc/s3_common.h
@@ -17,8 +17,10 @@
     float* C;
     unsigned char* C3;
     int64_t M;
+    int64_t M_plan;
     int N, K, nbn, sm, sn;
-    int tokN, tokNpad, heads;
+    RowSegs seg;
+    int tokNpad, heads;
     float qscale;
     int stagger;
     int first_gen;
@@ -28,7 +30,7 @@
     float* ss_out;
     float ss_sqrt_d, ss_eps;
     const float* gamma;
-    int r_seg, r_stride;
+    int r_seg;
 #ifdef AVD_S3_STAMPS
     unsigned long long* dbg;
 #endif
@@ -107,7 +109,7 @@
         const int dmodel = g.heads * 64;
         const int part = nbase / dmodel, head = (nbase % dmodel) >> 6;
         mul = part == 0 ? g.qscale : 1.0f;
-        qbase = (((int64_t)part * (g.M / g.tokN)) * g.heads + head) * (int64_t)g.tokNpad * QKV3_ROWB;
+        qbase = (((int64_t)part * g.seg.n_samples()) * g.heads + head) * (int64_t)g.tokNpad * QKV3_ROWB;
     }
 #pragma unroll
     for (int ip = 0; ip < 4; ++ip) {
@@ -130,7 +132,8 @@
         [[maybe_unused]] unsigned char* qrow = nullptr;
         [[maybe_unused]] int qsw = 0;
         if constexpr (EPI == S3_EPI_QKV3) {
-            const unsigned b = (unsigned)m / (unsigned)g.tokN, tok = (unsigned)m - b * (unsigned)g.tokN;
+            int b, tok;
+            g.seg.locate(m, b, tok);
             qrow = g.C3 + qbase + ((int64_t)b * g.heads * g.tokNpad + tok) * QKV3_ROWB;
             qsw = qkv3_swizzle(nbase / (g.heads * 64), (int)tok);
         }
@@ -139,7 +142,7 @@
         if constexpr (EPI == S3_EPI_RES_IMG) {
             if (g.r_seg > 0 && m < g.M) {
                 const unsigned sgi = (unsigned)m / (unsigned)g.r_seg;
-                rrow = (int64_t)sgi * g.r_stride + ((unsigned)m - sgi * (unsigned)g.r_seg);
+                rrow = g.seg.row((int)sgi, (int)((unsigned)m - sgi * (unsigned)g.r_seg));
             }
         }
 #pragma unroll
diff --git a/multimodal_diffusion_amd/csrc/tokens.hip b/multimodal_diffusion_amd/csrc/tokens.hip
--- a/multimodal_diffusion_amd/csrc/tokens.hip
+++ b/multimodal_diffusion_amd/csrc/tokens.hip
@@ -1368,12 +1368,12 @@
 __global__ __launch_bounds__(256) void assemble_rows_kernel(float* __restrict__ X2, const int64_t* __restrict__ t_now,
                                                             const float* __restrict__ freqs, const float* __restrict__ Xp,
                                                             float* __restrict__ ss, int B, int N, int d, int tdim, int Nt, int Np,
-                                                            int target_first, float neg_log_mp) {
+                                                            int target_first, float neg_log_mp, RowSegs seg) {
     const int lane = threadIdx.x & 63;
     const int64_t row = (int64_t)blockIdx.x * 4 + (threadIdx.x >> 6);
-    if (row >= (int64_t)2 * B * N) return;
-    const int n = (int)(row % N);
-    const int bb = (int)(row / N);
+    if (row >= seg.rows()) return;
+    int n, bb;
+    seg.locate(row, bb, n);
     const int half = bb >= B, b = half ? bb - B : bb;
     const int t0 = target_first ? 0 : Np;
     const bool is_t = n >= t0 && n < t0 + Nt;
@@ -1413,13 +1413,53 @@
 }
 
 int assemble_rows_f32(float* X2, const int64_t* t_now, const float* freqs, const float* Xp, float* ss, int B, int N, int d, int tdim,
-                      int Nt, int Np, int target_first, float max_period, hipStream_t st) {
-    const int64_t rows = (int64_t)2 * B * N;
+                      int Nt, int Np, int target_first, float max_period, hipStream_t st, const RowSegs* short_null) {
+    AVD_REQUIRE(!short_null || (target_first && Np >= 1 && short_null->samples[0] == B && short_null->samples[1] == B && short_null->tok[0] == N &&
+                                short_null->tok[1] == Nt + 1 && short_null->m0 == (int64_t)B * N), AVD_EINVAL,
+                "assemble_rows: a short null half is B samples of N rows, then B of the target rows and one prompt row behind them");
+    const RowSegs seg = short_null ? *short_null : RowSegs::uniform(2 * B, N);
+    const int64_t rows = seg.rows();
     static const int tag = prof_tag_id("assemble_rows_kernel");
-    ProfScope prof(tag, 4.0 * (2.0 * B * N * d + (double)B * Nt * (d - tdim) + (double)B * Np * d), st);
+    ProfScope prof(tag, 4.0 * ((double)rows * d + (double)B * Nt * (d - tdim) + (double)B * Np * d), st);
     hipLaunchKernelGGL(assemble_rows_kernel, dim3((unsigned)((rows + 3) / 4)), dim3(256), 0, st, X2, t_now, freqs, Xp, ss, B, N, d, tdim,
-                       Nt, Np, target_first, -(float)log((double)max_period));
+                       Nt, Np, target_first, -(float)log((double)max_period), seg);
     AVD_CHECK_LAUNCH("assemble_rows");
+    return AVD_OK;
+}
+
+__global__ __launch_bounds__(256) void qkv3_replicate_kernel(unsigned char* __restrict__ img, int Bt, int H, int Npad, int first_sample,
+                                                             int n_samples, int src, int n_keys) {
+    const int dup = n_keys - 1 - src;
+    const int64_t i = (int64_t)blockIdx.x * 256 + threadIdx.x;
+    const int64_t total = (int64_t)2 * n_samples * H * dup * 24;
+    if (i >= total) return;
+    const int c = (int)(i % 8), plane = (int)(i / 8 % 3);
+    int64_t r = i / 24;
+    const int j = (int)(r % dup);
+    r /= dup;
+    const int h = (int)(r % H);
+    r /= H;
+    const int b = (int)(r % n_samples), part = 1 + (int)(r / n_samples);
+    unsigned char* base = img + (((int64_t)part * Bt + first_sample + b) * H + h) * (int64_t)Npad * QKV3_ROWB;
+    const int dst = src + 1 + j;
+    const u32x4 v = *reinterpret_cast<const u32x4*>(base + (int64_t)src * QKV3_ROWB + plane * 128 + ((c ^ qkv3_swizzle(part, src)) << 4));
+    *reinterpret_cast<u32x4*>(base + (int64_t)dst * QKV3_ROWB + plane * 128 + ((c ^ qkv3_swizzle(part, dst)) << 4)) = v;
+}
+
+int qkv3_replicate(void* img, int img_samples, int H, int n_keys, int first_sample, int n_samples, int src, hipStream_t st) {
+    AVD_REQUIRE(img && aligned16(img), AVD_EINVAL, "qkv3_replicate: null or misaligned image");
+    AVD_REQUIRE(H > 0 && n_keys > 0 && src >= 0 && src < n_keys && first_sample >= 0 && n_samples > 0 && first_sample + n_samples <= img_samples,
+                AVD_EINVAL, "qkv3_replicate: bad geometry (samples %d + %d of %d, token %d of %d keys)", first_sample, n_samples, img_samples,
+                src, n_keys);
+    const int dup = n_keys - 1 - src;
+    if (dup == 0) return AVD_OK;
+    const int64_t total = (int64_t)2 * n_samples * H * dup * 24;
+    AVD_REQUIRE((total + 255) / 256 < (1ll << 31), AVD_EUNSUPPORTED, "qkv3_replicate: grid too large");
+    static const int tag = prof_tag_id("qkv3_replicate_kernel");
+    ProfScope prof(tag, 32.0 * (double)total, st);
+    hipLaunchKernelGGL(qkv3_replicate_kernel, dim3((unsigned)((total + 255) / 256)), dim3(256), 0, st, static_cast<unsigned char*>(img),
+                       img_samples, H, qkv3_npad(n_keys), first_sample, n_samples, src, n_keys);
+    AVD_CHECK_LAUNCH("qkv3_replicate");
     return AVD_OK;
 }
 
```

After: 117.2 steps/s, median of 6. +2.0%, better.
